# openai/ot-gan

Hardware: AMD Instinct MI355X
Metric: OT-GAN train images/sec (CIFAR-10 32x32, bs=256/GPU) (higher is better)
Workload: dtype f32 (Winograd-domain GEMMs on the fp16 matrix pipe with operands split into two scaled fp16 pieces = 22 significand bits, fp32 accumulate; errors at or below the fp32 MFMA chain's)

## Files before the change

### include/otgan_layers.h

```cpp
#ifndef OTGAN_LAYERS_H
#define OTGAN_LAYERS_H

#define OTGAN_ACT_NONE 0
#define OTGAN_ACT_CRELU 1
#define OTGAN_ACT_CELU 2
#define OTGAN_ACT_ELU 3
#define OTGAN_ACT_RELU 4

typedef struct otgan_conv_desc {
  int N;
  int H, W;
  int C;
  int ldx;
  int upsample;
  int KH, KW;
  int stride;
  int Cout;
  int ldy;
  int y_coff;
  int preact;
  int list_quads;
  const float* x_amax;
  const float* dy_amax;
  int y_accumulate;
  void* x_operand;
  float* y_amax_out;
  float* dx_amax_out;
  const float* w_amax;
  int x_amax_count;
  int list_width;
  float* glu_out;
  float* glu_amax_out;
  int dy_amax_count;
} otgan_conv_desc;


size_t otgan_conv2d_workspace_bytes(const otgan_conv_desc* d, int which);
int otgan_conv2d_glu_fused(const otgan_conv_desc* d);
size_t otgan_conv2d_operand_bytes(const otgan_conv_desc* d);

#define OTGAN_AMAX_RECORD_FLOATS 512
int otgan_absmax_f32(const float* x, long rows, int C, long ld, float* record, void* stream);
int otgan_conv2d_amax_fused(const otgan_conv_desc* d, int which);


size_t otgan_conv2d_folded_weight_elems(const otgan_conv_desc* d);
int otgan_conv2d_fold_weights_f32(const otgan_conv_desc* d, const float* w, float* weff,
                                  float* weffT, void* stream);

int otgan_conv2d_fwd_f32(const otgan_conv_desc* d, const float* x, const int32_t* cmap,
                         const float* wT, const float* bias, float* y, void* workspace,
                         size_t workspace_bytes, void* stream);

int otgan_conv2d_dgrad_f32(const otgan_conv_desc* d, const float* dy, const float* w,
                           const float* x, const int32_t* inv, float* dx, int lddx,
                           int accumulate, void* workspace, size_t workspace_bytes, void* stream);

size_t otgan_conv2d_filter_bytes(const otgan_conv_desc* d, int which);
#define OTGAN_DENSE16_MAX_BATCH 16
size_t otgan_dense16_filter_bytes(int nslices);
int otgan_dense16_prepare_filters_f32(const float* const* wT, const int* nslices, void* const* filters, int count,
                                      void* stream);
int otgan_dense16_h2_ok(const otgan_conv_desc* d);
int otgan_dense16_chain_fwd_f32(int N, int H, int W, int nslices, float* buf_group, int ld, const void* const* filters,
                                float* records, void* stream);
int otgan_dense16_chain_bwd_f32(int N, int H, int W, int nslices, float* g_group, int ldg, const float* x_group, int ldx,
                                const void* const* filters, const float* rec0, float* slice_records, void* stream);
typedef struct otgan_dense16_bwd_pair {
  const float* w;
  const void* fwd_filters;
  void* filters;
  int nslices_src, slice_index, pair_index;
} otgan_dense16_bwd_pair;
size_t otgan_dense16_bwd_filter_bytes(int npairs);
int otgan_dense16_prepare_bwd_filters_f32(const otgan_dense16_bwd_pair* pairs, int npairs, const void* const* all_fwd_filters,
                                          int nall, void* stream);
int otgan_dense16_bwd_slice_f32(int N, int H, int W, int npairs, const float* g, int ldg, const void* filters, const float* x,
                                int ldx, float* dx, const float* rec0, int nrec0, const float* rec1, int nrec1,
                                float* amax_out, void* stream);
int otgan_conv2d_prepare_filters_f32(const otgan_conv_desc* d, int which, const float* w, void* filters,
                                     size_t filter_bytes, void* stream);
int otgan_conv2d_prepare_filters_raw_f32(const otgan_conv_desc* d, int which, const float* V, const float* scale,
                                         void* filters, size_t filter_bytes, void* stream);
int otgan_conv2d_fwd_pf_f32(const otgan_conv_desc* d, const float* x, const int32_t* cmap,
                            const float* wT, const void* filters, const float* bias, float* y,
                            void* workspace, size_t workspace_bytes, void* stream);
int otgan_conv2d_dgrad_pf_f32(const otgan_conv_desc* d, const float* dy, const float* w, const void* filters,
                              const float* x, const int32_t* inv, float* dx, int lddx,
                              int accumulate, void* workspace, size_t workspace_bytes, void* stream);

int otgan_conv2d_wgrad_f32(const otgan_conv_desc* d, const float* x, const int32_t* cmap,
                           const float* dy, float* dw, void* workspace, size_t workspace_bytes,
                           void* stream);

int otgan_weightnorm_fwd_f32(const float* V, const float* g, int K, int Cout, float* w,
                             float* wT, float* inv_norm, void* stream);
int otgan_weightnorm_fwd_amax_f32(const float* V, const float* g, int K, int Cout, float* w, float* wT,
                                  float* inv_norm, float* w_amax, void* stream);
size_t otgan_weightnorm_scale_scratch_floats(int K, int Cout);
int otgan_weightnorm_scale_amax_f32(const float* V, const float* g, int K, int Cout, float* inv_norm, float* scale,
                                    float* w_amax, float* scratch, size_t scratch_floats, void* stream);
int otgan_weightnorm_bwd_f32(const float* V, const float* g, const float* inv_norm,
                             const float* dw, int K, int Cout, float* dV, float* dg,
                             float* scratch, void* stream);

#define OTGAN_WN_MAX_LAYERS 16
typedef struct otgan_wn_fwd_layer {
  const float* V;
  const float* g;
  float* w;
  float* wT;
  float* inv;
  int K;
} otgan_wn_fwd_layer;
typedef struct otgan_wn_part {
  const float* p;
  const int32_t* perm;
  int nrows;
  int rstride;
} otgan_wn_part;
typedef struct otgan_wn_bwd_layer {
  const float* V;
  const float* g;
  const float* inv;
  float* dV;
  float* dg;
  int Ceff, taps;
  otgan_wn_part part[3];
} otgan_wn_bwd_layer;
int otgan_weightnorm_fwd_batched16_f32(const otgan_wn_fwd_layer* layers, int n_layers, void* stream);
int otgan_weightnorm_bwd_batched16_f32(const otgan_wn_bwd_layer* layers, int n_layers, void* stream);

int otgan_colsum_f32(const float* a, long rows, int cols, long lda, float* out, float* scratch,
                     void* stream);

int otgan_glu_fwd_f32(const float* x, long rows, int C, float* y, void* stream);
int otgan_glu_bwd_f32(const float* x, const float* dy, long rows, int C, float* dx, void* stream);
int otgan_glu_fwd_amax_f32(const float* x, long rows, int C, float* y, float* y_amax, void* stream);
int otgan_glu_bwd_amax_f32(const float* x, const float* dy, long rows, int C, float* dx, float* dx_amax, void* stream);
int otgan_glu_bwd_colsum_f32(const float* x, const float* dy, long rows, int C, float* dx, float* dx_amax, float* colsum,
                             float* scratch, void* stream);
int otgan_tanh_fwd_f32(const float* x, long n, float* y, void* stream);
int otgan_tanh_bwd_f32(const float* y, const float* dy, long n, float* dx, void* stream);
int otgan_feature_head_fwd_f32(const float* x, int N, int HW, int C, float* f, float* norm,
                               void* stream);
int otgan_feature_head_bwd_f32(const float* x, const float* f, const float* norm,
                               const float* df, int N, int HW, int C, float* dx, void* stream);
int otgan_feature_head_bwd_amax_f32(const float* x, const float* f, const float* norm, const float* df, int N, int HW,
                                    int C, float* dx, float* dx_amax, void* stream);

int otgan_adam_step_f32(float* p, const float* grad, float* v, float* mg, long n, double lr,
                        double mom1, double mom2, double t, void* stream);
#define OTGAN_ADAM_MAX_SEGMENTS 32
int otgan_adam_step_gather_f32(float* p, const float* const* grads, const long* offsets, int nseg, float* v, float* mg,
                               double lr, double mom1, double mom2, double t, float* ema_shadow, double ema_decay,
                               void* stream);
void otgan_adam_coefficients(double mom1, double mom2, double t, float* out2);
int otgan_adam_step_coef_f32(float* p, const float* grad, float* v, float* mg, long n, double lr,
                             double mom1, double mom2, double t, const float* coef_dev, void* stream);
int otgan_adam_step_gather_coef_f32(float* p, const float* const* grads, const long* offsets, int nseg, float* v, float* mg,
                                    double lr, double mom1, double mom2, double t, const float* coef_dev, float* ema_shadow,
                                    double ema_decay, void* stream);
#define OTGAN_COPY2D_MAX_SEGMENTS 64
int otgan_copy2d_batched_f32(const float* const* src, float* const* dst, const int* rows, const int* cols,
                             const long* src_ld, const long* dst_ld, int nseg, void* stream);
#define OTGAN_GATHER3D_MAX_SEGMENTS 32
int otgan_gather3d_batched_f32(const float* const* src, float* const* dst, const int* n0, int n1, int n2,
                               const long* src_s0, const long* src_s1, const long* dst_s0, const long* dst_s1,
                               int base1, const int* map1_dev, float* amax_out, int nseg, void* stream);
int otgan_adamax_step_f32(float* p, const float* grad, float* v, float* mg, long n, double lr,
                          double mom1, double mom2, void* stream);
int otgan_nesterov_step_f32(float* p, const float* grad, float* v, long n, double lr, double mom1,
                            void* stream);
int otgan_ema_update_f32(float* shadow, const float* p, long n, double decay, void* stream);

typedef struct otgan_incep_conv_desc {
  int N, H, W;
  int C, ldx;
  int KH, KW;
  int stride_h, stride_w;
  int same;
  int Cout;
  int ldy, y_coff;
  int relu;
} otgan_incep_conv_desc;

#define OTGAN_INCEP_POOL_MAX 0
#define OTGAN_INCEP_POOL_AVG 1
typedef struct otgan_incep_pool_desc {
  int N, H, W, C, ldx;
  int KH, KW, stride_h, stride_w, same;
  int op;
  int ldy, y_coff;
} otgan_incep_pool_desc;

int otgan_incep_out_size(int in, int k, int stride, int same);
int otgan_incep_conv2d_f32(const otgan_incep_conv_desc* d, const float* x, const float* w, const float* bias, float* y,
                           void* stream);
int otgan_incep_pool_f32(const otgan_incep_pool_desc* d, const float* x, float* y, void* stream);
int otgan_incep_resize_f32(int N, int H, int W, int C, int OH, int OW, int align_corners, float scale, float shift,
                           const float* x, float* y, void* stream);
int otgan_incep_head_f32(int N, int HW, int C, int ldx, int classes, const float* x, const float* w, float* pool3,
                         float* logits, float* probs, void* stream);

int otgan_moments_update_f64(int n, int C, int ldx, const float* x, double* sum, double* outer, void* stream);

size_t otgan_kid_workspace_bytes(int nsub, int m);
int otgan_kid_sums_f64(int nsub, int m, int C, const float* x, int ldx, const int32_t* xi, const float* y, int ldy,
                       const int32_t* yi, double* out, void* workspace, size_t workspace_bytes, void* stream);

size_t otgan_knn_workspace_bytes(int nq, int ny, int k);
int otgan_knn_f64(int nq, int ny, int C, const float* q, int ldq, const float* y, int ldy, int k, int self0,
                  const double* thresh, double* nearest, int32_t* inside, void* workspace, size_t workspace_bytes,
                  void* stream);

size_t otgan_topk_dot_workspace_bytes(int nq, int ny, int k);
int otgan_topk_dot_f64(int nq, int ny, int C, const float* q, int ldq, const float* y, int ldy, int k, int self0,
                       int32_t* index, double* score, void* workspace, size_t workspace_bytes, void* stream);

#define OTGAN_BATCH_U8_MAX_SHARDS 32
int otgan_batch_from_u8_f32(const uint8_t* store, long n_images, int SH, int SW, const int32_t* perm, long perm_len,
                            const long* shard_offsets, int n_shards, int B, const uint8_t* flip, const float* lut, int S,
                            float* out, long ldo, void* stream);

#define OTGAN_AUG_COLOR 1
#define OTGAN_AUG_TRANSLATION 2
#define OTGAN_AUG_CUTOUT 4
int otgan_augment_fwd_f32(const float* x, long rows, int S, const float* u, int policy, float* y, void* stream);
int otgan_augment_bwd_f32(const float* dy, long rows, int S, const float* u, int policy, float* dx, void* stream);

#endif
```

### ot-gan_amd/_lib_layers.py

```python
import ctypes

c_fp = ctypes.c_void_p
c_int, c_long, c_float, c_size_t = ctypes.c_int, ctypes.c_long, ctypes.c_float, ctypes.c_size_t
c_double = ctypes.c_double


class ConvDesc(ctypes.Structure):
    _fields_ = [("N", c_int), ("H", c_int), ("W", c_int), ("C", c_int), ("ldx", c_int),
                ("upsample", c_int), ("KH", c_int), ("KW", c_int), ("stride", c_int),
                ("Cout", c_int), ("ldy", c_int), ("y_coff", c_int), ("preact", c_int),
                ("list_quads", c_int), ("x_amax", ctypes.c_void_p), ("dy_amax", ctypes.c_void_p),
                ("y_accumulate", c_int), ("x_operand", ctypes.c_void_p),
                ("y_amax_out", ctypes.c_void_p), ("dx_amax_out", ctypes.c_void_p), ("w_amax", ctypes.c_void_p),
                ("x_amax_count", c_int), ("list_width", c_int),
                ("glu_out", ctypes.c_void_p), ("glu_amax_out", ctypes.c_void_p), ("dy_amax_count", c_int)]


P_DESC = ctypes.POINTER(ConvDesc)


class IncepConvDesc(ctypes.Structure):
    _fields_ = [("N", c_int), ("H", c_int), ("W", c_int), ("C", c_int), ("ldx", c_int), ("KH", c_int), ("KW", c_int),
                ("stride_h", c_int), ("stride_w", c_int), ("same", c_int), ("Cout", c_int), ("ldy", c_int),
                ("y_coff", c_int), ("relu", c_int)]


class IncepPoolDesc(ctypes.Structure):
    _fields_ = [("N", c_int), ("H", c_int), ("W", c_int), ("C", c_int), ("ldx", c_int), ("KH", c_int), ("KW", c_int),
                ("stride_h", c_int), ("stride_w", c_int), ("same", c_int), ("op", c_int), ("ldy", c_int),
                ("y_coff", c_int)]


INCEP_POOL_MAX, INCEP_POOL_AVG = 0, 1


class Dense16BwdPair(ctypes.Structure):
    _fields_ = [("w", ctypes.c_void_p), ("fwd_filters", ctypes.c_void_p), ("filters", ctypes.c_void_p),
                ("nslices_src", c_int), ("slice_index", c_int), ("pair_index", c_int)]


class WnFwdLayer(ctypes.Structure):
    _fields_ = [("V", c_fp), ("g", c_fp), ("w", c_fp), ("wT", c_fp), ("inv", c_fp), ("K", c_int)]


class WnPart(ctypes.Structure):
    _fields_ = [("p", c_fp), ("perm", c_fp), ("nrows", c_int), ("rstride", c_int)]


class WnBwdLayer(ctypes.Structure):
    _fields_ = [("V", c_fp), ("g", c_fp), ("inv", c_fp), ("dV", c_fp), ("dg", c_fp), ("Ceff", c_int), ("taps", c_int),
                ("part", WnPart * 3)]


SIGNATURES = {
    "otgan_conv2d_workspace_bytes": (c_size_t, [P_DESC, c_int]),
    "otgan_conv2d_operand_bytes": (c_size_t, [P_DESC]),
    "otgan_conv2d_glu_fused": (c_int, [P_DESC]),
    "otgan_absmax_f32": (c_int, [c_fp, c_long, c_int, c_long, c_fp, c_fp]),
    "otgan_conv2d_amax_fused": (c_int, [P_DESC, c_int]),
    "otgan_conv2d_folded_weight_elems": (c_size_t, [P_DESC]),
    "otgan_conv2d_fold_weights_f32": (c_int, [P_DESC, c_fp, c_fp, c_fp, c_fp]),
    "otgan_conv2d_fwd_f32": (c_int, [P_DESC, c_fp, c_fp, c_fp, c_fp, c_fp, c_fp, c_size_t, c_fp]),
    "otgan_conv2d_dgrad_f32": (c_int, [P_DESC, c_fp, c_fp, c_fp, c_fp, c_fp, c_int, c_int, c_fp,
                                       c_size_t, c_fp]),
    "otgan_conv2d_wgrad_f32": (c_int, [P_DESC, c_fp, c_fp, c_fp, c_fp, c_fp, c_size_t, c_fp]),
    "otgan_conv2d_filter_bytes": (c_size_t, [P_DESC, c_int]),
    "otgan_dense16_filter_bytes": (c_size_t, [c_int]),
    "otgan_dense16_prepare_filters_f32": (c_int, [c_fp, c_fp, c_fp, c_int, c_fp]),
    "otgan_dense16_h2_ok": (c_int, [P_DESC]),
    "otgan_dense16_chain_fwd_f32": (c_int, [c_int, c_int, c_int, c_int, c_fp, c_int, c_fp, c_fp, c_fp]),
    "otgan_dense16_chain_bwd_f32": (c_int, [c_int, c_int, c_int, c_int, c_fp, c_int, c_fp, c_int, c_fp, c_fp, c_fp, c_fp]),
    "otgan_dense16_bwd_filter_bytes": (c_size_t, [c_int]),
    "otgan_dense16_prepare_bwd_filters_f32": (c_int, [c_fp, c_int, c_fp, c_int, c_fp]),
    "otgan_dense16_bwd_slice_f32": (c_int, [c_int, c_int, c_int, c_int, c_fp, c_int, c_fp, c_fp, c_int, c_fp, c_fp, c_int,
                                            c_fp, c_int, c_fp, c_fp]),
    "otgan_conv2d_prepare_filters_f32": (c_int, [P_DESC, c_int, c_fp, c_fp, c_size_t, c_fp]),
    "otgan_conv2d_fwd_pf_f32": (c_int, [P_DESC, c_fp, c_fp, c_fp, c_fp, c_fp, c_fp, c_fp, c_size_t, c_fp]),
    "otgan_conv2d_dgrad_pf_f32": (c_int, [P_DESC, c_fp, c_fp, c_fp, c_fp, c_fp, c_fp, c_int, c_int, c_fp,
                                          c_size_t, c_fp]),
    "otgan_weightnorm_fwd_f32": (c_int, [c_fp, c_fp, c_int, c_int, c_fp, c_fp, c_fp, c_fp]),
    "otgan_weightnorm_fwd_amax_f32": (c_int, [c_fp, c_fp, c_int, c_int, c_fp, c_fp, c_fp, c_fp, c_fp]),
    "otgan_weightnorm_scale_scratch_floats": (c_size_t, [c_int, c_int]),
    "otgan_weightnorm_scale_amax_f32": (c_int, [c_fp, c_fp, c_int, c_int, c_fp, c_fp, c_fp, c_fp, c_size_t, c_fp]),
    "otgan_conv2d_prepare_filters_raw_f32": (c_int, [P_DESC, c_int, c_fp, c_fp, c_fp, c_size_t, c_fp]),
    "otgan_weightnorm_bwd_f32": (c_int, [c_fp, c_fp, c_fp, c_fp, c_int, c_int, c_fp, c_fp, c_fp, c_fp]),
    "otgan_weightnorm_fwd_batched16_f32": (c_int, [ctypes.POINTER(WnFwdLayer), c_int, c_fp]),
    "otgan_weightnorm_bwd_batched16_f32": (c_int, [ctypes.POINTER(WnBwdLayer), c_int, c_fp]),
    "otgan_colsum_f32": (c_int, [c_fp, c_long, c_int, c_long, c_fp, c_fp, c_fp]),
    "otgan_glu_fwd_f32": (c_int, [c_fp, c_long, c_int, c_fp, c_fp]),
    "otgan_glu_bwd_f32": (c_int, [c_fp, c_fp, c_long, c_int, c_fp, c_fp]),
    "otgan_glu_fwd_amax_f32": (c_int, [c_fp, c_long, c_int, c_fp, c_fp, c_fp]),
    "otgan_glu_bwd_amax_f32": (c_int, [c_fp, c_fp, c_long, c_int, c_fp, c_fp, c_fp]),
    "otgan_feature_head_bwd_amax_f32": (c_int, [c_fp, c_fp, c_fp, c_fp, c_int, c_int, c_int, c_fp, c_fp, c_fp]),
    "otgan_tanh_fwd_f32": (c_int, [c_fp, c_long, c_fp, c_fp]),
    "otgan_tanh_bwd_f32": (c_int, [c_fp, c_fp, c_long, c_fp, c_fp]),
    "otgan_feature_head_fwd_f32": (c_int, [c_fp, c_int, c_int, c_int, c_fp, c_fp, c_fp]),
    "otgan_feature_head_bwd_f32": (c_int, [c_fp, c_fp, c_fp, c_fp, c_int, c_int, c_int, c_fp, c_fp]),
    "otgan_adam_step_f32": (c_int, [c_fp, c_fp, c_fp, c_fp, c_long, c_double, c_double, c_double,
                                    c_double, c_fp]),
    "otgan_adam_step_gather_f32": (c_int, [c_fp, c_fp, c_fp, c_int, c_fp, c_fp, c_double, c_double, c_double, c_double,
                                           c_fp, c_double, c_fp]),
    "otgan_adam_step_gather_coef_f32": (c_int, [c_fp, c_fp, c_fp, c_int, c_fp, c_fp, c_double, c_double, c_double, c_double,
                                                c_fp, c_fp, c_double, c_fp]),
    "otgan_adam_coefficients": (None, [c_double, c_double, c_double, c_fp]),
    "otgan_adam_step_coef_f32": (c_int, [c_fp, c_fp, c_fp, c_fp, c_long, c_double, c_double, c_double,
                                         c_double, c_fp, c_fp]),
    "otgan_glu_bwd_colsum_f32": (c_int, [c_fp, c_fp, c_long, c_int, c_fp, c_fp, c_fp, c_fp, c_fp]),
    "otgan_copy2d_batched_f32": (c_int, [c_fp, c_fp, c_fp, c_fp, c_fp, c_fp, c_int, c_fp]),
    "otgan_gather3d_batched_f32": (c_int, [c_fp, c_fp, c_fp, c_int, c_int, c_fp, c_fp, c_fp, c_fp, c_int, c_fp, c_fp, c_int, c_fp]),
    "otgan_adamax_step_f32": (c_int, [c_fp, c_fp, c_fp, c_fp, c_long, c_double, c_double, c_double, c_fp]),
    "otgan_nesterov_step_f32": (c_int, [c_fp, c_fp, c_fp, c_long, c_double, c_double, c_fp]),
    "otgan_ema_update_f32": (c_int, [c_fp, c_fp, c_long, c_double, c_fp]),
    "otgan_incep_out_size": (c_int, [c_int, c_int, c_int, c_int]),
    "otgan_incep_conv2d_f32": (c_int, [ctypes.POINTER(IncepConvDesc), c_fp, c_fp, c_fp, c_fp, c_fp]),
    "otgan_incep_pool_f32": (c_int, [ctypes.POINTER(IncepPoolDesc), c_fp, c_fp, c_fp]),
    "otgan_incep_resize_f32": (c_int, [c_int, c_int, c_int, c_int, c_int, c_int, c_int, c_float, c_float, c_fp, c_fp, c_fp]),
    "otgan_incep_head_f32": (c_int, [c_int, c_int, c_int, c_int, c_int, c_fp, c_fp, c_fp, c_fp, c_fp, c_fp]),
    "otgan_moments_update_f64": (c_int, [c_int, c_int, c_int, c_fp, c_fp, c_fp, c_fp]),
    "otgan_kid_workspace_bytes": (c_size_t, [c_int, c_int]),
    "otgan_kid_sums_f64": (c_int, [c_int, c_int, c_int, c_fp, c_int, c_fp, c_fp, c_int, c_fp, c_fp, c_fp, c_size_t, c_fp]),
    "otgan_knn_workspace_bytes": (c_size_t, [c_int, c_int, c_int]),
    "otgan_knn_f64": (c_int, [c_int, c_int, c_int, c_fp, c_int, c_fp, c_int, c_int, c_int, c_fp, c_fp, c_fp, c_fp, c_size_t, c_fp]),
    "otgan_topk_dot_workspace_bytes": (c_size_t, [c_int, c_int, c_int]),
    "otgan_topk_dot_f64": (c_int, [c_int, c_int, c_int, c_fp, c_int, c_fp, c_int, c_int, c_int, c_fp, c_fp, c_fp, c_size_t, c_fp]),
    "otgan_batch_from_u8_f32": (c_int, [c_fp, c_long, c_int, c_int, c_fp, c_long, c_fp, c_int, c_int, c_fp, c_fp, c_int,
                                        c_fp, c_long, c_fp]),
    "otgan_augment_fwd_f32": (c_int, [c_fp, c_long, c_int, c_fp, c_int, c_fp, c_fp]),
    "otgan_augment_bwd_f32": (c_int, [c_fp, c_long, c_int, c_fp, c_int, c_fp, c_fp]),
}
```

### ot-gan_amd/csrc/pointwise.hip

```cpp
#include "common.h"
#include "../../include/otgan.h"

namespace {

constexpr int kChunks = 256;

inline int grid_for(long n, int per_thread = 4) {
  long b = ceil_div_l(n, 256L * per_thread);
  if (b > 4096) b = 4096;
  if (b < 1) b = 1;
  return (int)b;
}

template <int OP, bool CMAX>
__device__ __forceinline__ void colreduce_body(const float* __restrict__ a, const float* __restrict__ b, long rows,
                                               int cols, long lda, float* __restrict__ partial,
                                               unsigned* __restrict__ pmax) {
  const int lane = threadIdx.x & 63, wave = threadIdx.x >> 6;
  const int c = blockIdx.x * 64 + lane;
  const int chunk = blockIdx.y;
  const long per = ceil_div_l(rows, (long)gridDim.y);
  const long r0 = chunk * per;
  long r1 = r0 + per;
  if (r1 > rows) r1 = rows;
  float s = 0.f;
  unsigned m = 0u;
  if (c < cols) {
    for (long r = r0 + wave; r < r1; r += 4) {
      const float av = a[r * lda + c];
      if (OP == 0) s += av;
      else if (OP == 1) s += av * av;
      else s += av * b[r * lda + c];
      if constexpr (CMAX) {
        const unsigned ab = amax_bits(av);
        m = ab > m ? ab : m;
      }
    }
  }
  __shared__ float red[4][64];
  red[wave][lane] = s;
  __syncthreads();
  if (wave == 0 && c < cols)
    partial[(long)chunk * cols + c] = (red[0][lane] + red[1][lane]) + (red[2][lane] + red[3][lane]);
  if constexpr (CMAX) {
    __shared__ unsigned redm[4][64];
    redm[wave][lane] = m;
    __syncthreads();
    if (wave == 0 && c < cols) {
#pragma unroll
      for (int k = 1; k < 4; ++k) m = redm[k][lane] > m ? redm[k][lane] : m;
      pmax[(long)chunk * cols + c] = m;
    }
  }
}
template <int OP>
__global__ __launch_bounds__(256) void colreduce_kernel(const float* __restrict__ a,
                                                        const float* __restrict__ b, long rows,
                                                        int cols, long lda,
                                                        float* __restrict__ partial) {
  colreduce_body<OP, false>(a, b, rows, cols, lda, partial, nullptr);
}
__global__ __launch_bounds__(256) void colsq_cmax_kernel(const float* __restrict__ a, long rows, int cols, long lda,
                                                         float* __restrict__ partial, unsigned* __restrict__ pmax) {
  colreduce_body<1, true>(a, nullptr, rows, cols, lda, partial, pmax);
}

template <int MODE>
__global__ __launch_bounds__(256) void colreduce_finish_kernel(const float* __restrict__ partial,
                                                               int nchunk, int cols,
                                                               float* __restrict__ out) {
  const int lane = threadIdx.x & 63, part = threadIdx.x >> 6;
  const int c = blockIdx.x * 64 + lane;
  float s = 0.f;
  if (c < cols)
    for (int k = part; k < nchunk; k += 4) s += partial[(long)k * cols + c];
  __shared__ float red[4][64];
  red[part][lane] = s;
  __syncthreads();
  if (part == 0 && c < cols) {
    const float t = (red[0][lane] + red[1][lane]) + (red[2][lane] + red[3][lane]);
    out[c] = MODE == 1 ? rsqrtf(fmaxf(t, 1e-12f)) : t;
  }
}

template <int OP, bool CMAX>
__device__ __forceinline__ void colreduce4_body(const float* __restrict__ a, const float* __restrict__ b, long rows,
                                                int cols, long lda, float* __restrict__ partial,
                                                unsigned* __restrict__ pmax) {
  const int lane = threadIdx.x & 63, wave = threadIdx.x >> 6;
  const int cq = lane & 15, rsub = (lane >> 4) + 4 * wave;
  const int c = blockIdx.x * 64 + 4 * cq;
  const int chunk = blockIdx.y;
  const long per = ceil_div_l(rows, (long)gridDim.y);
  const long r0 = chunk * per;
  long r1 = r0 + per;
  if (r1 > rows) r1 = rows;
  float4 s = make_float4(0.f, 0.f, 0.f, 0.f);
  uint4 m = make_uint4(0u, 0u, 0u, 0u);
  if (c < cols) {
    for (long r = r0 + rsub; r < r1; r += 16) {
      const float4 av = *reinterpret_cast<const float4*>(a + r * lda + c);
      if (OP == 0) {
        s.x += av.x; s.y += av.y; s.z += av.z; s.w += av.w;
      } else if (OP == 1) {
        s.x += av.x * av.x; s.y += av.y * av.y; s.z += av.z * av.z; s.w += av.w * av.w;
      } else {
        const float4 bv = *reinterpret_cast<const float4*>(b + r * lda + c);
        s.x += av.x * bv.x; s.y += av.y * bv.y; s.z += av.z * bv.z; s.w += av.w * bv.w;
      }
      if constexpr (CMAX) {
        const unsigned bx = amax_bits(av.x), by = amax_bits(av.y), bz = amax_bits(av.z), bw = amax_bits(av.w);
        m.x = bx > m.x ? bx : m.x; m.y = by > m.y ? by : m.y; m.z = bz > m.z ? bz : m.z; m.w = bw > m.w ? bw : m.w;
      }
    }
  }
  __shared__ float4 red[16][17];
  red[rsub][cq] = s;
  __syncthreads();
  if (threadIdx.x < 16 && c < cols) {
    float4 t = make_float4(0.f, 0.f, 0.f, 0.f);
#pragma unroll
    for (int k = 0; k < 16; ++k) {
      const float4 v = red[k][threadIdx.x];
      t.x += v.x; t.y += v.y; t.z += v.z; t.w += v.w;
    }
    const int cc = blockIdx.x * 64 + 4 * threadIdx.x;
    *reinterpret_cast<float4*>(partial + (long)chunk * cols + cc) = t;
  }
  if constexpr (CMAX) {
    __shared__ uint4 redm[16][17];
    redm[rsub][cq] = m;
    __syncthreads();
    if (threadIdx.x < 16 && c < cols) {
      uint4 u = make_uint4(0u, 0u, 0u, 0u);
#pragma unroll
      for (int k = 0; k < 16; ++k) {
        const uint4 v = redm[k][threadIdx.x];
        u.x = v.x > u.x ? v.x : u.x; u.y = v.y > u.y ? v.y : u.y; u.z = v.z > u.z ? v.z : u.z; u.w = v.w > u.w ? v.w : u.w;
      }
      *reinterpret_cast<uint4*>(pmax + (long)chunk * cols + (blockIdx.x * 64 + 4 * threadIdx.x)) = u;
    }
  }
}
template <int OP>
__global__ __launch_bounds__(256) void colreduce4_kernel(const float* __restrict__ a,
                                                         const float* __restrict__ b, long rows,
                                                         int cols, long lda,
                                                         float* __restrict__ partial) {
  colreduce4_body<OP, false>(a, b, rows, cols, lda, partial, nullptr);
}
__global__ __launch_bounds__(256) void colsq_cmax4_kernel(const float* __restrict__ a, long rows, int cols, long lda,
                                                          float* __restrict__ partial, unsigned* __restrict__ pmax) {
  colreduce4_body<1, true>(a, nullptr, rows, cols, lda, partial, pmax);
}

template <int OP>
int colreduce(const float* a, const float* b, long rows, int cols, long lda, float* partial,
              int* nchunk_out, hipStream_t s, unsigned* pmax = nullptr) {
  const int colblocks = ceil_div(cols, 64);
  long nchunk = ceil_div(1024, colblocks);
  if (nchunk > kChunks) nchunk = kChunks;
  if (nchunk > ceil_div_l(rows, 64)) nchunk = ceil_div_l(rows, 64);
  if (nchunk < 1) nchunk = 1;
  dim3 grid(colblocks, (int)nchunk);
  const bool vec = (cols % 4 == 0) && (lda % 4 == 0) && ((reinterpret_cast<uintptr_t>(a) & 15) == 0) &&
                   (!b || (reinterpret_cast<uintptr_t>(b) & 15) == 0) &&
                   ((reinterpret_cast<uintptr_t>(partial) & 15) == 0) &&
                   ((reinterpret_cast<uintptr_t>(pmax) & 15) == 0);
  if (pmax) {
    if (vec) hipLaunchKernelGGL(colsq_cmax4_kernel, grid, dim3(256), 0, s, a, rows, cols, lda, partial, pmax);
    else hipLaunchKernelGGL(colsq_cmax_kernel, grid, dim3(256), 0, s, a, rows, cols, lda, partial, pmax);
  } else if (vec) hipLaunchKernelGGL(colreduce4_kernel<OP>, grid, dim3(256), 0, s, a, b, rows, cols, lda, partial);
  else hipLaunchKernelGGL(colreduce_kernel<OP>, grid, dim3(256), 0, s, a, b, rows, cols, lda, partial);
  *nchunk_out = (int)nchunk;
  OTGAN_CHECK_LAUNCH("colreduce");
  return OTGAN_OK;
}

__global__ __launch_bounds__(256) void weightnorm_apply_kernel(const float* __restrict__ V,
                                                               const float* __restrict__ g,
                                                               const float* __restrict__ inv,
                                                               int K, int Cout,
                                                               float* __restrict__ w,
                                                               float* __restrict__ wT,
                                                               float* __restrict__ rec) {
  __shared__ float tile[32][33];
  const int c0 = blockIdx.x * 32, k0 = blockIdx.y * 32;
  const int tx = threadIdx.x & 31, ty = threadIdx.x >> 5;
  unsigned mb = 0u;
#pragma unroll
  for (int i = 0; i < 4; ++i) {
    const int k = k0 + ty + 8 * i, c = c0 + tx;
    float v = 0.f;
    if (k < K && c < Cout) {
      v = V[(long)k * Cout + c] * (g[c] * inv[c]);
      w[(long)k * Cout + c] = v;
    }
    tile[ty + 8 * i][tx] = v;
    const unsigned b = amax_bits(v);
    mb = b > mb ? b : mb;
  }
  if (wT) {
    __syncthreads();
#pragma unroll
    for (int i = 0; i < 4; ++i) {
      const int c = c0 + ty + 8 * i, k = k0 + tx;
      if (k < K && c < Cout) wT[(long)c * K + k] = tile[tx][ty + 8 * i];
    }
  }
  if (rec) amax_commit(rec, mb);
}

__global__ __launch_bounds__(256) void weightnorm_scale_finish_kernel(const float* __restrict__ partial,
                                                                      const unsigned* __restrict__ pmax, int nchunk,
                                                                      int cols, const float* __restrict__ g,
                                                                      float* __restrict__ inv, float* __restrict__ scale,
                                                                      float* __restrict__ rec) {
  const int lane = threadIdx.x & 63, part = threadIdx.x >> 6;
  const int c = blockIdx.x * 64 + lane;
  float s = 0.f;
  unsigned m = 0u;
  if (c < cols)
    for (int k = part; k < nchunk; k += 4) {
      s += partial[(long)k * cols + c];
      const unsigned b = pmax[(long)k * cols + c];
      m = b > m ? b : m;
    }
  __shared__ float red[4][64];
  __shared__ unsigned redm[4][64];
  red[part][lane] = s;
  redm[part][lane] = m;
  __syncthreads();
  unsigned mb = 0u;
  if (part == 0 && c < cols) {
    const float t = (red[0][lane] + red[1][lane]) + (red[2][lane] + red[3][lane]);
    const float iv = rsqrtf(fmaxf(t, 1e-12f));
    const float sc = __fmul_rn(g[c], iv);
#pragma unroll
    for (int k = 1; k < 4; ++k) m = redm[k][lane] > m ? redm[k][lane] : m;
    inv[c] = iv;
    scale[c] = sc;
    mb = amax_bits(__fmul_rn(__uint_as_float(m), sc));
  }
  amax_commit(rec, mb);
}

__global__ void weightnorm_bwd_kernel(const float* __restrict__ V, const float* __restrict__ g,
                                      const float* __restrict__ inv, const float* __restrict__ dw,
                                      const float* __restrict__ dot, long total, int Cout,
                                      float* __restrict__ dV) {
  for (long i = (long)blockIdx.x * blockDim.x + threadIdx.x; i < total;
       i += (long)gridDim.x * blockDim.x) {
    const int c = (int)(i % Cout);
    const float iv = inv[c];
    dV[i] = g[c] * iv * (dw[i] - V[i] * dot[c] * iv * iv);
  }
}
__global__ __launch_bounds__(256) void wn_dot_finish_kernel(const float* __restrict__ partial, int nchunk, int cols,
                                                            const float* __restrict__ inv, float* __restrict__ dot,
                                                            float* __restrict__ dg) {
  const int lane = threadIdx.x & 63, part = threadIdx.x >> 6;
  const int c = blockIdx.x * 64 + lane;
  float s = 0.f;
  if (c < cols)
    for (int k = part; k < nchunk; k += 4) s += partial[(long)k * cols + c];
  __shared__ float red[4][64];
  red[part][lane] = s;
  __syncthreads();
  if (part == 0 && c < cols) {
    const float t = (red[0][lane] + red[1][lane]) + (red[2][lane] + red[3][lane]);
    dot[c] = t;
    dg[c] = t * inv[c];
  }
}
__global__ void weightnorm_dg_kernel(const float* __restrict__ dot, const float* __restrict__ inv,
                                     int Cout, float* __restrict__ dg) {
  const int c = blockIdx.x * blockDim.x + threadIdx.x;
  if (c < Cout) dg[c] = dot[c] * inv[c];
}

constexpr int kWnThreads = 512, kWnRowLanes = kWnThreads / 4;
inline bool aligned16(const void* p) { return (reinterpret_cast<uintptr_t>(p) & 15) == 0; }
struct WnFwdArgs {
  otgan_wn_fwd_layer l[OTGAN_WN_MAX_LAYERS];
};
struct WnBwdArgs {
  otgan_wn_bwd_layer l[OTGAN_WN_MAX_LAYERS];
};
__device__ __forceinline__ float4 wn_tree(float4 v, float4 (*red)[4], int rl, int cq) {
  red[rl][cq] = v;
  __syncthreads();
#pragma unroll
  for (int h = kWnRowLanes / 2; h > 0; h >>= 1) {
    if (rl < h) {
      const float4 a = red[rl][cq], b = red[rl + h][cq];
      red[rl][cq] = make_float4(a.x + b.x, a.y + b.y, a.z + b.z, a.w + b.w);
    }
    __syncthreads();
  }
  const float4 r = red[0][cq];
  __syncthreads();
  return r;
}
__global__ __launch_bounds__(kWnThreads) void wn_fwd_batched_kernel(WnFwdArgs a) {
  __shared__ float4 red[kWnRowLanes][4];
  const otgan_wn_fwd_layer& L = a.l[blockIdx.x];
  const int cq = threadIdx.x & 3, rl = threadIdx.x >> 2;
  float4 s = make_float4(0.f, 0.f, 0.f, 0.f);
  for (int r = rl; r < L.K; r += kWnRowLanes) {
    const float4 v = *reinterpret_cast<const float4*>(L.V + (long)r * 16 + 4 * cq);
    s.x += v.x * v.x; s.y += v.y * v.y; s.z += v.z * v.z; s.w += v.w * v.w;
  }
  s = wn_tree(s, red, rl, cq);
  const float4 g = *reinterpret_cast<const float4*>(L.g + 4 * cq);
  const float4 iv = make_float4(rsqrtf(fmaxf(s.x, 1e-12f)), rsqrtf(fmaxf(s.y, 1e-12f)), rsqrtf(fmaxf(s.z, 1e-12f)),
                                rsqrtf(fmaxf(s.w, 1e-12f)));
  if (rl == 0) *reinterpret_cast<float4*>(L.inv + 4 * cq) = iv;
  const float4 sc = make_float4(g.x * iv.x, g.y * iv.y, g.z * iv.z, g.w * iv.w);
  for (int r = rl; r < L.K; r += kWnRowLanes) {
    const float4 v = *reinterpret_cast<const float4*>(L.V + (long)r * 16 + 4 * cq);
    const float4 w = make_float4(v.x * sc.x, v.y * sc.y, v.z * sc.z, v.w * sc.w);
    *reinterpret_cast<float4*>(L.w + (long)r * 16 + 4 * cq) = w;
    if (L.wT) {
      float* t = L.wT + (long)(4 * cq) * L.K + r;
      t[0] = w.x; t[L.K] = w.y; t[2L * L.K] = w.z; t[3L * L.K] = w.w;
    }
  }
}
__device__ __forceinline__ const float* wn_dw_row(const otgan_wn_bwd_layer& L, int tap, int e) {
#pragma unroll
  for (int i = 0; i < 3; ++i) {
    const otgan_wn_part& p = L.part[i];
    if (e < p.nrows || i == 2) {
      const int ee = p.perm ? p.perm[e] : e;
      return p.p + ((long)tap * p.nrows + ee) * p.rstride;
    }
    e -= p.nrows;
  }
  return nullptr;
}
__global__ __launch_bounds__(kWnThreads) void wn_bwd_batched_kernel(WnBwdArgs a) {
  __shared__ float4 red[kWnRowLanes][4];
  const otgan_wn_bwd_layer& L = a.l[blockIdx.x];
  const int cq = threadIdx.x & 3, rl = threadIdx.x >> 2;
  const int K = L.taps * L.Ceff;
  float4 s = make_float4(0.f, 0.f, 0.f, 0.f);
  for (int r = rl; r < K; r += kWnRowLanes) {
    const int tap = r / L.Ceff, e = r - tap * L.Ceff;
    const float4 d = *reinterpret_cast<const float4*>(wn_dw_row(L, tap, e) + 4 * cq);
    const float4 v = *reinterpret_cast<const float4*>(L.V + (long)r * 16 + 4 * cq);
    s.x += d.x * v.x; s.y += d.y * v.y; s.z += d.z * v.z; s.w += d.w * v.w;
  }
  s = wn_tree(s, red, rl, cq);
  const float4 g = *reinterpret_cast<const float4*>(L.g + 4 * cq);
  const float4 iv = *reinterpret_cast<const float4*>(L.inv + 4 * cq);
  if (rl == 0) *reinterpret_cast<float4*>(L.dg + 4 * cq) = make_float4(s.x * iv.x, s.y * iv.y, s.z * iv.z, s.w * iv.w);
  const float4 sc = make_float4(g.x * iv.x, g.y * iv.y, g.z * iv.z, g.w * iv.w);
  const float4 pr = make_float4(s.x * iv.x * iv.x, s.y * iv.y * iv.y, s.z * iv.z * iv.z, s.w * iv.w * iv.w);
  for (int r = rl; r < K; r += kWnRowLanes) {
    const int tap = r / L.Ceff, e = r - tap * L.Ceff;
    const float4 d = *reinterpret_cast<const float4*>(wn_dw_row(L, tap, e) + 4 * cq);
    const float4 v = *reinterpret_cast<const float4*>(L.V + (long)r * 16 + 4 * cq);
    *reinterpret_cast<float4*>(L.dV + (long)r * 16 + 4 * cq) =
        make_float4(sc.x * (d.x - v.x * pr.x), sc.y * (d.y - v.y * pr.y), sc.z * (d.z - v.z * pr.z), sc.w * (d.w - v.w * pr.w));
  }
}

__device__ __forceinline__ float sigmoidf_(float x) { return 1.f / (1.f + expf(-x)); }

__global__ void glu_fwd_kernel(const float* __restrict__ x, long rows, int C, float* __restrict__ y) {
  const long total = rows * C;
  for (long i = (long)blockIdx.x * blockDim.x + threadIdx.x; i < total;
       i += (long)gridDim.x * blockDim.x) {
    const long r = i / C;
    const int c = (int)(i - r * C);
    const float a = x[r * 2 * C + c], l = x[r * 2 * C + C + c];
    y[i] = a * sigmoidf_(l);
  }
}
__global__ void glu_bwd_kernel(const float* __restrict__ x, const float* __restrict__ dy, long rows,
                               int C, float* __restrict__ dx) {
  const long total = rows * C;
  for (long i = (long)blockIdx.x * blockDim.x + threadIdx.x; i < total;
       i += (long)gridDim.x * blockDim.x) {
    const long r = i / C;
    const int c = (int)(i - r * C);
    const float a = x[r * 2 * C + c], l = x[r * 2 * C + C + c];
    const float s = sigmoidf_(l), d = dy[i];
    dx[r * 2 * C + c] = d * s;
    dx[r * 2 * C + C + c] = d * a * s * (1.f - s);
  }
}
__global__ __launch_bounds__(256) void glu_fwd4_kernel(const float* __restrict__ x, long rows, int C4,
                                                       float* __restrict__ y, float* __restrict__ rec) {
  const long total = rows * C4;
  unsigned mb = 0u;
  for (long i = (long)blockIdx.x * 256 + threadIdx.x; i < total; i += (long)gridDim.x * 256) {
    const long r = i / C4;
    const long c = i - r * C4;
    const f32x4 a = *reinterpret_cast<const f32x4*>(x + 4 * (r * 2 * C4 + c));
    const f32x4 l = *reinterpret_cast<const f32x4*>(x + 4 * (r * 2 * C4 + C4 + c));
    f32x4 o;
#pragma unroll
    for (int k = 0; k < 4; ++k) o[k] = a[k] * sigmoidf_(l[k]);
    *reinterpret_cast<f32x4*>(y + 4 * i) = o;
    mb = amax_bits4(o, mb);
  }
  if (rec) amax_commit(rec, mb);
}
__global__ __launch_bounds__(256) void glu_bwd4_kernel(const float* __restrict__ x, const float* __restrict__ dy,
                                                       long rows, int C4, float* __restrict__ dx,
                                                       float* __restrict__ rec) {
  const long total = rows * C4;
  unsigned mb = 0u;
  for (long i = (long)blockIdx.x * 256 + threadIdx.x; i < total; i += (long)gridDim.x * 256) {
    const long r = i / C4;
    const long c = i - r * C4;
    const f32x4 a = *reinterpret_cast<const f32x4*>(x + 4 * (r * 2 * C4 + c));
    const f32x4 l = *reinterpret_cast<const f32x4*>(x + 4 * (r * 2 * C4 + C4 + c));
    const f32x4 d = *reinterpret_cast<const f32x4*>(dy + 4 * i);
    f32x4 da, dl;
#pragma unroll
    for (int k = 0; k < 4; ++k) {
      const float s = sigmoidf_(l[k]);
      da[k] = d[k] * s;
      dl[k] = d[k] * a[k] * s * (1.f - s);
    }
    *reinterpret_cast<f32x4*>(dx + 4 * (r * 2 * C4 + c)) = da;
    *reinterpret_cast<f32x4*>(dx + 4 * (r * 2 * C4 + C4 + c)) = dl;
    mb = amax_bits4(dl, amax_bits4(da, mb));
  }
  if (rec) amax_commit(rec, mb);
}
__global__ __launch_bounds__(256) void glu_bwd4_colsum_kernel(const float* __restrict__ x, const float* __restrict__ dy,
                                                              long rows, int C, float* __restrict__ dx,
                                                              float* __restrict__ rec, float* __restrict__ partial) {
  const int lane = threadIdx.x & 63, wave = threadIdx.x >> 6;
  const int cq = lane & 15, rsub = (lane >> 4) + 4 * wave;
  const int c = blockIdx.x * 64 + 4 * cq;
  const int chunk = blockIdx.y;
  const long per = ceil_div_l(rows, (long)gridDim.y);
  const long r0 = chunk * per;
  long r1 = r0 + per;
  if (r1 > rows) r1 = rows;
  f32x4 sa = {0.f, 0.f, 0.f, 0.f}, sl = {0.f, 0.f, 0.f, 0.f};
  unsigned mb = 0u;
  if (c < C) {
    for (long r = r0 + rsub; r < r1; r += 16) {
      const f32x4 a = *reinterpret_cast<const f32x4*>(x + r * 2 * C + c);
      const f32x4 l = *reinterpret_cast<const f32x4*>(x + r * 2 * C + C + c);
      const f32x4 d = *reinterpret_cast<const f32x4*>(dy + r * C + c);
      f32x4 da, dl;
#pragma unroll
      for (int k = 0; k < 4; ++k) {
        const float sg = sigmoidf_(l[k]);
        da[k] = d[k] * sg;
        dl[k] = d[k] * a[k] * sg * (1.f - sg);
      }
      *reinterpret_cast<f32x4*>(dx + r * 2 * C + c) = da;
      *reinterpret_cast<f32x4*>(dx + r * 2 * C + C + c) = dl;
      sa += da;
      sl += dl;
      mb = amax_bits4(dl, amax_bits4(da, mb));
    }
  }
  __shared__ f32x4 red[2][16][17];
  red[0][rsub][cq] = sa;
  red[1][rsub][cq] = sl;
  __syncthreads();
  if (threadIdx.x < 32) {
    const int half = threadIdx.x >> 4, q = threadIdx.x & 15;
    const int cc = blockIdx.x * 64 + 4 * q;
    if (cc < C) {
      f32x4 t = {0.f, 0.f, 0.f, 0.f};
#pragma unroll
      for (int k = 0; k < 16; ++k) t += red[half][k][q];
      *reinterpret_cast<f32x4*>(partial + (long)chunk * 2 * C + half * C + cc) = t;
    }
  }
  if (rec) amax_commit(rec, mb);
}
__global__ void tanh_fwd_kernel(const float* __restrict__ x, long n, float* __restrict__ y) {
  for (long i = (long)blockIdx.x * blockDim.x + threadIdx.x; i < n; i += (long)gridDim.x * blockDim.x)
    y[i] = tanhf(x[i]);
}
__global__ void tanh_bwd_kernel(const float* __restrict__ y, const float* __restrict__ dy, long n,
                                float* __restrict__ dx) {
  for (long i = (long)blockIdx.x * blockDim.x + threadIdx.x; i < n; i += (long)gridDim.x * blockDim.x)
    dx[i] = dy[i] * (1.f - y[i] * y[i]);
}

__device__ __forceinline__ double block_sum_d(double v, double* red) {
  v = wave_sum_d(v);
  const int wave = threadIdx.x >> 6, lane = threadIdx.x & 63;
  __syncthreads();
  if (lane == 0) red[wave] = v;
  __syncthreads();
  double s = 0;
  for (int k = 0; k < (int)(blockDim.x >> 6); ++k) s += red[k];
  return s;
}

template <int THREADS>
__global__ __launch_bounds__(THREADS) void feature_head_fwd4_kernel(const float* __restrict__ x, int HW, int C4,
                                                                    float* __restrict__ f, float* __restrict__ norm) {
  __shared__ double red[THREADS / 64];
  const int n = blockIdx.x;
  const long per4 = (long)HW * C4;
  const f32x4* xp = reinterpret_cast<const f32x4*>(x) + n * per4;
  double s = 0;
  for (long i = threadIdx.x; i < per4; i += THREADS) {
    const f32x4 v = xp[i];
    s += (double)v[0] * v[0] + (double)v[1] * v[1] + (double)v[2] * v[2] + (double)v[3] * v[3];
  }
  s = block_sum_d(s, red);
  const float nrm = (float)sqrt(s);
  if (threadIdx.x == 0) norm[n] = nrm;
  f32x4* fp = reinterpret_cast<f32x4*>(f) + n * per4 * 2;
  for (long i = threadIdx.x; i < per4; i += THREADS) {
    const long p = i / C4;
    const long c = i - p * C4;
    const f32x4 v = xp[i];
    f32x4 a, b;
#pragma unroll
    for (int k = 0; k < 4; ++k) {
      a[k] = fmaxf(v[k], 0.f) / nrm;
      b[k] = fmaxf(-v[k], 0.f) / nrm;
    }
    fp[p * 2 * C4 + c] = a;
    fp[p * 2 * C4 + C4 + c] = b;
  }
}
template <int THREADS>
__global__ __launch_bounds__(THREADS) void feature_head_bwd4_kernel(const float* __restrict__ x, const float* __restrict__ f,
                                                                    const float* __restrict__ norm, const float* __restrict__ df,
                                                                    int HW, int C4, float* __restrict__ dx, float* __restrict__ rec) {
  __shared__ double red[THREADS / 64];
  const int n = blockIdx.x;
  const long per4 = (long)HW * C4;
  const f32x4* fp = reinterpret_cast<const f32x4*>(f) + n * per4 * 2;
  const f32x4* dfp = reinterpret_cast<const f32x4*>(df) + n * per4 * 2;
  double s = 0;
  for (long i = threadIdx.x; i < 2 * per4; i += THREADS) {
    const f32x4 a = fp[i], b = dfp[i];
    s += (double)a[0] * b[0] + (double)a[1] * b[1] + (double)a[2] * b[2] + (double)a[3] * b[3];
  }
  s = block_sum_d(s, red);
  const float dot = (float)s, inv = 1.f / norm[n];
  const f32x4* xp = reinterpret_cast<const f32x4*>(x) + n * per4;
  f32x4* dxp = reinterpret_cast<f32x4*>(dx) + n * per4;
  unsigned mb = 0u;
  for (long i = threadIdx.x; i < per4; i += THREADS) {
    const long p = i / C4;
    const long c = i - p * C4;
    const f32x4 v = xp[i];
    const long ip = p * 2 * C4 + c, in = ip + C4;
    const f32x4 fpv = fp[ip], fnv = fp[in], dpv = dfp[ip], dnv = dfp[in];
    f32x4 o;
#pragma unroll
    for (int k = 0; k < 4; ++k) {
      const float dup = (dpv[k] - fpv[k] * dot) * inv;
      const float dun = (dnv[k] - fnv[k] * dot) * inv;
      o[k] = v[k] > 0.f ? dup : (v[k] < 0.f ? -dun : 0.f);
    }
    dxp[i] = o;
    mb = amax_bits4(o, mb);
  }
  if (rec) amax_commit(rec, mb);
}

__global__ __launch_bounds__(256) void feature_head_fwd_kernel(const float* __restrict__ x, int HW,
                                                               int C, float* __restrict__ f,
                                                               float* __restrict__ norm) {
  __shared__ double red[4];
  const int n = blockIdx.x;
  const long per = (long)HW * C;
  const float* xp = x + n * per;
  double s = 0;
  for (long i = threadIdx.x; i < per; i += blockDim.x) s += (double)xp[i] * (double)xp[i];
  s = block_sum_d(s, red);
  const float nrm = (float)sqrt(s);
  if (threadIdx.x == 0) norm[n] = nrm;
  float* fp = f + n * per * 2;
  for (long i = threadIdx.x; i < per; i += blockDim.x) {
    const long p = i / C;
    const int c = (int)(i - p * C);
    const float v = xp[i];
    fp[p * 2 * C + c] = fmaxf(v, 0.f) / nrm;
    fp[p * 2 * C + C + c] = fmaxf(-v, 0.f) / nrm;
  }
}
__global__ __launch_bounds__(256) void feature_head_bwd_kernel(const float* __restrict__ x,
                                                               const float* __restrict__ f,
                                                               const float* __restrict__ norm,
                                                               const float* __restrict__ df, int HW,
                                                               int C, float* __restrict__ dx,
                                                               float* __restrict__ rec) {
  __shared__ double red[4];
  const int n = blockIdx.x;
  const long per = (long)HW * C;
  const float* fp = f + n * per * 2;
  const float* dfp = df + n * per * 2;
  double s = 0;
  for (long i = threadIdx.x; i < 2 * per; i += blockDim.x) s += (double)fp[i] * (double)dfp[i];
  s = block_sum_d(s, red);
  const float dot = (float)s, inv = 1.f / norm[n];
  const float* xp = x + n * per;
  float* dxp = dx + n * per;
  unsigned mb = 0u;
  for (long i = threadIdx.x; i < per; i += blockDim.x) {
    const long p = i / C;
    const int c = (int)(i - p * C);
    const float v = xp[i];
    const long ip = p * 2 * C + c, in = ip + C;
    const float dup = (dfp[ip] - fp[ip] * dot) * inv;
    const float dun = (dfp[in] - fp[in] * dot) * inv;
    const float o = v > 0.f ? dup : (v < 0.f ? -dun : 0.f);
    dxp[i] = o;
    const unsigned b = amax_bits(o);
    mb = b > mb ? b : mb;
  }
  if (rec) amax_commit(rec, mb);
}

__device__ __forceinline__ float adam_elem(float p, float gi, float* __restrict__ v, float* __restrict__ mg, long j, float lr,
                                           float mom1, float om1, float mom2, float om2, float c1, float c2) {
#pragma clang fp contract(off)
  float vhat;
  if (mom1 > 0.f) {
    const float vt = mom1 * v[j] + om1 * gi;
    v[j] = vt;
    vhat = vt / c1;
  } else {
    vhat = gi;
  }
  const float mgt = mom2 * mg[j] + om2 * gi * gi;
  mg[j] = mgt;
  const float mghat = mgt / c2;
  const float step = lr * (vhat / sqrtf(mghat + 1e-8f));
  return p - step;
}
__device__ __forceinline__ float ema_elem(float sh, float p, float decay, float omd) {
#pragma clang fp contract(off)
  return decay * sh + omd * p;
}
__global__ void adam_kernel(float* __restrict__ p, const float* __restrict__ g, float* __restrict__ v,
                            float* __restrict__ mg, long n, float lr, float mom1, float om1,
                            float mom2, float om2, float c1, float c2, const float* __restrict__ coef) {
  if (coef) {
    c1 = coef[0];
    c2 = coef[1];
  }
  for (long i = (long)blockIdx.x * blockDim.x + threadIdx.x; i < n; i += (long)gridDim.x * blockDim.x)
    p[i] = adam_elem(p[i], g[i], v, mg, i, lr, mom1, om1, mom2, om2, c1, c2);
}
__global__ void adamax_kernel(float* __restrict__ p, const float* __restrict__ g,
                              float* __restrict__ v, float* __restrict__ mg, long n, float lr,
                              float mom1, float om1, float mom2) {
#pragma clang fp contract(off)
  for (long i = (long)blockIdx.x * blockDim.x + threadIdx.x; i < n; i += (long)gridDim.x * blockDim.x) {
    const float gi = g[i];
    float vt = gi;
    if (mom1 > 0.f) {
      vt = mom1 * v[i] + om1 * gi;
      v[i] = vt;
    }
    const float mgt = fmaxf(mom2 * mg[i] + 1e-8f, fabsf(gi));
    mg[i] = mgt;
    p[i] -= lr * (vt / mgt);
  }
}
__global__ void nesterov_kernel(float* __restrict__ p, const float* __restrict__ g,
                                float* __restrict__ v, long n, float lr, float mom1, float opm) {
#pragma clang fp contract(off)
  for (long i = (long)blockIdx.x * blockDim.x + threadIdx.x; i < n; i += (long)gridDim.x * blockDim.x) {
    const float vo = v[i];
    const float vn = mom1 * vo - lr * g[i];
    p[i] = p[i] - mom1 * vo + opm * vn;
    v[i] = vn;
  }
}
struct Copy2dSegs {
  const float* src[OTGAN_COPY2D_MAX_SEGMENTS];
  float* dst[OTGAN_COPY2D_MAX_SEGMENTS];
  int rows[OTGAN_COPY2D_MAX_SEGMENTS], cols[OTGAN_COPY2D_MAX_SEGMENTS];
  long sld[OTGAN_COPY2D_MAX_SEGMENTS], dld[OTGAN_COPY2D_MAX_SEGMENTS];
};
__global__ __launch_bounds__(256) void copy2d_batched_kernel(Copy2dSegs g) {
  const int sg = blockIdx.y;
  const int rows = g.rows[sg], cols = g.cols[sg];
  const float* __restrict__ src = g.src[sg];
  float* __restrict__ dst = g.dst[sg];
  const long sld = g.sld[sg], dld = g.dld[sg];
  const long total = (long)rows * cols;
  for (long i = (long)blockIdx.x * 256 + threadIdx.x; i < total; i += (long)gridDim.x * 256) {
    const long r = i / cols, c = i - r * cols;
    dst[r * dld + c] = src[r * sld + c];
  }
}
extern "C" int otgan_copy2d_batched_f32(const float* const* src, float* const* dst, const int* rows, const int* cols,
                                        const long* src_ld, const long* dst_ld, int nseg, void* stream) {
  OTGAN_CHECK_ARG(src && dst && rows && cols && src_ld && dst_ld && nseg > 0 && nseg <= OTGAN_COPY2D_MAX_SEGMENTS, "bad arguments");
  Copy2dSegs g;
  long most = 0;
  for (int i = 0; i < nseg; ++i) {
    OTGAN_CHECK_ARG(src[i] && dst[i] && rows[i] > 0 && cols[i] > 0 && src_ld[i] >= cols[i] && dst_ld[i] >= cols[i], "bad segment");
    g.src[i] = src[i]; g.dst[i] = dst[i]; g.rows[i] = rows[i]; g.cols[i] = cols[i]; g.sld[i] = src_ld[i]; g.dld[i] = dst_ld[i];
    const long t = (long)rows[i] * cols[i];
    most = t > most ? t : most;
  }
  long bx = (most + 256 * 4 - 1) / (256 * 4);
  if (bx > 256) bx = 256;
  hipLaunchKernelGGL(copy2d_batched_kernel, dim3((unsigned)bx, (unsigned)nseg), dim3(256), 0, (hipStream_t)stream, g);
  OTGAN_CHECK_LAUNCH("copy2d_batched");
  return OTGAN_OK;
}

struct Gather3dSegs {
  const float* src[OTGAN_GATHER3D_MAX_SEGMENTS];
  float* dst[OTGAN_GATHER3D_MAX_SEGMENTS];
  int n0[OTGAN_GATHER3D_MAX_SEGMENTS];
  long ss0[OTGAN_GATHER3D_MAX_SEGMENTS], ss1[OTGAN_GATHER3D_MAX_SEGMENTS];
  long ds0[OTGAN_GATHER3D_MAX_SEGMENTS], ds1[OTGAN_GATHER3D_MAX_SEGMENTS];
  int n1, n2, base1;
  const int* map1;
  float* amax;
};
__global__ __launch_bounds__(256) void gather3d_batched_kernel(Gather3dSegs g) {
  const int sg = blockIdx.y;
  const float* __restrict__ src = g.src[sg];
  float* __restrict__ dst = g.dst[sg];
  const long ss0 = g.ss0[sg], ss1 = g.ss1[sg], ds0 = g.ds0[sg], ds1 = g.ds1[sg];
  const int n1 = g.n1, n2 = g.n2;
  const long total = (long)g.n0[sg] * n1 * n2;
  unsigned mb = 0u;
  for (long i = (long)blockIdx.x * 256 + threadIdx.x; i < total; i += (long)gridDim.x * 256) {
    const int i2 = (int)(i % n2);
    const long r = i / n2;
    const int i1 = (int)(r % n1);
    const long i0 = r / n1;
    const int j1 = g.base1 + (g.map1 ? g.map1[i1] : i1);
    const float v = src[i0 * ss0 + j1 * ss1 + i2];
    const unsigned b = amax_bits(v);
    mb = b > mb ? b : mb;
    dst[i0 * ds0 + i1 * ds1 + i2] = v;
  }
  if (g.amax) amax_commit(g.amax, mb);
}
extern "C" int otgan_gather3d_batched_f32(const float* const* src, float* const* dst, const int* n0, int n1, int n2,
                                          const long* src_s0, const long* src_s1, const long* dst_s0, const long* dst_s1,
                                          int base1, const int* map1_dev, float* amax_out, int nseg, void* stream) {
  OTGAN_CHECK_ARG(src && dst && n0 && src_s0 && src_s1 && dst_s0 && dst_s1 && n1 > 0 && n2 > 0 && base1 >= 0 && nseg > 0 &&
                  nseg <= OTGAN_GATHER3D_MAX_SEGMENTS, "bad arguments");
  Gather3dSegs g;
  long most = 0;
  for (int i = 0; i < nseg; ++i) {
    OTGAN_CHECK_ARG(src[i] && dst[i] && n0[i] > 0, "bad segment");
    g.src[i] = src[i]; g.dst[i] = dst[i]; g.n0[i] = n0[i];
    g.ss0[i] = src_s0[i]; g.ss1[i] = src_s1[i]; g.ds0[i] = dst_s0[i]; g.ds1[i] = dst_s1[i];
    const long t = (long)n0[i] * n1 * n2;
    most = t > most ? t : most;
  }
  g.n1 = n1; g.n2 = n2; g.base1 = base1; g.map1 = map1_dev; g.amax = amax_out;
  long bx = (most + 256 * 4 - 1) / (256 * 4);
  if (bx > 256) bx = 256;
  hipLaunchKernelGGL(gather3d_batched_kernel, dim3((unsigned)bx, (unsigned)nseg), dim3(256), 0, (hipStream_t)stream, g);
  OTGAN_CHECK_LAUNCH("gather3d_batched");
  return OTGAN_OK;
}

struct AdamSegs {
  const float* g[OTGAN_ADAM_MAX_SEGMENTS];
  long off[OTGAN_ADAM_MAX_SEGMENTS + 1];
};
__global__ void adam_gather_kernel(float* __restrict__ p, AdamSegs segs, float* __restrict__ v, float* __restrict__ mg,
                                   float lr, float mom1, float om1, float mom2, float om2, float c1, float c2,
                                   float* __restrict__ sh, float decay, float omd, const float* __restrict__ coef) {
  if (coef) {
    c1 = coef[0];
    c2 = coef[1];
  }
  const int seg = blockIdx.y;
  const long base = segs.off[seg], n = segs.off[seg + 1] - base;
  const float* __restrict__ g = segs.g[seg];
  for (long i = (long)blockIdx.x * blockDim.x + threadIdx.x; i < n; i += (long)gridDim.x * blockDim.x) {
    const long j = base + i;
    const float pn = adam_elem(p[j], g[i], v, mg, j, lr, mom1, om1, mom2, om2, c1, c2);
    p[j] = pn;
    if (sh) sh[j] = ema_elem(sh[j], pn, decay, omd);
  }
}
__global__ void ema_kernel(float* __restrict__ sh, const float* __restrict__ p, long n, float decay,
                           float omd) {
  for (long i = (long)blockIdx.x * blockDim.x + threadIdx.x; i < n; i += (long)gridDim.x * blockDim.x)
    sh[i] = ema_elem(sh[i], p[i], decay, omd);
}

}

extern "C" {

int otgan_weightnorm_fwd_amax_f32(const float* V, const float* g, int K, int Cout, float* w, float* wT,
                                  float* inv_norm, float* w_amax, void* stream) {
  OTGAN_CHECK_ARG(V && g && w && inv_norm && K > 0 && Cout > 0, "bad arguments");
  hipStream_t s = (hipStream_t)stream;
  ProfScope ps(OTGAN_PROF_POINTWISE, 0.0, 4.0 * 3 * (double)K * Cout, s);
  float* partial = w;
  int nchunk = 0;
  int rc = colreduce<1>(V, nullptr, K, Cout, Cout, partial, &nchunk, s);
  if (rc) return rc;
  hipLaunchKernelGGL(colreduce_finish_kernel<1>, dim3(ceil_div(Cout, 64)), dim3(256), 0, s, partial,
                     nchunk, Cout, inv_norm);
  dim3 grid(ceil_div(Cout, 32), ceil_div(K, 32));
  hipLaunchKernelGGL(weightnorm_apply_kernel, grid, dim3(256), 0, s, V, g, inv_norm, K, Cout, w, wT, w_amax);
  OTGAN_CHECK_LAUNCH("weightnorm fwd");
  return OTGAN_OK;
}
size_t otgan_weightnorm_scale_scratch_floats(int K, int Cout) {
  if (K <= 0 || Cout <= 0) return 0;
  long nchunk = ceil_div_l(K, 64);
  if (nchunk > kChunks) nchunk = kChunks;
  return 2 * (size_t)nchunk * Cout;
}
int otgan_weightnorm_scale_amax_f32(const float* V, const float* g, int K, int Cout, float* inv_norm, float* scale,
                                    float* w_amax, float* scratch, size_t scratch_floats, void* stream) {
  OTGAN_CHECK_ARG(V && g && inv_norm && scale && w_amax && scratch && K > 0 && Cout > 0, "bad arguments");
  OTGAN_CHECK_ARG((reinterpret_cast<uintptr_t>(scratch) & 15) == 0 && scratch_floats >= otgan_weightnorm_scale_scratch_floats(K, Cout),
                  "scratch misaligned or smaller than otgan_weightnorm_scale_scratch_floats");
  hipStream_t s = (hipStream_t)stream;
  ProfScope ps(OTGAN_PROF_POINTWISE, 0.0, 4.0 * (double)K * Cout, s);
  long bound = ceil_div_l(K, 64);
  if (bound > kChunks) bound = kChunks;
  unsigned* pmax = reinterpret_cast<unsigned*>(scratch + (size_t)bound * Cout);
  int nchunk = 0;
  int rc = colreduce<1>(V, nullptr, K, Cout, Cout, scratch, &nchunk, s, pmax);
  if (rc) return rc;
  hipLaunchKernelGGL(weightnorm_scale_finish_kernel, dim3(ceil_div(Cout, 64)), dim3(256), 0, s, scratch, pmax, nchunk,
                     Cout, g, inv_norm, scale, w_amax);
  OTGAN_CHECK_LAUNCH("weightnorm scale");
  return OTGAN_OK;
}
int otgan_weightnorm_fwd_f32(const float* V, const float* g, int K, int Cout, float* w, float* wT, float* inv_norm,
                             void* stream) {
  return otgan_weightnorm_fwd_amax_f32(V, g, K, Cout, w, wT, inv_norm, nullptr, stream);
}

int otgan_weightnorm_bwd_f32(const float* V, const float* g, const float* inv_norm, const float* dw,
                             int K, int Cout, float* dV, float* dg, float* scratch, void* stream) {
  OTGAN_CHECK_ARG(V && g && inv_norm && dw && dV && dg && scratch && K > 0 && Cout > 0, "bad arguments");
  hipStream_t s = (hipStream_t)stream;
  ProfScope ps(OTGAN_PROF_POINTWISE, 0.0, 4.0 * 5 * (double)K * Cout, s);
  float* partial = dV;
  int nchunk = 0;
  int rc = colreduce<2>(dw, V, K, Cout, Cout, partial, &nchunk, s);
  if (rc) return rc;
  hipLaunchKernelGGL(wn_dot_finish_kernel, dim3(ceil_div(Cout, 64)), dim3(256), 0, s, partial, nchunk, Cout, inv_norm, scratch, dg);
  const long total = (long)K * Cout;
  hipLaunchKernelGGL(weightnorm_bwd_kernel, dim3(grid_for(total)), dim3(256), 0, s, V, g, inv_norm, dw,
                     scratch, total, Cout, dV);
  OTGAN_CHECK_LAUNCH("weightnorm bwd");
  return OTGAN_OK;
}

int otgan_weightnorm_fwd_batched16_f32(const otgan_wn_fwd_layer* layers, int n_layers, void* stream) {
  OTGAN_CHECK_ARG(layers && n_layers > 0, "bad arguments");
  hipStream_t s = (hipStream_t)stream;
  double bytes = 0.0;
  for (int i = 0; i < n_layers; ++i) {
    const otgan_wn_fwd_layer& l = layers[i];
    OTGAN_CHECK_ARG(l.V && l.g && l.w && l.inv && l.K > 0, "layer %d: null pointer or empty", i);
    OTGAN_CHECK_ARG(aligned16(l.V) && aligned16(l.g) && aligned16(l.w) && aligned16(l.inv), "layer %d: 16-byte alignment", i);
    bytes += 4.0 * 4 * (double)l.K * 16;
  }
  ProfScope ps(OTGAN_PROF_POINTWISE, 0.0, bytes, s);
  for (int i0 = 0; i0 < n_layers; i0 += OTGAN_WN_MAX_LAYERS) {
    const int n = n_layers - i0 < OTGAN_WN_MAX_LAYERS ? n_layers - i0 : OTGAN_WN_MAX_LAYERS;
    WnFwdArgs a;
    memset(&a, 0, sizeof(a));
    for (int i = 0; i < n; ++i) a.l[i] = layers[i0 + i];
    hipLaunchKernelGGL(wn_fwd_batched_kernel, dim3(n), dim3(kWnThreads), 0, s, a);
  }
  OTGAN_CHECK_LAUNCH("weightnorm fwd (batched)");
  return OTGAN_OK;
}

int otgan_weightnorm_bwd_batched16_f32(const otgan_wn_bwd_layer* layers, int n_layers, void* stream) {
  OTGAN_CHECK_ARG(layers && n_layers > 0, "bad arguments");
  hipStream_t s = (hipStream_t)stream;
  double bytes = 0.0;
  for (int i = 0; i < n_layers; ++i) {
    const otgan_wn_bwd_layer& l = layers[i];
    OTGAN_CHECK_ARG(l.V && l.g && l.inv && l.dV && l.dg && l.Ceff > 0 && l.taps > 0, "layer %d: null pointer or empty", i);
    OTGAN_CHECK_ARG(aligned16(l.V) && aligned16(l.g) && aligned16(l.inv) && aligned16(l.dV) && aligned16(l.dg), "layer %d: 16-byte alignment", i);
    int rows = 0;
    for (int p = 0; p < 3; ++p) {
      const otgan_wn_part& q = l.part[p];
      OTGAN_CHECK_ARG(q.nrows >= 0 && (q.nrows == 0 || (q.p && aligned16(q.p) && q.rstride >= 16 && q.rstride % 4 == 0)),
                      "layer %d part %d: pointer / stride", i, p);
      rows += q.nrows;
    }
    OTGAN_CHECK_ARG(rows == l.Ceff, "layer %d: the parts hold %d rows per tap, Ceff is %d", i, rows, l.Ceff);
    bytes += 4.0 * 5 * (double)l.taps * l.Ceff * 16;
  }
  ProfScope ps(OTGAN_PROF_POINTWISE, 0.0, bytes, s);
  for (int i0 = 0; i0 < n_layers; i0 += OTGAN_WN_MAX_LAYERS) {
    const int n = n_layers - i0 < OTGAN_WN_MAX_LAYERS ? n_layers - i0 : OTGAN_WN_MAX_LAYERS;
    WnBwdArgs a;
    memset(&a, 0, sizeof(a));
    for (int i = 0; i < n; ++i) a.l[i] = layers[i0 + i];
    hipLaunchKernelGGL(wn_bwd_batched_kernel, dim3(n), dim3(kWnThreads), 0, s, a);
  }
  OTGAN_CHECK_LAUNCH("weightnorm bwd (batched)");
  return OTGAN_OK;
}

int otgan_colsum_f32(const float* a, long rows, int cols, long lda, float* out, float* scratch,
                     void* stream) {
  OTGAN_CHECK_ARG(a && out && scratch && rows > 0 && cols > 0 && lda >= cols, "bad arguments");
  hipStream_t s = (hipStream_t)stream;
  ProfScope ps(OTGAN_PROF_POINTWISE, 0.0, 4.0 * (double)rows * cols, s);
  int nchunk = 0;
  int rc = colreduce<0>(a, nullptr, rows, cols, lda, scratch, &nchunk, s);
  if (rc) return rc;
  hipLaunchKernelGGL(colreduce_finish_kernel<0>, dim3(ceil_div(cols, 64)), dim3(256), 0, s, scratch,
                     nchunk, cols, out);
  OTGAN_CHECK_LAUNCH("colsum");
  return OTGAN_OK;
}


int otgan_glu_fwd_amax_f32(const float* x, long rows, int C, float* y, float* y_amax, void* stream) {
  OTGAN_CHECK_ARG(x && y && rows > 0 && C > 0, "bad arguments");
  hipStream_t s = (hipStream_t)stream;
  ProfScope ps(OTGAN_PROF_POINTWISE, 0.0, 4.0 * 3 * (double)rows * C, s);
  if (C % 4 == 0 && aligned16(x) && aligned16(y)) {
    hipLaunchKernelGGL(glu_fwd4_kernel, dim3(grid_for(rows * C, 8)), dim3(256), 0, s, x, rows, C / 4, y, y_amax);
  } else {
    OTGAN_CHECK_ARG(!y_amax, "glu: an amax record needs C %% 4 == 0 and 16-byte aligned tensors");
    hipLaunchKernelGGL(glu_fwd_kernel, dim3(grid_for(rows * C)), dim3(256), 0, s, x, rows, C, y);
  }
  OTGAN_CHECK_LAUNCH("glu fwd");
  return OTGAN_OK;
}
int otgan_glu_fwd_f32(const float* x, long rows, int C, float* y, void* stream) {
  return otgan_glu_fwd_amax_f32(x, rows, C, y, nullptr, stream);
}
int otgan_glu_bwd_amax_f32(const float* x, const float* dy, long rows, int C, float* dx, float* dx_amax, void* stream) {
  OTGAN_CHECK_ARG(x && dy && dx && rows > 0 && C > 0, "bad arguments");
  hipStream_t s = (hipStream_t)stream;
  ProfScope ps(OTGAN_PROF_POINTWISE, 0.0, 4.0 * 5 * (double)rows * C, s);
  if (C % 4 == 0 && aligned16(x) && aligned16(dy) && aligned16(dx)) {
    hipLaunchKernelGGL(glu_bwd4_kernel, dim3(grid_for(rows * C, 8)), dim3(256), 0, s, x, dy, rows, C / 4, dx, dx_amax);
  } else {
    OTGAN_CHECK_ARG(!dx_amax, "glu: an amax record needs C %% 4 == 0 and 16-byte aligned tensors");
    hipLaunchKernelGGL(glu_bwd_kernel, dim3(grid_for(rows * C)), dim3(256), 0, s, x, dy, rows, C, dx);
  }
  OTGAN_CHECK_LAUNCH("glu bwd");
  return OTGAN_OK;
}
int otgan_glu_bwd_colsum_f32(const float* x, const float* dy, long rows, int C, float* dx, float* dx_amax, float* colsum,
                             float* scratch, void* stream) {
  OTGAN_CHECK_ARG(x && dy && dx && colsum && scratch && rows > 0 && C > 0 && C % 4 == 0 && aligned16(x) && aligned16(dy) &&
                      aligned16(dx) && aligned16(scratch),
                  "glu bwd with column sums: C %% 4 == 0 and 16-byte aligned tensors");
  hipStream_t s = (hipStream_t)stream;
  ProfScope ps(OTGAN_PROF_POINTWISE, 0.0, 4.0 * 5 * (double)rows * C, s);
  const int colblocks = ceil_div(C, 64);
  long nchunk = ceil_div(1024, colblocks);
  if (nchunk > kChunks) nchunk = kChunks;
  if (nchunk > ceil_div_l(rows, 64)) nchunk = ceil_div_l(rows, 64);
  if (nchunk < 1) nchunk = 1;
  hipLaunchKernelGGL(glu_bwd4_colsum_kernel, dim3(colblocks, (int)nchunk), dim3(256), 0, s, x, dy, rows, C, dx, dx_amax, scratch);
  hipLaunchKernelGGL(colreduce_finish_kernel<0>, dim3(ceil_div(2 * C, 64)), dim3(256), 0, s, scratch, (int)nchunk, 2 * C, colsum);
  OTGAN_CHECK_LAUNCH("glu bwd (+ column sums)");
  return OTGAN_OK;
}
int otgan_glu_bwd_f32(const float* x, const float* dy, long rows, int C, float* dx, void* stream) {
  return otgan_glu_bwd_amax_f32(x, dy, rows, C, dx, nullptr, stream);
}
int otgan_tanh_fwd_f32(const float* x, long n, float* y, void* stream) {
  OTGAN_CHECK_ARG(x && y && n > 0, "bad arguments");
  hipLaunchKernelGGL(tanh_fwd_kernel, dim3(grid_for(n)), dim3(256), 0, (hipStream_t)stream, x, n, y);
  OTGAN_CHECK_LAUNCH("tanh fwd");
  return OTGAN_OK;
}
int otgan_tanh_bwd_f32(const float* y, const float* dy, long n, float* dx, void* stream) {
  OTGAN_CHECK_ARG(y && dy && dx && n > 0, "bad arguments");
  hipLaunchKernelGGL(tanh_bwd_kernel, dim3(grid_for(n)), dim3(256), 0, (hipStream_t)stream, y, dy, n, dx);
  OTGAN_CHECK_LAUNCH("tanh bwd");
  return OTGAN_OK;
}

int otgan_feature_head_fwd_f32(const float* x, int N, int HW, int C, float* f, float* norm,
                               void* stream) {
  OTGAN_CHECK_ARG(x && f && norm && N > 0 && HW > 0 && C > 0, "bad arguments");
  hipStream_t s = (hipStream_t)stream;
  ProfScope ps(OTGAN_PROF_POINTWISE, 0.0, 4.0 * 4 * (double)N * HW * C, s);
  if (C % 4 == 0 && aligned16(x) && aligned16(f))
    hipLaunchKernelGGL(feature_head_fwd4_kernel<1024>, dim3(N), dim3(1024), 0, s, x, HW, C / 4, f, norm);
  else
    hipLaunchKernelGGL(feature_head_fwd_kernel, dim3(N), dim3(256), 0, s, x, HW, C, f, norm);
  OTGAN_CHECK_LAUNCH("feature head fwd");
  return OTGAN_OK;
}
int otgan_feature_head_bwd_amax_f32(const float* x, const float* f, const float* norm, const float* df,
                                    int N, int HW, int C, float* dx, float* dx_amax, void* stream) {
  OTGAN_CHECK_ARG(x && f && norm && df && dx && N > 0 && HW > 0 && C > 0, "bad arguments");
  hipStream_t s = (hipStream_t)stream;
  ProfScope ps(OTGAN_PROF_POINTWISE, 0.0, 4.0 * 10 * (double)N * HW * C, s);
  if (C % 4 == 0 && aligned16(x) && aligned16(f) && aligned16(df) && aligned16(dx))
    hipLaunchKernelGGL(feature_head_bwd4_kernel<1024>, dim3(N), dim3(1024), 0, s, x, f, norm, df, HW, C / 4, dx, dx_amax);
  else
    hipLaunchKernelGGL(feature_head_bwd_kernel, dim3(N), dim3(256), 0, s, x, f, norm, df, HW, C, dx, dx_amax);
  OTGAN_CHECK_LAUNCH("feature head bwd");
  return OTGAN_OK;
}
int otgan_feature_head_bwd_f32(const float* x, const float* f, const float* norm, const float* df,
                               int N, int HW, int C, float* dx, void* stream) {
  return otgan_feature_head_bwd_amax_f32(x, f, norm, df, N, HW, C, dx, nullptr, stream);
}

void otgan_adam_coefficients(double mom1, double mom2, double t, float* out2) {
  out2[0] = 1.f - powf((float)mom1, (float)t);
  out2[1] = 1.f - powf((float)mom2, (float)t);
}
int otgan_adam_step_f32(float* p, const float* grad, float* v, float* mg, long n, double lr,
                        double mom1, double mom2, double t, void* stream) {
  return otgan_adam_step_coef_f32(p, grad, v, mg, n, lr, mom1, mom2, t, nullptr, stream);
}
int otgan_adam_step_coef_f32(float* p, const float* grad, float* v, float* mg, long n, double lr,
                             double mom1, double mom2, double t, const float* coef_dev, void* stream) {
  OTGAN_CHECK_ARG(p && grad && mg && n > 0 && (coef_dev || t >= 1.0) && (mom1 <= 0.0 || v), "bad arguments");
  hipStream_t s = (hipStream_t)stream;
  ProfScope ps(OTGAN_PROF_POINTWISE, 0.0, 4.0 * 7 * (double)n, s);
  float c[2] = {1.f, 1.f};
  if (!coef_dev) otgan_adam_coefficients(mom1, mom2, t, c);
  hipLaunchKernelGGL(adam_kernel, dim3(grid_for(n)), dim3(256), 0, s, p, grad, v, mg, n, (float)lr,
                     (float)mom1, (float)(1.0 - mom1), (float)mom2, (float)(1.0 - mom2), c[0], c[1], coef_dev);
  OTGAN_CHECK_LAUNCH("adam");
  return OTGAN_OK;
}
int otgan_adam_step_gather_f32(float* p, const float* const* grads, const long* offsets, int nseg, float* v, float* mg,
                               double lr, double mom1, double mom2, double t, float* ema_shadow, double ema_decay,
                               void* stream) {
  return otgan_adam_step_gather_coef_f32(p, grads, offsets, nseg, v, mg, lr, mom1, mom2, t, nullptr, ema_shadow, ema_decay, stream);
}
int otgan_adam_step_gather_coef_f32(float* p, const float* const* grads, const long* offsets, int nseg, float* v, float* mg,
                                    double lr, double mom1, double mom2, double t, const float* coef_dev, float* ema_shadow,
                                    double ema_decay, void* stream) {
  OTGAN_CHECK_ARG(p && grads && offsets && mg && nseg > 0 && nseg <= OTGAN_ADAM_MAX_SEGMENTS && (coef_dev || t >= 1.0) && (mom1 <= 0.0 || v),
                  "bad arguments (at most %d segments)", OTGAN_ADAM_MAX_SEGMENTS);
  hipStream_t s = (hipStream_t)stream;
  AdamSegs segs;
  memset(&segs, 0, sizeof(segs));
  long longest = 0;
  for (int i = 0; i < nseg; ++i) {
    OTGAN_CHECK_ARG(grads[i] && offsets[i + 1] > offsets[i], "segment %d: null gradient or empty range", i);
    segs.g[i] = grads[i];
    segs.off[i] = offsets[i];
    if (offsets[i + 1] - offsets[i] > longest) longest = offsets[i + 1] - offsets[i];
  }
  segs.off[nseg] = offsets[nseg];
  const long n = offsets[nseg] - offsets[0];
  ProfScope ps(OTGAN_PROF_POINTWISE, 0.0, 4.0 * (ema_shadow ? 9 : 7) * (double)n, s);
  float c[2] = {1.f, 1.f};
  if (!coef_dev) otgan_adam_coefficients(mom1, mom2, t, c);
  hipLaunchKernelGGL(adam_gather_kernel, dim3(grid_for(longest), nseg), dim3(256), 0, s, p, segs, v, mg, (float)lr,
                     (float)mom1, (float)(1.0 - mom1), (float)mom2, (float)(1.0 - mom2), c[0], c[1], ema_shadow,
                     (float)ema_decay, (float)(1.0 - ema_decay), coef_dev);
  OTGAN_CHECK_LAUNCH("adam (gathered gradients)");
  return OTGAN_OK;
}
int otgan_adamax_step_f32(float* p, const float* grad, float* v, float* mg, long n, double lr,
                          double mom1, double mom2, void* stream) {
  OTGAN_CHECK_ARG(p && grad && mg && n > 0 && (mom1 <= 0.0 || v), "bad arguments");
  hipLaunchKernelGGL(adamax_kernel, dim3(grid_for(n)), dim3(256), 0, (hipStream_t)stream, p, grad, v,
                     mg, n, (float)lr, (float)mom1, (float)(1.0 - mom1), (float)mom2);
  OTGAN_CHECK_LAUNCH("adamax");
  return OTGAN_OK;
}
int otgan_nesterov_step_f32(float* p, const float* grad, float* v, long n, double lr, double mom1,
                            void* stream) {
  OTGAN_CHECK_ARG(p && grad && v && n > 0, "bad arguments");
  hipLaunchKernelGGL(nesterov_kernel, dim3(grid_for(n)), dim3(256), 0, (hipStream_t)stream, p, grad,
                     v, n, (float)lr, (float)mom1, (float)(1.0 + mom1));
  OTGAN_CHECK_LAUNCH("nesterov");
  return OTGAN_OK;
}
int otgan_ema_update_f32(float* shadow, const float* p, long n, double decay, void* stream) {
  OTGAN_CHECK_ARG(shadow && p && n > 0, "bad arguments");
  hipLaunchKernelGGL(ema_kernel, dim3(grid_for(n)), dim3(256), 0, (hipStream_t)stream, shadow, p, n,
                     (float)decay, (float)(1.0 - decay));
  OTGAN_CHECK_LAUNCH("ema");
  return OTGAN_OK;
}

}
```

### ot-gan_amd/ops.py

```python
import ctypes
import os
import sys
import weakref
from collections import OrderedDict

import torch

from . import _lib
from ._lib_layers import ConvDesc, WnBwdLayer, WnFwdLayer

ACT = {None: 0, "none": 0, "crelu": 1, "celu": 2, "elu": 3, "relu": 4}
DOUBLED = (1, 2)

_ws = {}


class _NullCtx:
    def __enter__(self):
        return None

    def __exit__(self, *exc):
        return False


_NULL_CTX = _NullCtx()


def workspace(nbytes, device):
    key = (device.index if device.index is not None else torch.cuda.current_device(),
           torch.cuda.current_stream(device).cuda_stream)
    buf = _ws.get(key)
    if buf is None or buf.numel() < nbytes:
        buf = torch.empty(int(max(nbytes, 1 << 20)), dtype=torch.uint8, device=device)
        _ws[key] = buf
    return buf


def _need_cuda(*ts):
    for t in ts:
        if t is not None and not t.is_cuda:
            raise _lib.OtganError("otgan_amd ops need CUDA (MI355X) tensors; there is no CPU fallback")


_map_cache = {}


def channel_maps(segs, preact, device):
    segs = tuple(int(s) for s in segs)
    if preact not in DOUBLED or len(segs) <= 1:
        return None, None
    key = (segs, device)
    hit = _map_cache.get(key)
    if hit is not None:
        return hit
    C = sum(segs)
    cmap, invp, invn = [], [0] * C, [0] * C
    off = 0
    for s in segs:
        base = len(cmap)
        cmap += [off + i for i in range(s)]
        cmap += [(off + i) | (1 << 31) for i in range(s)]
        for i in range(s):
            invp[off + i] = base + i
            invn[off + i] = base + s + i
        off += s
    cm = torch.tensor([c - (1 << 32) if c >= (1 << 31) else c for c in cmap], dtype=torch.int32,
                      device=device)
    inv = torch.tensor(invp + invn, dtype=torch.int32, device=device)
    _map_cache[key] = (cm, inv)
    return cm, inv


def make_desc(x, C, upsample, kh, kw, stride, cout, ldy, y_coff, preact, segs=None):
    N, H, W, ldx = x.shape
    quads = 1 if all(int(s) % 4 == 0 for s in (segs or (C,))) else 0
    return ConvDesc(N, H, W, C, ldx, 1 if upsample else 0, kh, kw, stride, cout, ldy, y_coff, preact, quads)


def out_hw(H, W, upsample, stride):
    Hin, Win = (H * 2, W * 2) if upsample else (H, W)
    return -(-Hin // stride), -(-Win // stride)


weights_epoch = 0
_storage_epoch = {}
_wcache = OrderedDict()
_WCACHE_MAX = 1024


def bump_weights_epoch(t=None):
    global weights_epoch
    if t is None:
        weights_epoch += 1
    else:
        key = t.untyped_storage().data_ptr()
        _storage_epoch[key] = _storage_epoch.get(key, 0) + 1


def _epoch_of(t):
    return _storage_epoch.get(t.untyped_storage().data_ptr(), 0)


def _token(V, g):
    return (weights_epoch, _epoch_of(V), _epoch_of(g), V._version, g._version)


def cached_weights(V, g, compute):
    key = id(V)
    token = _token(V, g)
    hit = _wcache.get(key)
    if hit is not None and hit[0] is V and hit[1] is g and hit[2] == token:
        _wcache.move_to_end(key)
        return hit[3]
    val = compute()
    _wcache[key] = (V, g, token, val)
    _wcache.move_to_end(key)
    while len(_wcache) > _WCACHE_MAX:
        _wcache.popitem(last=False)
    return val


def weights_in(t):
    key = t.untyped_storage().data_ptr()
    ents = [(k, e[0], e[1], e[3]) for k, e in _wcache.items() if e[0].untyped_storage().data_ptr() == key]
    mine = {id(e[3][0]) for e in ents}
    blocks = [(k, e) for k, e in _block_cache.items() if e[0] and all(id(w) in mine for w in e[0])]
    return ents, blocks


def forget_weights(t):
    ents, blocks = weights_in(t)
    for k, *_ in ents:
        _wcache.pop(k, None)
    for k, _e in blocks:
        _block_cache.pop(k, None)


def forget_stream(stream):
    for key in [k for k in _ws if k[1] == stream.cuda_stream]:
        del _ws[key]


def forget_side_events():
    for e in _wcache.values():
        if isinstance(e[3][-1], dict):
            e[3][-1].pop("bwd_event", None)


def reinstate_weights(snap):
    ents, blocks = snap
    for k, V, g, val in ents:
        _wcache[k] = (V, g, _token(V, g), val)
        _wcache.move_to_end(k)
    for k, e in blocks:
        _block_cache[k] = e
        _block_cache.move_to_end(k)
    while len(_wcache) > _WCACHE_MAX:
        _wcache.popitem(last=False)
    while len(_block_cache) > 64:
        _block_cache.popitem(last=False)


def weightnorm_fwd(V2d, g):
    K, Cout = V2d.shape
    w = torch.empty_like(V2d)
    wT = torch.empty((Cout, K), dtype=V2d.dtype, device=V2d.device)
    inv = torch.empty(Cout, dtype=V2d.dtype, device=V2d.device)
    rec = amax_slot(V2d.device)
    _lib.check(_lib.lib().otgan_weightnorm_fwd_amax_f32(V2d.data_ptr(), g.data_ptr(), K, Cout,
                                                        w.data_ptr(), wT.data_ptr(), inv.data_ptr(), rec.data_ptr(),
                                                        _lib.stream_ptr()), "weightnorm_fwd")
    tag_amax(w, rec)
    tag_amax(wT, rec)
    return w, wT, inv


FILTERS_FROM_RAW = True


def weightnorm_scale(V2d, g):
    K, Cout = V2d.shape
    L = _lib.lib()
    inv = torch.empty(Cout, dtype=V2d.dtype, device=V2d.device)
    scale = torch.empty(Cout, dtype=V2d.dtype, device=V2d.device)
    rec = amax_slot(V2d.device)
    n = L.otgan_weightnorm_scale_scratch_floats(K, Cout)
    scratch = torch.empty(n, dtype=torch.float32, device=V2d.device)
    _lib.check(L.otgan_weightnorm_scale_amax_f32(V2d.data_ptr(), g.data_ptr(), K, Cout, inv.data_ptr(), scale.data_ptr(),
                                                 rec.data_ptr(), scratch.data_ptr(), n, _lib.stream_ptr()),
               "weightnorm_scale")
    tag_amax(scale, rec)
    leave(scale, "raw", V2d)
    return scale, inv


def weightnorm_bwd(V2d, g, inv, dw):
    K, Cout = V2d.shape
    dV = torch.empty_like(V2d)
    dg = torch.empty_like(g)
    scratch = torch.empty(Cout, dtype=V2d.dtype, device=V2d.device)
    _lib.check(_lib.lib().otgan_weightnorm_bwd_f32(V2d.data_ptr(), g.data_ptr(), inv.data_ptr(),
                                                   dw.data_ptr(), K, Cout, dV.data_ptr(),
                                                   dg.data_ptr(), scratch.data_ptr(),
                                                   _lib.stream_ptr()), "weightnorm_bwd")
    return dV, dg


def colsum(a2d_ptr, rows, cols, lda, device):
    out = torch.empty(cols, dtype=torch.float32, device=device)
    scratch = torch.empty(256 * cols, dtype=torch.float32, device=device)
    _lib.check(_lib.lib().otgan_colsum_f32(a2d_ptr, rows, cols, lda, out.data_ptr(),
                                           scratch.data_ptr(), _lib.stream_ptr()), "colsum")
    return out


_LAUNCH_POINTERS = ("x_amax", "dy_amax", "w_amax", "y_amax_out", "dx_amax_out", "glu_out", "glu_amax_out", "x_operand")
_LAUNCH_INTS = ("ldy", "y_accumulate")


def launch_desc(desc, **fields):
    d = ConvDesc.from_buffer_copy(desc)
    for name, v in fields.items():
        if name in _LAUNCH_INTS:
            setattr(d, name, int(v))
        elif name in _LAUNCH_POINTERS:
            if isinstance(v, tuple):
                v, count = v
                assert name in ("x_amax", "dy_amax"), name
                setattr(d, name + "_count", int(count))
            setattr(d, name, _lib.ptr(v))
        else:
            raise TypeError(f"{name} is not a per-launch field of otgan_conv_desc")
    return d


def conv_fwd_raw(desc, x, cmap, wT, bias, y, filters=None, **fields):
    L = _lib.lib()
    desc = launch_desc(desc, **fields)
    need = L.otgan_conv2d_workspace_bytes(ctypes.byref(desc), 0)
    ws = workspace(need, x.device)
    _lib.check(L.otgan_conv2d_fwd_pf_f32(ctypes.byref(desc), x.data_ptr(), _lib.ptr(cmap),
                                         wT.data_ptr(), _lib.ptr(filters), _lib.ptr(bias), y.data_ptr(),
                                         ws.data_ptr(), ws.numel(), _lib.stream_ptr()), "conv2d_fwd")


def conv_dgrad_raw(desc, dy, w, x, inv, dx, lddx, accumulate, filters=None, **fields):
    L = _lib.lib()
    desc = launch_desc(desc, **fields)
    need = L.otgan_conv2d_workspace_bytes(ctypes.byref(desc), 1)
    ws = workspace(need, dy.device)
    _lib.check(L.otgan_conv2d_dgrad_pf_f32(ctypes.byref(desc), dy.data_ptr(), w.data_ptr(), _lib.ptr(filters),
                                           _lib.ptr(x), _lib.ptr(inv), dx.data_ptr(), lddx,
                                           1 if accumulate else 0, ws.data_ptr(), ws.numel(),
                                           _lib.stream_ptr()), "conv2d_dgrad")


def absmax_record(t):
    rec = torch.empty(AMAX_RECORD_FLOATS, dtype=torch.float32, device=t.device)
    C = t.shape[-1]
    _lib.check(_lib.lib().otgan_absmax_f32(t.data_ptr(), t.numel() // C, C, C, rec.data_ptr(), _lib.stream_ptr()),
               "absmax")
    return rec


AMAX_RECORD_FLOATS = 512
_AMAX_SLOTS = 256
_amax_pool = {}
_GRAD_INPLACE = True
DENSE_SPLIT = True
DENSE_H2_AT_64 = True
DENSE_GROUP = None


_HANDOFF = "_otgan_handoff"


def leave(t, kind, value):
    tag = getattr(t, _HANDOFF, None)
    if tag is None or tag[0] != t._version:
        tag = (t._version, {})
        setattr(t, _HANDOFF, tag)
    tag[1][kind] = value
    return t


def take(t, kind, remove=False):
    tag = getattr(t, _HANDOFF, None)
    if tag is None:
        return None
    if tag[0] != t._version:
        delattr(t, _HANDOFF)
        return None
    return tag[1].pop(kind, None) if remove else tag[1].get(kind)


def forget(t):
    if hasattr(t, _HANDOFF):
        delattr(t, _HANDOFF)


def colsum_of(t):
    return take(t, "colsum")


def amax_slot(device):
    ent = _amax_pool.get(device)
    cur = torch.cuda.current_stream(device)
    if ent is None or ent[1] >= _AMAX_SLOTS:
        pool = torch.zeros((_AMAX_SLOTS, AMAX_RECORD_FLOATS), dtype=torch.float32, device=device)
        ent = [pool, 0, cur.cuda_stream, cur.record_event(), set()]
        _amax_pool[device] = ent
    elif cur.cuda_stream != ent[2] and cur.cuda_stream not in ent[4]:
        cur.wait_event(ent[3])
        ent[0].record_stream(cur)
        ent[4].add(cur.cuda_stream)
    rec = ent[0][ent[1]]
    ent[1] += 1
    return rec


def amax_slots(device, n):
    if n > _AMAX_SLOTS:
        return torch.zeros((n, AMAX_RECORD_FLOATS), dtype=torch.float32, device=device)
    ent = _amax_pool.get(device)
    if ent is not None and ent[1] + n > _AMAX_SLOTS:
        ent[1] = _AMAX_SLOTS
    first = amax_slot(device)
    ent = _amax_pool[device]
    i0 = ent[1] - 1
    ent[1] = i0 + n
    return ent[0][i0:i0 + n]


def reset_amax_pool():
    _amax_pool.clear()


def tag_amax(t, rec):
    return leave(t, "amax", rec)


def amax_of(t):
    return take(t, "amax")


def carry_amax(dst, src):
    rec = amax_of(src)
    if rec is not None:
        tag_amax(dst, rec)
    return dst


def amax_fused(desc, which):
    return bool(_lib.lib().otgan_conv2d_amax_fused(ctypes.byref(desc), which))


def shared_x_operand(desc, device):
    nbytes = _lib.lib().otgan_conv2d_operand_bytes(ctypes.byref(desc))
    if not nbytes:
        return None
    buf = torch.empty((nbytes + 3) // 4, dtype=torch.float32, device=device)
    desc.x_operand = buf.data_ptr()
    return buf


def prepare_filters(desc, which, w, **fields):
    L = _lib.lib()
    fields.setdefault("w_amax", amax_of(w))
    desc = launch_desc(desc, **fields)
    nbytes = L.otgan_conv2d_filter_bytes(ctypes.byref(desc), which)
    if not nbytes:
        return None
    buf = torch.empty((nbytes + 3) // 4, dtype=torch.float32, device=w.device)
    raw = take(w, "raw")
    if raw is not None:
        _lib.check(L.otgan_conv2d_prepare_filters_raw_f32(ctypes.byref(desc), which, raw.data_ptr(), w.data_ptr(),
                                                          buf.data_ptr(), buf.numel() * 4, _lib.stream_ptr()),
                   "prepare_filters_raw")
        return buf
    _lib.check(L.otgan_conv2d_prepare_filters_f32(ctypes.byref(desc), which, w.data_ptr(), buf.data_ptr(),
                                                  buf.numel() * 4, _lib.stream_ptr()), "prepare_filters")
    return buf


def conv_wgrad_raw(desc, x, cmap, dy, dw, **fields):
    L = _lib.lib()
    desc = launch_desc(desc, **fields)
    need = L.otgan_conv2d_workspace_bytes(ctypes.byref(desc), 2)
    ws = workspace(need, dy.device)
    _lib.check(L.otgan_conv2d_wgrad_f32(ctypes.byref(desc), x.data_ptr(), _lib.ptr(cmap),
                                        dy.data_ptr(), dw.data_ptr(), ws.data_ptr(), ws.numel(),
                                        _lib.stream_ptr()), "conv2d_wgrad")


def fold_weights(desc, w):
    nfold = _lib.lib().otgan_conv2d_folded_weight_elems(ctypes.byref(desc))
    weff = torch.empty(nfold, dtype=w.dtype, device=w.device)
    weffT = torch.empty(nfold, dtype=w.dtype, device=w.device)
    _lib.check(_lib.lib().otgan_conv2d_fold_weights_f32(ctypes.byref(desc), w.data_ptr(), weff.data_ptr(),
                                                        weffT.data_ptr(), _lib.stream_ptr()), "fold_weights")
    return weff, weffT


SIDE_STREAM = None
_SIDE_SEEN = set()


def join_side_stream(tensors=()):
    _SIDE_SEEN.clear()
    if SIDE_STREAM is None:
        return
    cur = torch.cuda.current_stream()
    cur.wait_stream(SIDE_STREAM)
    for t in tensors:
        if t is not None and t.is_cuda:
            t.record_stream(cur)


_PENDING_GLU = [None]


def _drop_unclaimed_glu():
    ref = _PENDING_GLU[0]
    if ref is not None:
        t = ref()
        if t is not None:
            take(t, "glu", remove=True)
        _PENDING_GLU[0] = None


SIGN_TRACE = None


def _trace_signs(x):
    if SIGN_TRACE is not None:
        SIGN_TRACE.append((x.detach() > 0).cpu())


class Conv2dFunction(torch.autograd.Function):

    @staticmethod
    def forward(ctx, x, V, g, b, stride, upsample, preact, segs, glu_hint=False, grow=0):
        _need_cuda(x, V, g, b)
        _drop_unclaimed_glu()
        x = x.contiguous()
        if preact in (1, 4):
            _trace_signs(x)
        N, H, W, C = x.shape
        KH, KW, Cin_eff, Cout = V.shape if V.dim() == 4 else (1, 1) + tuple(V.shape)
        if Cin_eff != C * (2 if preact in DOUBLED else 1):
            raise ValueError(f"weight expects {Cin_eff} effective input channels, input gives "
                             f"{C * (2 if preact in DOUBLED else 1)}")
        V2d = V.contiguous().view(KH * KW * Cin_eff, Cout)
        OH, OW = out_hw(H, W, upsample, stride)
        grow = int(grow) if (grow and Cout % 4 == 0 and not glu_hint and _GROW_IN_PLACE) else 0
        if grow:
            full = torch.empty((N, OH, OW, Cout + grow), dtype=x.dtype, device=x.device)
            full._otgan_grow = True
            y = full[..., :Cout]
        else:
            y = torch.empty((N, OH, OW, Cout), dtype=x.dtype, device=x.device)
        desc = make_desc(x, C, upsample, KH, KW, stride, Cout, Cout + grow, 0, preact,
                         segs if (segs and not upsample) else None)
        cmap, inv = channel_maps(segs if (segs and not upsample) else (C,), preact, x.device)
        nfold = _lib.lib().otgan_conv2d_folded_weight_elems(ctypes.byref(desc))

        def has(which):
            return _lib.lib().otgan_conv2d_filter_bytes(ctypes.byref(desc), which) > 0

        unf_f = bool(nfold) and has(2)
        unf_b = bool(nfold) and has(3)
        raw_ok = (FILTERS_FROM_RAW and cmap is None and ((unf_f and unf_b) if nfold else (has(0) and has(1))) and
                  all(t is None or t.data_ptr() % 16 == 0 for t in (x, V2d, b)))

        def compute(raw=raw_ok):
            if raw:
                scale, inv_norm = weightnorm_scale(V2d, g)
                return scale, scale, inv_norm, {"fwd": prepare_filters(desc, 2 if nfold else 0, scale), "bwd": None,
                                                "bwd_done": False, "bwd_which": 3 if nfold else 1, "raw": scale}
            w, wT, inv_norm = weightnorm_fwd(V2d, g)
            wd = w
            if nfold and not (unf_f and unf_b):
                wd_f, wT_f = fold_weights(desc, w)
                if not unf_b:
                    wd = wd_f
                if not unf_f:
                    wT = wT_f
            return wd, wT, inv_norm, {"fwd": prepare_filters(desc, 2 if unf_f else 0, wT), "bwd": None,
                                      "bwd_done": False, "bwd_which": 3 if unf_b else 1}

        wd, wT, inv_norm, filt = cached_weights(V, g, compute)
        if "raw" in filt and not raw_ok:
            wd, wT, inv_norm, filt = compute(False)
        ctx.w_rec = amax_of(wT)
        ctx.x_rec = None
        if filt["fwd"] is not None and x.is_contiguous() and C % 4 == 0:
            ctx.x_rec = amax_of(x)
            if ctx.x_rec is None:
                ctx.x_rec = absmax_record(x)
        fwd = launch_desc(desc, w_amax=ctx.w_rec, x_amax=ctx.x_rec if ctx.x_rec is not None else amax_of(x))
        ctx.x_op = None
        if (ctx.needs_input_grad[1] or ctx.needs_input_grad[2]) and cmap is None and filt["fwd"] is not None:
            ctx.x_op = shared_x_operand(fwd, x.device)
        y_rec = y_glu = glu_rec = None
        if amax_fused(fwd, 0):
            y_rec = amax_slot(x.device)
        if glu_hint and cmap is None and _lib.lib().otgan_conv2d_glu_fused(ctypes.byref(fwd)):
            y_glu = torch.empty((N, OH, OW, Cout // 2), dtype=x.dtype, device=x.device)
            glu_rec = amax_slot(x.device)
        conv_fwd_raw(fwd, x, cmap, V2d if "raw" in filt else wT, b, y, filt["fwd"], y_amax_out=y_rec, glu_out=y_glu,
                     glu_amax_out=glu_rec)
        if y_glu is not None:
            leave(y, "glu", tag_amax(y_glu, glu_rec))
            _PENDING_GLU[0] = weakref.ref(y)
        if y_rec is not None:
            tag_amax(y, y_rec)
        if (SIDE_STREAM is not None and ctx.needs_input_grad[0] and not filt["bwd_done"] and
                _lib.lib().otgan_conv2d_filter_bytes(ctypes.byref(desc), filt["bwd_which"]) > 0):
            cur = torch.cuda.current_stream()
            SIDE_STREAM.wait_stream(cur)
            with torch.cuda.stream(SIDE_STREAM):
                filt["bwd"], filt["bwd_done"] = prepare_filters(desc, filt["bwd_which"], wd), True
                filt["bwd_event"] = SIDE_STREAM.record_event()
            wd.record_stream(SIDE_STREAM)
        ctx.save_for_backward(x, V2d, g, wd, inv_norm)
        ctx.filt = filt
        ctx.desc, ctx.cmap, ctx.inv = desc, cmap, inv
        ctx.vshape = V.shape
        ctx.has_b = b is not None
        return y

    @staticmethod
    def backward(ctx, dy):
        x, V2d, g, w, inv_norm = ctx.saved_tensors
        ld = channel_prefix_stride(dy)
        if ld is None:
            dy = carry_amax(dy.contiguous(), dy)
            if "raw" in ctx.filt and dy.data_ptr() % 16:
                dy = carry_amax(dy.clone(), dy)
            ld = dy.shape[-1]
        dx = dV = dg = db = None
        dy_rec = None
        if ctx.x_rec is not None and dy.shape[-1] % 4 == 0:
            dy_rec = amax_of(dy)
            if dy_rec is None:
                dy_rec = (absmax_record(dy) if dy.is_contiguous() else
                          absmax_record_strided(dy.data_ptr(), dy.numel() // dy.shape[-1], dy.shape[-1], ld, dy.device))
        desc = launch_desc(ctx.desc, ldy=ld, w_amax=ctx.w_rec, x_amax=ctx.x_rec, x_operand=ctx.x_op, dy_amax=dy_rec)
        if ctx.needs_input_grad[0]:
            dx = torch.empty_like(x)
            filt = ctx.filt
            if "raw" in filt:
                src, w = filt["raw"], V2d
            else:
                src = w
            if not filt["bwd_done"]:
                filt["bwd"], filt["bwd_done"] = prepare_filters(desc, filt["bwd_which"], src), True
            elif filt.get("bwd_event") is not None:
                torch.cuda.current_stream().wait_event(filt["bwd_event"])
                if filt["bwd"] is not None:
                    filt["bwd"].record_stream(torch.cuda.current_stream())
            dx_rec = None
            if amax_fused(desc, 1) and (ctx.inv is None or filt["bwd"] is None):
                dx_rec = amax_slot(x.device)
            conv_dgrad_raw(desc, dy, w, x, ctx.inv, dx, x.shape[3], False, filt["bwd"], dx_amax_out=dx_rec)
            if dx_rec is not None:
                tag_amax(dx, dx_rec)
        need_w = ctx.needs_input_grad[1] or ctx.needs_input_grad[2]
        need_b = ctx.has_b and ctx.needs_input_grad[3]
        side = SIDE_STREAM if (need_w or need_b) else None
        if side is not None:
            side.wait_stream(torch.cuda.current_stream())
            for t in (dy, x, ctx.x_op, dy_rec, ctx.x_rec):
                if t is not None:
                    t.record_stream(side)
        with (torch.cuda.stream(side) if side is not None else _NULL_CTX):
            if need_w:
                dw = torch.empty_like(V2d)
                conv_wgrad_raw(desc, x, ctx.cmap, dy, dw)
                dV2d, dg = weightnorm_bwd(V2d, g, inv_norm, dw)
                dV = dV2d.view(ctx.vshape)
            if need_b:
                db = colsum_of(dy)
                if db is None:
                    rows = dy.numel() // dy.shape[-1]
                    db = colsum(dy.data_ptr(), rows, dy.shape[-1], ld, dy.device)
        if side is not None:
            key = V2d.untyped_storage().data_ptr() + V2d.storage_offset()
            if key in _SIDE_SEEN:
                torch.cuda.current_stream().wait_stream(side)
            _SIDE_SEEN.add(key)
        return dx, dV, dg, db, None, None, None, None, None, None


def conv2d_op(x, V, g, b, stride=1, upsample=False, preact=0, segs=None, glu_hint=False, grow=0):
    return Conv2dFunction.apply(x, V, g, b, int(stride), bool(upsample), int(preact),
                                tuple(segs) if segs else None, bool(glu_hint), int(grow))


def channel_prefix_stride(t):
    if t.dim() != 4 or t.is_contiguous():
        return None
    N, H, W, C = t.shape
    ld = t.stride(2)
    if (t.stride(3) != 1 or ld < C or ld % 4 or C % 4 or t.stride(1) != W * ld or t.stride(0) != H * W * ld
            or t.data_ptr() % 16):
        return None
    return int(ld)


def grown_buffer(x, Ctot, claim=False):
    base = x._base if x.dim() == 4 else None
    if base is None or not getattr(base, "_otgan_grow", False) or not base.is_contiguous():
        return None
    N, H, W, C = x.shape
    if tuple(base.shape) != (N, H, W, Ctot) or x.data_ptr() != base.data_ptr() or channel_prefix_stride(x) != Ctot:
        return None
    if claim:
        base._otgan_grow = False
    return base


def dense_op(x, V, g, b, preact=0, segs=None):
    N, C = x.shape
    y = Conv2dFunction.apply(x.view(N, 1, 1, C), V, g, b, 1, False,
                             int(preact), tuple(segs) if segs else None)
    return y.view(N, -1)


def absmax_record_strided(t_ptr, rows, C, ld, device):
    rec = torch.empty(AMAX_RECORD_FLOATS, dtype=torch.float32, device=device)
    _lib.check(_lib.lib().otgan_absmax_f32(t_ptr, rows, C, ld, rec.data_ptr(), _lib.stream_ptr()), "absmax")
    return rec


def _input_row_order(segs0, preact, device):
    segs0 = tuple(int(c) for c in segs0)
    if preact not in DOUBLED or len(segs0) <= 1:
        return None
    key = ("rows", segs0, device)
    hit = _map_cache.get(key)
    if hit is None:
        pos, neg, off = [], [], 0
        for c in segs0:
            pos += [2 * off + i for i in range(c)]
            neg += [2 * off + c + i for i in range(c)]
            off += c
        hit = torch.tensor(pos + neg, dtype=torch.int64, device=device)
        _map_cache[key] = hit
    return hit


def _aligned16(*ts):
    return all(t is None or t.data_ptr() % 16 == 0 for t in ts)


def weightnorm_fwd_block(V2ds, gs):
    L = len(V2ds)
    Ks = [int(v.shape[0]) for v in V2ds]
    dev, dt = V2ds[0].device, V2ds[0].dtype
    w_all = torch.empty(sum(Ks) * 16, dtype=dt, device=dev)
    wT_all = torch.empty(sum(Ks) * 16, dtype=dt, device=dev)
    inv_all = torch.empty(L * 16, dtype=dt, device=dev)
    arr = (WnFwdLayer * L)()
    out, off = [], 0
    wp, tp, ip = w_all.data_ptr(), wT_all.data_ptr(), inv_all.data_ptr()
    for k in range(L):
        n = Ks[k] * 16
        a = arr[k]
        a.V, a.g, a.K = V2ds[k].data_ptr(), gs[k].data_ptr(), Ks[k]
        a.w, a.wT, a.inv = wp + 4 * off, tp + 4 * off, ip + 64 * k
        out.append((w_all[off:off + n].view(Ks[k], 16), wT_all[off:off + n].view(16, Ks[k]), inv_all[16 * k:16 * k + 16]))
        off += n
    _lib.check(_lib.lib().otgan_weightnorm_fwd_batched16_f32(arr, L, _lib.stream_ptr()), "weightnorm_fwd_batched")
    return out


def weightnorm_bwd_block(V2ds, gs, invs, parts):
    L = len(V2ds)
    Ks = [int(v.shape[0]) for v in V2ds]
    dev, dt = V2ds[0].device, V2ds[0].dtype
    dV_all = torch.empty(sum(Ks) * 16, dtype=dt, device=dev)
    dg_all = torch.empty(L * 16, dtype=dt, device=dev)
    arr = (WnBwdLayer * L)()
    dVs, dgs, off = [], [], 0
    vp, gp = dV_all.data_ptr(), dg_all.data_ptr()
    for k in range(L):
        n = Ks[k] * 16
        a = arr[k]
        a.V, a.g, a.inv = V2ds[k].data_ptr(), gs[k].data_ptr(), invs[k].data_ptr()
        a.dV, a.dg = vp + 4 * off, gp + 64 * k
        a.taps = 9
        a.Ceff = Ks[k] // 9
        for i, (ptr, perm, nrows, rstride) in enumerate(parts[k]):
            q = a.part[i]
            q.p, q.perm, q.nrows, q.rstride = ptr, (perm.data_ptr() if perm is not None else None), nrows, rstride
        dVs.append(dV_all[off:off + n].view(Ks[k], 16))
        dgs.append(dg_all[16 * k:16 * k + 16])
        off += n
    _lib.check(_lib.lib().otgan_weightnorm_bwd_batched16_f32(arr, L, _lib.stream_ptr()), "weightnorm_bwd_batched")
    return dVs, dgs


def _row_order_back(order):
    if order is None:
        return None
    key = ("back", order.data_ptr())
    hit = _map_cache.get(key)
    if hit is None:
        back = torch.empty_like(order)
        back[order] = torch.arange(order.numel(), device=order.device)
        hit = (order, back.to(torch.int32))
        _map_cache[key] = hit
    return hit[1]


_block_cache = OrderedDict()
DENSE16_MAX_BATCH = 16
DENSE16_MAX_CHAIN = 17


def _wide_operands(per_layer, layers, row0, nrows, order, F, desc):
    layers = list(layers)
    nl = len(layers)
    n = nl * F
    ref = per_layer[layers[0]][0]
    w = torch.empty((9 * nrows, n), dtype=ref.dtype, device=ref.device)
    wT = torch.empty((n, 9 * nrows), dtype=ref.dtype, device=ref.device)
    map32 = None
    if order is not None:
        key = ("rows32", order.data_ptr())
        hit = _map_cache.get(key)
        if hit is None:
            hit = (order, order.to(torch.int32))
            _map_cache[key] = hit
        map32 = hit[1]
    segs_w, segs_t = [], []
    for j, k in enumerate(layers):
        w_k, wT_k = per_layer[k][0], per_layer[k][1]
        assert w_k.is_contiguous() and wT_k.is_contiguous()
        ceff = w_k.shape[0] // 9
        assert row0 + nrows <= ceff
        segs_w.append((w_k.data_ptr(), w.data_ptr() + 4 * j * F, 9, ceff * F, F, nrows * n, n))
        segs_t.append((wT_k.data_ptr(), wT.data_ptr() + 4 * j * F * 9 * nrows, F * 9, ceff, 1, nrows, 1))
    rec = amax_slot(ref.device)
    gather3d_batched(segs_w, nrows, F, row0, map32, rec)
    gather3d_batched(segs_t, nrows, 1, row0, map32)
    tag_amax(w, rec)
    tag_amax(wT, rec)
    return {"w": w, "wT": wT, "fwd": prepare_filters(desc, 0, wT), "bwd": None, "bwd_done": False}


def _split_block_weights(Vs, per_layer, plan, F):
    key = id(Vs[0])
    ws = [pl[0] for pl in per_layer]
    hit = _block_cache.get(key)
    cut = plan["key"][1:]
    if hit is not None and len(hit[0]) == len(ws) and all(a is b for a, b in zip(hit[0], ws)) and hit[2] == cut:
        _block_cache.move_to_end(key)
        return hit[1]
    L = len(per_layer)
    val = {"wide": [_wide_operands(per_layer, range(wd["d0"], L), wd["row0"], wd["nrows"], wd["order"], F, wd["desc"])
                    for wd in plan["wide"]],
           "w_g": [None] * L, "wT_g": [None] * L}
    own = [k for k in range(L) if plan["own_len"][k]]
    if own:
        dev, dt = per_layer[own[0]][0].device, per_layer[own[0]][0].dtype
        sizes = [9 * (per_layer[k][0].shape[0] // 9 - plan["own_row0"][k]) * F for k in own]
        flat_w = torch.empty(sum(sizes), dtype=dt, device=dev)
        flat_wT = torch.empty(sum(sizes), dtype=dt, device=dev)
        segs, off = [], 0
        for k, sz in zip(own, sizes):
            r0 = plan["own_row0"][k]
            ceff = per_layer[k][0].shape[0] // 9
            n_own = ceff - r0
            w_k, wT_k = per_layer[k][0], per_layer[k][1]
            assert w_k.is_contiguous() and wT_k.is_contiguous()
            val["w_g"][k] = flat_w[off:off + sz].view(9 * n_own, F)
            val["wT_g"][k] = flat_wT[off:off + sz].view(F, 9 * n_own)
            segs.append((w_k.data_ptr() + 4 * r0 * F, val["w_g"][k].data_ptr(), 9, n_own * F, ceff * F, n_own * F))
            segs.append((wT_k.data_ptr() + 4 * r0, val["wT_g"][k].data_ptr(), 9 * F, n_own, ceff, n_own))
            off += sz
        copy2d_batched(segs)
        val["_own_flat"] = (flat_w, flat_wT)
        val["h2"] = [None] * L
        if plan.get("h2"):
            lib = _lib.lib()
            nsl = [plan["own_len"][k] for k in own]
            fbytes = [int(lib.otgan_dense16_filter_bytes(n)) for n in nsl]
            flat_q = torch.empty(sum(fbytes), dtype=torch.uint8, device=dev)
            off = 0
            for k, nb in zip(own, fbytes):
                val["h2"][k] = flat_q[off:off + nb]
                off += nb
            n = len(own)
            pw = (ctypes.c_void_p * n)(*[val["wT_g"][k].data_ptr() for k in own])
            pn = (ctypes.c_int * n)(*nsl)
            pf = (ctypes.c_void_p * n)(*[val["h2"][k].data_ptr() for k in own])
            _lib.check(lib.otgan_dense16_prepare_filters_f32(ctypes.cast(pw, ctypes.c_void_p), ctypes.cast(pn, ctypes.c_void_p),
                                                              ctypes.cast(pf, ctypes.c_void_p), n, _lib.stream_ptr()),
                       "dense16_prepare_filters")
            val["_h2_flat"] = flat_q
    _block_cache[key] = (ws, val, cut)
    while len(_block_cache) > 64:
        _block_cache.popitem(last=False)
    return val


def _split_block_plan(N, H, W, C0, L, F, segs0, preact, device):
    if not DENSE_SPLIT or F != 16 or L < 2 or any(int(c) % 4 for c in segs0):
        return None
    mult = 2 if preact in DOUBLED else 1
    Ctot = C0 + L * F
    lib = _lib.lib()
    desc_in = ConvDesc(N, H, W, C0, Ctot, 0, 3, 3, 1, L * F, Ctot, C0, preact, 1)
    if not lib.otgan_conv2d_filter_bytes(ctypes.byref(desc_in), 0):
        return None
    wide = [{"desc": desc_in, "x_off": 0, "C": C0, "d0": 0, "row0": 0, "nrows": C0 * mult,
             "order": _input_row_order(segs0, preact, device), "accumulate": 0, "after": -1}]
    group = (L + 1) // 2 if DENSE_GROUP is None else int(DENSE_GROUP)
    g0 = [0] * L
    for s0 in range(0, L, group) if group > 0 else ():
        s1 = min(s0 + group, L)
        if s1 >= L:
            break
        n = s1 - s0
        desc = ConvDesc(N, H, W, n * F, Ctot, 0, 3, 3, 1, (L - s1) * F, Ctot, C0 + s1 * F, preact, 1)
        if not lib.otgan_conv2d_filter_bytes(ctypes.byref(desc), 0):
            break
        wide.append({"desc": desc, "x_off": C0 + s0 * F, "C": n * F, "d0": s1, "row0": (C0 + s0 * F) * mult,
                     "nrows": n * F * mult, "order": _input_row_order((F,) * n, preact, device), "accumulate": 1,
                     "after": s1 - 1})
        for k in range(s1, L):
            g0[k] = s1
    for wd in wide:
        wd["back"] = _row_order_back(wd["order"])
    probe = ConvDesc(N, H, W, F, Ctot, 0, 3, 3, 1, F, Ctot, C0, preact, 1)
    probe.list_width = F
    h2 = bool(lib.otgan_dense16_h2_ok(ctypes.byref(launch_desc(probe, y_accumulate=1)))) and (W != 64 or DENSE_H2_AT_64)
    own_len = [k - g0[k] for k in range(L)]
    starts = sorted({wd["d0"] for wd in wide}) + [L]
    if sum(1 for n in own_len if n) > DENSE16_MAX_BATCH or max(b - a for a, b in zip(starts[:-1], starts[1:])) > DENSE16_MAX_CHAIN:
        h2 = False
    return {"wide": wide, "g0": g0, "own_len": own_len, "h2": h2,
            "own_row0": [(C0 + g0[k] * F) * mult for k in range(L)],
            "key": (N, H, W, C0, L, F, tuple(segs0), preact, tuple(g0), h2)}


def _calibrate_backward_arg_refs():
    seen = []

    class _Probe(torch.autograd.Function):
        @staticmethod
        def forward(ctx, x):
            return x * 2

        @staticmethod
        def backward(ctx, dy):
            seen.append(sys.getrefcount(dy))
            return dy

    with torch.enable_grad():
        x = torch.zeros(2, requires_grad=True)
        (_Probe.apply(x) * 3).sum().backward()
    return seen[0]


_BACKWARD_ARG_REFS = _calibrate_backward_arg_refs()
_GROW_IN_PLACE = True


class DenseBlockFunction(torch.autograd.Function):

    @staticmethod
    def forward(ctx, x0, segs0, ksize, preact, *params):
        _need_cuda(x0)
        L = len(params) // 3
        N, H, W, C0 = x0.shape
        F = params[0].shape[-1]
        Ctot = C0 + L * F
        buf = grown_buffer(x0, Ctot, claim=True)
        if buf is None:
            buf = torch.empty((N, H, W, Ctot), dtype=x0.dtype, device=x0.device)
            buf[..., :C0].copy_(x0)
# ... 243 lines not shown


def _block_input_grad(G, C0):
    v = G[..., :C0]
    return v if channel_prefix_stride(v) is not None else v.contiguous()


def _dense16_bwd_filters(sw, plan, L, F, device):
    hit = sw.get("h2_bwd")
    if hit is not None:
        return hit
    from ._lib_layers import Dense16BwdPair
    lib = _lib.lib()
    starts = [wd["d0"] for wd in plan["wide"]] + [L]
    gend = {}
    for a, b in zip(starts[:-1], starts[1:]):
        for c in range(a, b):
            gend[c] = b
    nsl = {c: gend[c] - 1 - c for c in range(L) if gend[c] - 1 - c >= 1}
    sizes = {c: int(lib.otgan_dense16_bwd_filter_bytes(n)) for c, n in nsl.items()}
    flat = torch.empty(sum(sizes.values()), dtype=torch.uint8, device=device)
    out, off, pairs = {}, 0, []
    for c in sorted(nsl):
        out[c] = flat[off:off + sizes[c]]
        off += sizes[c]
        for j in range(nsl[c]):
            k = c + 1 + j
            pairs.append(Dense16BwdPair(sw["w_g"][k].data_ptr(), sw["h2"][k].data_ptr(), out[c].data_ptr(),
                                        plan["own_len"][k], c - plan["g0"][k], j))
    allf = [sw["h2"][k] for k in range(L) if sw["h2"][k] is not None]
    if pairs:
        arr = (Dense16BwdPair * len(pairs))(*pairs)
        pf = (ctypes.c_void_p * len(allf))(*[t.data_ptr() for t in allf])
        _lib.check(lib.otgan_dense16_prepare_bwd_filters_f32(ctypes.cast(arr, ctypes.c_void_p), len(pairs),
                                                              ctypes.cast(pf, ctypes.c_void_p), len(allf), _lib.stream_ptr()),
                   "dense16_prepare_bwd_filters")
    res = {"flat": flat, "slice": out, "nsl": nsl}
    sw["h2_bwd"] = res
    return res


def _backward_by_slice(ctx, buf, saved, G, dbuf, need_w):
    L, C0, F = ctx.L, ctx.C0, ctx.F
    N, H, W, Ctot = buf.shape
    plan, sw = ctx.plan, ctx.sw
    lib = _lib.lib()
    grads = [None] * (3 * L)
    dw_g = [None] * L
    wides = plan["wide"]
    dw_wide = [None] * len(wides)
    bw = _dense16_bwd_filters(sw, plan, L, F, buf.device)
    tag = amax_of(dbuf)
    RR = amax_slots(buf.device, L + 1)
    RS, Rc = RR[:L], RR[L]
    Rc.copy_(tag if tag is not None else absmax_record(G))
    R0 = amax_slot(buf.device)
    ctx.dx0_rec = R0
    gptr, bptr = G.data_ptr(), buf.data_ptr()
    side = SIDE_STREAM if need_w else None
    if side is not None:
        for t in [G, buf, RR, R0, ctx.fwd_recs[0]] + [t for t in ctx.x_ops if t is not None]:
            t.record_stream(side)

    def wgrad_stream():
        if side is None:
            return _NULL_CTX
        side.wait_stream(torch.cuda.current_stream())
        return torch.cuda.stream(side)

    def wide_bwd(i, need_dx):
        d0 = wides[i]["d0"]
        dw_wide[i] = _wide_bwd(ctx, buf, G, i, need_w, need_dx, (RR[d0], L + 1 - d0), Rc if i > 0 else R0, wgrad_stream)

    starts = [wd["d0"] for wd in wides] + [L]
    for gi in reversed(range(len(wides))):
        d0, d1 = starts[gi], starts[gi + 1]
        if gi + 1 < len(wides):
            wide_bwd(gi + 1, True)
        if d1 - d0 >= 2:
            pf = (ctypes.c_void_p * (d1 - d0 - 1))(*[bw["slice"][c].data_ptr() for c in range(d0, d1 - 1)])
            off0 = 4 * (C0 + d0 * F)
            _lib.check(lib.otgan_dense16_chain_bwd_f32(N, H, W, d1 - d0, gptr + off0, Ctot, bptr + off0, Ctot,
                                                       ctypes.cast(pf, ctypes.c_void_p), Rc.data_ptr(), RS[d0].data_ptr(),
                                                       _lib.stream_ptr()), "dense16_chain_bwd")
        for c in reversed(range(d0, d1)):
            if need_w and plan["own_len"][c]:
                desc = ctx.descs[c]
                cmap, _inv = ctx.maps[c]
                off = C0 + plan["g0"][c] * F
                R, gbase, gidx = ctx.fwd_recs
                with wgrad_stream():
                    dw_g[c] = torch.empty_like(sw["w_g"][c])
                    conv_wgrad_raw(desc, buf[..., off:], cmap, G, dw_g[c], dy_amax=(RR[c], L + 1 - c),
                                   x_amax=(R[gbase[gidx[plan["g0"][c]]]], 1 + plan["own_len"][c]))
    wide_bwd(0, ctx.needs_input_grad[0])
    if need_w:
        assert ctx.batched and len(wides) <= 2
        with wgrad_stream():
            _block_weight_grads(ctx, saved, grads, dw_g, dw_wide)
            _block_bias_grads(ctx, G, grads)
    return grads


def dense_block_op(x0, segs0, params, ksize=3, preact=1):
    flat = [t for p in params for t in p]
    return DenseBlockFunction.apply(x0, tuple(segs0), int(ksize), int(preact), *flat)


class GluFunction(torch.autograd.Function):

    @staticmethod
    def forward(ctx, x):
        _need_cuda(x)
        x = x.contiguous()
        C2 = x.shape[-1]
        rows = x.numel() // C2
        pre = take(x, "glu", remove=True)
        if pre is not None:
            _PENDING_GLU[0] = None
            ctx.save_for_backward(x)
            return pre
        y = torch.empty(x.shape[:-1] + (C2 // 2,), dtype=x.dtype, device=x.device)
        rec = amax_slot(x.device) if (C2 // 2) % 4 == 0 and _aligned16(x, y) else None
        _lib.check(_lib.lib().otgan_glu_fwd_amax_f32(x.data_ptr(), rows, C2 // 2, y.data_ptr(), _lib.ptr(rec),
                                                     _lib.stream_ptr()), "glu_fwd")
        if rec is not None:
            tag_amax(y, rec)
        ctx.save_for_backward(x)
        return y

    @staticmethod
    def backward(ctx, dy):
        (x,) = ctx.saved_tensors
        dy = dy.contiguous()
        C2 = x.shape[-1]
        dx = torch.empty_like(x)
        if (C2 // 2) % 4 == 0 and _aligned16(x, dy, dx):
            rec = amax_slot(x.device)
            cs = torch.empty(C2, dtype=x.dtype, device=x.device)
            scratch = torch.empty(256 * C2, dtype=x.dtype, device=x.device)
            _lib.check(_lib.lib().otgan_glu_bwd_colsum_f32(x.data_ptr(), dy.data_ptr(), x.numel() // C2, C2 // 2,
                                                           dx.data_ptr(), rec.data_ptr(), cs.data_ptr(), scratch.data_ptr(),
                                                           _lib.stream_ptr()), "glu_bwd_colsum")
            leave(dx, "colsum", cs)
            tag_amax(dx, rec)
        else:
            _lib.check(_lib.lib().otgan_glu_bwd_amax_f32(x.data_ptr(), dy.data_ptr(), x.numel() // C2,
                                                         C2 // 2, dx.data_ptr(), None, _lib.stream_ptr()), "glu_bwd")
        return dx


class TanhFunction(torch.autograd.Function):
    @staticmethod
    def forward(ctx, x):
        _need_cuda(x)
        x = x.contiguous()
        y = torch.empty_like(x)
        _lib.check(_lib.lib().otgan_tanh_fwd_f32(x.data_ptr(), x.numel(), y.data_ptr(),
                                                 _lib.stream_ptr()), "tanh_fwd")
        ctx.save_for_backward(y)
        return y

    @staticmethod
    def backward(ctx, dy):
        (y,) = ctx.saved_tensors
        dy = dy.contiguous()
        dx = torch.empty_like(y)
        _lib.check(_lib.lib().otgan_tanh_bwd_f32(y.data_ptr(), dy.data_ptr(), y.numel(),
                                                 dx.data_ptr(), _lib.stream_ptr()), "tanh_bwd")
        return dx


class FeatureHeadFunction(torch.autograd.Function):

    @staticmethod
    def forward(ctx, x):
        _need_cuda(x)
        x = x.contiguous()
        _trace_signs(x)
        N, H, W, C = x.shape
        f = torch.empty((N, H * W * 2 * C), dtype=x.dtype, device=x.device)
        norm = torch.empty(N, dtype=x.dtype, device=x.device)
        _lib.check(_lib.lib().otgan_feature_head_fwd_f32(x.data_ptr(), N, H * W, C, f.data_ptr(),
                                                         norm.data_ptr(), _lib.stream_ptr()), "head_fwd")
        ctx.save_for_backward(x, f, norm)
        return f

    @staticmethod
    def backward(ctx, df):
        x, f, norm = ctx.saved_tensors
        df = df.contiguous()
        N, H, W, C = x.shape
        dx = torch.empty_like(x)
        rec = amax_slot(x.device) if C % 4 == 0 else None
        _lib.check(_lib.lib().otgan_feature_head_bwd_amax_f32(x.data_ptr(), f.data_ptr(), norm.data_ptr(),
                                                              df.data_ptr(), N, H * W, C, dx.data_ptr(), _lib.ptr(rec),
                                                              _lib.stream_ptr()), "head_bwd")
        if rec is not None:
            tag_amax(dx, rec)
        return dx


class ConcatChannelsFunction(torch.autograd.Function):

    @staticmethod
    def forward(ctx, *xs):
        ctx.widths = [int(t.shape[-1]) for t in xs]
        y = torch.cat(xs, 3)
        if all(w % 4 == 0 for w in ctx.widths) and any(amax_of(t) is not None for t in xs):
            recs = [amax_of(t) if amax_of(t) is not None else absmax_record(t.contiguous()) for t in xs]
            rec = recs[0]
            for r in recs[1:]:
                rec = torch.maximum(rec, r)
            tag_amax(y, rec)
        return y

    @staticmethod
    def backward(ctx, dy):
        rec = amax_of(dy)
        outs = []
        for piece in dy.split(ctx.widths, 3):
            piece = piece.contiguous()
            if rec is not None:
                tag_amax(piece, rec)
            outs.append(piece)
        return tuple(outs)


def concat_channels(xs):
    return ConcatChannelsFunction.apply(*xs)


class ExtendChannelsFunction(torch.autograd.Function):

    @staticmethod
    def forward(ctx, Ctot, x, *others):
        base = grown_buffer(x, Ctot)
        assert base is not None
        ctx.widths = [int(t.shape[-1]) for t in (x,) + others]
        rec = amax_of(x) if all(w % 4 == 0 for w in ctx.widths) else None
        if rec is not None:
            for t in others:
                r = amax_of(t)
                rec = torch.maximum(rec, r if r is not None else absmax_record(t.contiguous()))
        off = ctx.widths[0]
        for t in others:
            base[..., off:off + t.shape[-1]].copy_(t)
            off += t.shape[-1]
        y = base[..., :off]
        if rec is not None:
            tag_amax(y, rec)
        return y

    @staticmethod
    def backward(ctx, dy):
        rec = amax_of(dy)
        outs, off = [], 0
        for i, w in enumerate(ctx.widths):
            piece = dy[..., off:off + w]
            off += w
            if not ctx.needs_input_grad[1 + i]:
                outs.append(None)
                continue
            if i > 0 or channel_prefix_stride(piece) is None:
                piece = piece.contiguous()
            if rec is not None:
                tag_amax(piece, rec)
            outs.append(piece)
        return (None, *outs)


def extend_channels(xs, Ctot):
    if grown_buffer(xs[0], Ctot) is None or any(t.shape[:3] != xs[0].shape[:3] for t in xs[1:]):
        return None
    return ExtendChannelsFunction.apply(int(Ctot), *xs)


glu = GluFunction.apply
tanh = TanhFunction.apply
feature_head = FeatureHeadFunction.apply


def adam_step(p, grad, v, mg, lr, mom1, mom2, t, coef=None):
    bump_weights_epoch(p)
    _lib.check(_lib.lib().otgan_adam_step_coef_f32(p.data_ptr(), grad.data_ptr(), _lib.ptr(v), mg.data_ptr(),
                                                   p.numel(), float(lr), float(mom1), float(mom2),
                                                   float(t), _lib.ptr(coef), _lib.stream_ptr()), "adam_step")


ADAM_MAX_SEGMENTS = 32


def adam_coefficients(mom1, mom2, t):
    out = (ctypes.c_float * 2)()
    _lib.lib().otgan_adam_coefficients(float(mom1), float(mom2), float(t), ctypes.cast(out, ctypes.c_void_p))
    return float(out[0]), float(out[1])


def adam_step_gather(p_flat, grads, offsets, v, mg, lr, mom1, mom2, t, ema_shadow=None, ema_decay=0.0, coef=None):
    n = len(grads)
    bump_weights_epoch(p_flat)
    if ema_shadow is not None:
        bump_weights_epoch(ema_shadow)
    gp = (ctypes.c_void_p * n)(*[g.data_ptr() for g in grads])
    off = (ctypes.c_long * (n + 1))(*offsets)
    _lib.check(_lib.lib().otgan_adam_step_gather_coef_f32(p_flat.data_ptr(), ctypes.cast(gp, ctypes.c_void_p),
                                                          ctypes.cast(off, ctypes.c_void_p), n, _lib.ptr(v), mg.data_ptr(),
                                                          float(lr), float(mom1), float(mom2), float(t), _lib.ptr(coef),
                                                          _lib.ptr(ema_shadow), float(ema_decay), _lib.stream_ptr()),
               "adam_step_gather")


COPY2D_MAX_SEGMENTS = 64


def copy2d_batched(segs):
    for i0 in range(0, len(segs), COPY2D_MAX_SEGMENTS):
        part = segs[i0:i0 + COPY2D_MAX_SEGMENTS]
        n = len(part)
        src = (ctypes.c_void_p * n)(*[q[0] for q in part])
        dst = (ctypes.c_void_p * n)(*[q[1] for q in part])
        rows = (ctypes.c_int * n)(*[q[2] for q in part])
        cols = (ctypes.c_int * n)(*[q[3] for q in part])
        sld = (ctypes.c_long * n)(*[q[4] for q in part])
        dld = (ctypes.c_long * n)(*[q[5] for q in part])
        cast = lambda a: ctypes.cast(a, ctypes.c_void_p)
        _lib.check(_lib.lib().otgan_copy2d_batched_f32(cast(src), cast(dst), cast(rows), cast(cols), cast(sld), cast(dld), n,
                                                       _lib.stream_ptr()), "copy2d_batched")


GATHER3D_MAX_SEGMENTS = 32


def gather3d_batched(segs, n1, n2, base1=0, map1=None, amax_out=None):
    assert map1 is None or (map1.dtype == torch.int32 and map1.numel() == n1 and map1.is_contiguous())
    assert amax_out is None or len(segs) <= GATHER3D_MAX_SEGMENTS
    for i0 in range(0, len(segs), GATHER3D_MAX_SEGMENTS):
        part = segs[i0:i0 + GATHER3D_MAX_SEGMENTS]
        n = len(part)
        cast = lambda a: ctypes.cast(a, ctypes.c_void_p)
        arr = lambda ty, i: cast((ty * n)(*[q[i] for q in part]))
        _lib.check(_lib.lib().otgan_gather3d_batched_f32(arr(ctypes.c_void_p, 0), arr(ctypes.c_void_p, 1), arr(ctypes.c_int, 2),
                                                         int(n1), int(n2), arr(ctypes.c_long, 3), arr(ctypes.c_long, 4),
                                                         arr(ctypes.c_long, 5), arr(ctypes.c_long, 6), int(base1),
                                                         _lib.ptr(map1), _lib.ptr(amax_out), n, _lib.stream_ptr()),
                   "gather3d_batched")


def adamax_step(p, grad, v, mg, lr, mom1, mom2):
    bump_weights_epoch(p)
    _lib.check(_lib.lib().otgan_adamax_step_f32(p.data_ptr(), grad.data_ptr(), _lib.ptr(v),
                                                mg.data_ptr(), p.numel(), float(lr), float(mom1),
                                                float(mom2), _lib.stream_ptr()), "adamax_step")


def nesterov_step(p, grad, v, lr, mom1):
    bump_weights_epoch(p)
    _lib.check(_lib.lib().otgan_nesterov_step_f32(p.data_ptr(), grad.data_ptr(), v.data_ptr(),
                                                  p.numel(), float(lr), float(mom1),
                                                  _lib.stream_ptr()), "nesterov_step")


def ema_update(shadow, p, decay):
    bump_weights_epoch(shadow)
    _lib.check(_lib.lib().otgan_ema_update_f32(shadow.data_ptr(), p.data_ptr(), p.numel(),
                                               float(decay), _lib.stream_ptr()), "ema_update")


BATCH_U8_MAX_SHARDS = 32


def batch_from_u8(store, offsets, B, S, lut, perm=None, flip=None, out=None):
    if not (store.is_cuda and store.dtype == torch.uint8 and store.dim() == 4 and store.shape[3] == 3 and store.is_contiguous()):
        raise _lib.OtganError("batch_from_u8 takes a contiguous CUDA (MI355X) uint8 [n, H, W, 3] store; there is no CPU fallback")
    rows = len(offsets) * int(B)
    if out is None:
        out = torch.empty(rows, S, S, 3, dtype=torch.float32, device=store.device)
    if not (out.dtype == torch.float32 and out.shape == (rows, S, S, 3) and out[:1].is_contiguous() and out.device == store.device):
        raise _lib.OtganError("batch_from_u8: out must be float32 [%d, %d, %d, 3] on %s with contiguous images, found %s %s on %s"
                              % (rows, S, S, store.device, out.dtype, tuple(out.shape), out.device))
    if perm is not None and not (perm.dtype == torch.int32 and perm.dim() == 1 and perm.is_contiguous()
                                 and perm.device == store.device):
        raise _lib.OtganError("batch_from_u8: perm must be a contiguous 1-D int32 tensor on %s, found %s %s on %s"
                              % (store.device, perm.dtype, tuple(perm.shape), perm.device))
    if flip is not None:
        if flip.dtype == torch.bool and flip.is_contiguous():
            flip = flip.view(torch.uint8)
        if not (flip.dtype == torch.uint8 and flip.numel() == rows and flip.is_contiguous() and flip.device == store.device):
            raise _lib.OtganError("batch_from_u8: flip must be %d contiguous bool / uint8 values on %s, found %s %s on %s"
                                  % (rows, store.device, flip.dtype, tuple(flip.shape), flip.device))
    if not (lut.dtype == torch.float32 and lut.numel() == 256 and lut.is_contiguous() and lut.device == store.device):
        raise _lib.OtganError("batch_from_u8: lut must be 256 contiguous float32 values on %s, found %s %s on %s"
                              % (store.device, lut.dtype, tuple(lut.shape), lut.device))
    off = (ctypes.c_long * len(offsets))(*[int(o) for o in offsets])
    with torch.cuda.device(store.device):
        _lib.check(_lib.lib().otgan_batch_from_u8_f32(store.data_ptr(), store.shape[0], store.shape[1], store.shape[2],
                                                      _lib.ptr(perm), perm.numel() if perm is not None else 0,
                                                      ctypes.cast(off, ctypes.c_void_p), len(offsets), int(B), _lib.ptr(flip),
                                                      lut.data_ptr(), int(S), out.data_ptr(), out.stride(0) if rows > 1 else 3 * S * S,
                                                      _lib.stream_ptr()), "batch_from_u8")
    return out


AUG_COLOR, AUG_TRANSLATION, AUG_CUTOUT = 1, 2, 4


def _augment_launch(fn, name, src, u, policy):
    _need_cuda(src, u)
    src = src.contiguous()
    if not (src.dtype == torch.float32 and src.dim() == 4 and src.shape[1] == src.shape[2] and src.shape[3] == 3):
        raise _lib.OtganError("%s takes float32 [rows, S, S, 3] images, found %s %s" % (name, src.dtype, tuple(src.shape)))
    rows, S = src.shape[0], src.shape[1]
    if not (u.dtype == torch.float32 and tuple(u.shape) == (rows, 8) and u.is_contiguous() and u.device == src.device):
        raise _lib.OtganError("%s: u must be contiguous float32 [%d, 8] on %s, found %s %s on %s"
                              % (name, rows, src.device, u.dtype, tuple(u.shape), u.device))
    out = torch.empty_like(src)
    with torch.cuda.device(src.device):
        _lib.check(fn(src.data_ptr(), rows, S, u.data_ptr(), int(policy), out.data_ptr(), _lib.stream_ptr()), name)
    return out


class AugmentFunction(torch.autograd.Function):

    @staticmethod
    def forward(ctx, x, u, policy):
        ctx.policy = int(policy)
        ctx.save_for_backward(u)
        return _augment_launch(_lib.lib().otgan_augment_fwd_f32, "augment_fwd", x, u, policy)

    @staticmethod
    def backward(ctx, dy):
        (u,) = ctx.saved_tensors
        return augment_transpose(dy, u, ctx.policy), None, None


def augment(x, u, policy):
    return AugmentFunction.apply(x, u, policy)


def augment_transpose(dy, u, policy):
    return _augment_launch(_lib.lib().otgan_augment_bwd_f32, "augment_bwd", dy, u, policy)
```

### ot-gan_amd/trainer.py

```python
import importlib
import os

import torch

from . import parallel
from .utils import augment, matching, nn


def _lib_prof_on():
    from . import _lib
    return _lib.prof_enabled()


class _frozen:

    def __init__(self, params):
        self.params = [p for p in params if p.requires_grad]

    def __enter__(self):
        for p in self.params:
            p.requires_grad_(False)

    def __exit__(self, *exc):
        for p in self.params:
            p.requires_grad_(True)
        return False


class _Region:
    __slots__ = ("pairs", "e0")

    def __init__(self, pairs):
        self.pairs = pairs

    def __enter__(self):
        self.e0 = torch.cuda.Event(enable_timing=True)
        self.e0.record()

    def __exit__(self, *exc):
        e1 = torch.cuda.Event(enable_timing=True)
        e1.record()
        self.pairs.append((self.e0, e1))
        return False


class _NoRegion:
    def __enter__(self):
        return None

    def __exit__(self, *exc):
        return False


_NO_REGION = _NoRegion()


class OTGAN:

    def __init__(self, args, device, init_batch=None):
        self.args = args
        self.device = device
        self.rank, self.world = parallel.get_rank(), parallel.world_size()
        if args.nr_gpu % 2 != 0:
            raise AssertionError("nr_gpu must be even (train.py:34)")
        if args.nr_gpu % self.world != 0:
            raise ValueError("--nr_gpu (logical shards) must be a multiple of the number of ranks")
        self.shards = args.nr_gpu // self.world
        self.scope = getattr(args, "matching_scope", "global")
        if self.world == 1:
            self.scope = "local"
        if self.scope == "global" and self.world % 2 != 0:
            raise ValueError(f"global matching scope needs an even number of ranks (got {self.world}): with an odd "
                             "count one rank's shards straddle the two mini-batch halves; use --matching_scope local")
        self.collectives = not parallel._skip_collectives()
        if self.scope == "local" and self.shards % 2 != 0:
            raise ValueError("local matching needs an even number of shards per rank")
        self.nb = self.shards * args.batch_size
        self.aug_policy = augment.parse_policy(getattr(args, "augment", ""))
        mod = importlib.import_module(f".models.{args.model}", package=__package__)
        self.generator, self.discriminator = mod.generator, mod.discriminator
        self.generator.reset(seed=args.seed, device=device)
        self.discriminator.reset(seed=args.seed, device=device)
        self.model_opts = {"nonlinearity": args.nonlinearity}
        size = getattr(args, "image_size", 32)
        if size != 32:
            if args.model == "densenet":
                mod.check_image_size(size)
            elif args.model != "dcgan":
                raise ValueError(f"--model {args.model} takes --image_size 32 only (dcgan and densenet also take 64)")
            self.model_opts["image_size"] = size
        ddi = bool(getattr(args, "data_dependent_init", False))
        if ddi and init_batch is None:
            raise ValueError("--data_dependent_init needs an initial data batch (OTGAN(args, device, init_batch=...))")
        nn.data_dependent_init(ddi)
        try:
            with torch.no_grad():
                x0 = init_batch.to(device) if ddi else torch.zeros(2, size, size, 3, device=device)
                f = self.discriminator(x0, init=True, **self.model_opts)
                self.generator(batch_size=x0.shape[0], init=True, device=device, **self.model_opts)
        finally:
            nn.data_dependent_init(False)
        self.num_features = f.shape[-1]
        groups = (self.discriminator.flatten(), self.generator.flatten())
        if ddi and self.world > 1:
            from . import ops
            for grp in groups:
                parallel.broadcast_(grp.flat, src=0)
            ops.bump_weights_epoch()
        self.disc_params = self.discriminator.trainable_variables()
        self.gen_params = self.generator.trainable_variables()
        self.ema = nn.ExponentialMovingAverage(decay=0.999)
        self.maintain_averages = self.ema.apply(self.gen_params)
        mk = {"adam": nn.adam_updates, "adamax": nn.adamax_updates, "nesterov": nn.nesterov_updates}
        if args.optimizer not in mk:
            raise ValueError("unsupported optimizer")
        kw = {"mom1": 0.5} if args.optimizer == "nesterov" else {"mom1": 0.5, "mom2": 0.999}
        if self.collectives:
            parallel.resolve_collectives_mode(device)
        self.collectives_mode = parallel.collectives_mode() if self.collectives else "none"
        side_ok = os.environ.get("OTGAN_SIDE_STREAM", "1") != "0"
        overlap = self.collectives and self.collectives_mode == "overlapped"
        self.disc_buckets = parallel.GradBuckets(self.disc_params) if overlap else None
        self.gen_buckets = parallel.GradBuckets(self.gen_params) if overlap else None
        self.gen_optimizer = mk[args.optimizer](self.gen_params, **kw)
        self.disc_optimizer = mk[args.optimizer](self.disc_params, **kw)
        self.ema_fused = self.gen_optimizer.fuse_ema(self.ema)
        self.step_counter = 0
        self.last = {}
        import collections
        self._max_ahead = 2
        self._step_ends, self._free_events = collections.deque(), []
        self.timers = None
        self._d_weights_in_graph = False
        on = side_ok
        self.fork_real_pass = self.fork_wgrad = on
        self._side_stream = torch.cuda.Stream(device=device) if on else None
        env = os.environ.get("OTGAN_STEP_GRAPH")
        asked = getattr(args, "step_graph", None)
        want = (env == "1") if env in ("0", "1") else (args.model == "densenet" if asked is None else bool(asked))
        self.graphs = GraphedSteps(self) if (want and not self.collectives and self.world == 1) else None

    def enable_timers(self, on=True):
        self.timers = {} if on else None
        if on and self.graphs is not None:
            self.graphs.drop("region timers need the eager step")
            self.graphs = None

    def _timed(self, name):
        if self.timers is None:
            return _NO_REGION
        return _Region(self.timers.setdefault(name, []))

    def collect_timers(self, steps):
        torch.cuda.synchronize()
        out = {}
        for name, pairs in (self.timers or {}).items():
            out[name + "_ms"] = round(sum(a.elapsed_time(b) for a, b in pairs) / max(1, steps), 4)
        if "match_total_ms" in out:
            out["matching_ms"] = round(out.pop("match_total_ms") - out.get("allgather_in_match_ms", 0.0), 4)
        out["allgather_ms"] = round(out.pop("allgather_in_match_ms", 0.0) + out.pop("allgather_early_ms", 0.0), 4)
        self.timers = {} if self.timers is not None else None
        return out

    def sinkhorn_rows(self):
        S = self.args.nr_gpu if (self.scope == "global" and self.world > 1) else self.shards
        return S * self.args.batch_size if self.args.single_batch else (S // 2) * self.args.batch_size

    def _match(self, f_gen, f_dat, pending_dat=None, need_dat=True):
        a = self.args
        plain = not (a.single_batch or a.no_sinkhorn)
        if self.scope == "global" and self.world > 1:
            S = self.world * self.shards
            with self._timed("allgather_in_match"):
                allg = parallel.all_gather_rows(f_gen)
                alld = pending_dat.wait() if pending_dat is not None else parallel.all_gather_rows(f_dat)
            if plain:
                if rank_stack_ok(self.nb, allg):
                    g_gen, g_dat, ent, dist = rank_matching_stack(self.rank, self.world, self.nb, allg, alld, a.sinkhorn_lambda,
                                                                  a.nr_sinkhorn_iter, need_dat, self._gather_slices)
                    return g_gen, g_dat, dist, ent
                K = self._sharded_log_kernels(f_gen, f_dat, allg, alld)
                g_gen, g_dat, ent, dist = matching.matched_feature_grads(
                    allg, alld, a.sinkhorn_lambda, a.nr_sinkhorn_iter, need_b=need_dat,
                    rows=(self.rank * self.nb, self.nb), log_kernels=K)
                return g_gen, g_dat, dist, ent
            if a.single_batch:
                K = self._sharded_single_log_kernels(f_gen, f_dat, allg, alld)
                g_gen, g_dat, ent, dist = matching.matched_feature_grads_single_batch(
                    allg, alld, a.sinkhorn_lambda, a.nr_sinkhorn_iter, need_b=need_dat,
                    rows=(self.rank * self.nb, self.nb), log_kernels=K)
                return g_gen, g_dat, dist, ent
            fa, fb = list(torch.chunk(allg, S, 0)), list(torch.chunk(alld, S, 0))
        else:
            if pending_dat is not None:
                f_dat = pending_dat.wait()
            if plain:
                g_gen, g_dat, ent, dist = matching.matched_feature_grads(
                    f_gen, f_dat, a.sinkhorn_lambda, a.nr_sinkhorn_iter, need_b=need_dat)
                return g_gen, g_dat, dist, ent
            if a.single_batch:
                g_gen, g_dat, ent, dist = matching.matched_feature_grads_single_batch(
                    f_gen, f_dat, a.sinkhorn_lambda, a.nr_sinkhorn_iter, need_b=need_dat)
                return g_gen, g_dat, dist, ent
            fa = list(torch.chunk(f_gen, self.shards, 0))
            fb = list(torch.chunk(f_dat, self.shards, 0))
        if a.single_batch:
            m = matching.get_matched_features_single_batch(fa, fb, a.sinkhorn_lambda, a.nr_sinkhorn_iter)
        else:
            m = matching.get_matched_features_random(fa, fb)
        dist = m.distance if m.distance is not None else matching.calc_distance(fa, fb, m)
        lo = self.rank * self.shards if (self.scope == "global" and self.world > 1) else 0
        pick = lambda lst: torch.cat(lst[lo:lo + self.shards], 0)
        grad_gen = pick(m[0]) - pick(m[2])
        grad_dat = pick(m[1]) - pick(m[3])
        return grad_gen, grad_dat, dist, m[4]

    def _gather_slices(self, mine):
        with self._timed("allgather_in_match"):
            return parallel.all_gather_rows(mine.unsqueeze(0))

    def _sharded_log_kernels(self, f_gen, f_dat, fa, fb):
        mine = rank_log_kernel_slices(self.rank, self.world, f_gen, f_dat, fa, fb, self.args.sinkhorn_lambda)
        with self._timed("allgather_in_match"):
            allk = parallel.all_gather_rows(mine.unsqueeze(0))
        return assemble_log_kernels(allk, self.world)

    def _sharded_single_log_kernels(self, f_gen, f_dat, allg, alld):
        mine = rank_single_log_kernel_slices(f_gen, f_dat, allg, alld, self.args.sinkhorn_lambda)
        with self._timed("allgather_in_match"):
            allk = parallel.all_gather_rows(mine.unsqueeze(0))
        return assemble_single_log_kernels(allk, self.args.sinkhorn_lambda)

    def step(self, x_data, noise=None, aug=None, apply_updates=True):
        assert x_data.shape[0] == self.nb
        period = self.args.nr_gen_per_disc + 1
        phase = self.step_counter % period
        kind = "disc" if phase == 0 else "gen"
        self._throttle()
        if self.graphs is not None and noise is None and aug is None and apply_updates:
            done = self.graphs.run(x_data, phase)
            if done is not None:
                self.last = done
                self._mark_step_end()
                return self.last
        from . import ops
        ops.SIDE_STREAM = self._side_stream if self.fork_wgrad else None
        try:
            dist, ent, grads = self._step_body(x_data, kind, noise, apply_updates, aug)
        finally:
            ops.SIDE_STREAM = None
        self._mark_step_end()
        self._d_weights_in_graph = False
        self.step_counter += 1
        self.last = {"kind": kind, "distance": dist, "entropy": ent}
        if not apply_updates:
            self.last["grads"] = grads
        return self.last

    def _throttle(self):
        if self._max_ahead > 0 and len(self._step_ends) >= self._max_ahead:
            ev = self._step_ends.popleft()
            ev.synchronize()
            self._free_events.append(ev)

    def _mark_step_end(self):
        if self._max_ahead > 0:
            ev = self._free_events.pop() if self._free_events else torch.cuda.Event()
            ev.record()
            self._step_ends.append(ev)
            if len(self._step_ends) > self._max_ahead:
                self._free_events.append(self._step_ends.popleft())

    def _optimise(self, opt, grads, lr, critic):
        opt(grads, lr=lr)
        if not critic and not self.ema_fused:
            self.maintain_averages()

    def _backward(self, outputs, params, grad_outputs):
        from . import ops
        grads = torch.autograd.grad(outputs, params, grad_outputs)
        if self.fork_wgrad:
            ops.join_side_stream(grads)
        return grads

    def prepare_step_graphs(self, x_data):
        if self.graphs is None:
            return 0
        period = self.args.nr_gen_per_disc + 1
        kinds = {self.graphs._kind(p) for p in range(period)}
        n = 0
        while self.graphs is not None and self.graphs.dead is None and set(self.graphs.graphs) != kinds and n < 3 * period + 2:
            self.step(x_data)
            n += 1
        return n

    def _step_body(self, x_data, kind, noise=None, apply_updates=True, aug=None):
        a = self.args
        T = None
        if self.aug_policy:
            from . import ops
            u = aug if aug is not None else augment.draw(2 * self.nb, self.device)
            assert tuple(u.shape) == (2 * self.nb, augment.SLOTS), "aug: [2 * nb, 8] uniforms"
            T = lambda x, rows: ops.augment(x, u[rows], self.aug_policy)
        real, fake, both = slice(0, self.nb), slice(self.nb, 2 * self.nb), slice(0, 2 * self.nb)
        gkw = dict(self.model_opts)
        if noise is not None:
            gkw["noise"] = noise
        if kind == "disc":
            with torch.no_grad():
                ema = self.ema if a.train_disc_against_ema else None
                x_gen = self.generator(batch_size=self.nb, ema=ema, device=self.device, **gkw)
            x_all = torch.cat([x_data, x_gen], 0)
            f_all = self.discriminator(x_all if T is None else T(x_all, both), **self.model_opts)
            f_dat, f_gen = f_all[:self.nb], f_all[self.nb:]
            with self._timed("match_total"):
                g_gen, g_dat, dist, ent = self._match(f_gen.detach(), f_dat.detach())
            if self.disc_buckets is not None:
                self.disc_buckets.arm()
            grads = self._backward(f_all, self.disc_params, torch.cat([g_dat, g_gen], 0))
            with self._timed("allreduce"):
                grads = (self.disc_buckets.finish() if self.disc_buckets is not None
                         else parallel.allreduce_sum_(list(grads)))
            if apply_updates:
                self._optimise(self.disc_optimizer, grads, -a.learning_rate_disc, critic=True)
        else:
            side = self._side_stream if self.fork_real_pass else None
            if side is not None:
                main = torch.cuda.current_stream()
                side.wait_stream(main)
                with torch.cuda.stream(side), torch.no_grad():
                    f_dat = self.discriminator(x_data if T is None else T(x_data, real), **self.model_opts)
                    pending = None
                    if self.collectives_mode == "overlapped" and (self.scope == "global" or self.world == 1):
                        with self._timed("allgather_early"):
                            pending = parallel.all_gather_rows_async(f_dat)
                f_dat.record_stream(main)
                x_gen = self.generator(batch_size=self.nb, device=self.device, **gkw)
                main.wait_stream(side)
            else:
                with torch.no_grad():
                    f_dat = self.discriminator(x_data if T is None else T(x_data, real), **self.model_opts)
                with self._timed("allgather_early"):
                    pending = (parallel.all_gather_rows_async(f_dat)
                               if self.collectives and (self.scope == "global" or self.world == 1) else None)
                x_gen = self.generator(batch_size=self.nb, device=self.device, **gkw)
            with _frozen(self.disc_params):
                f_gen = self.discriminator(x_gen if T is None else T(x_gen, fake), **self.model_opts)
            with self._timed("match_total"):
                g_gen, _g_dat, dist, ent = self._match(f_gen.detach(), f_dat, pending, need_dat=False)
            if self.gen_buckets is not None:
                self.gen_buckets.arm()
            grads = self._backward(f_gen, self.gen_params, g_gen)
            with self._timed("allreduce"):
                grads = (self.gen_buckets.finish() if self.gen_buckets is not None
                         else parallel.allreduce_sum_(list(grads)))
            if apply_updates:
                self._optimise(self.gen_optimizer, grads, a.learning_rate_gen, critic=False)
        return dist, ent, grads

    @torch.no_grad()
    def sample(self, n, ema=False):
        return self.generator(batch_size=n, ema=self.ema if ema else None, device=self.device, **self.model_opts)

    PROBE_BATCH = 500

    @torch.no_grad()
    def critic_features(self, x):
        from . import ops
        f = self.discriminator(x, **self.model_opts).float()
        if self.graphs is not None and self._d_weights_in_graph and self.graphs.critic_ops is not None:
            ops.reinstate_weights(self.graphs.critic_ops)
        return f

    def state_dict(self, full=True):
        sd = {"step_counter": self.step_counter}
        for t in (self.discriminator, self.generator):
            sd.update({k: v.detach().cpu() for k, v in t.named_variables().items()})
        if full:
            sd["__optim__"] = {"gen": self.gen_optimizer.state_dict(), "disc": self.disc_optimizer.state_dict()}
            names = list(self.generator.named_variables())
            sd["__ema__"] = {n: self.ema.average(p).detach().cpu() for n, p in zip(names, self.gen_params)}
        return sd

    def load_state_dict(self, sd):
        from . import ops
        moments = lambda: [id(t) for o in (self.gen_optimizer, self.disc_optimizer) for st in getattr(o, "state", ())
                           for t in st.values() if t is not None]
        before = moments()
        with torch.no_grad():
            for t in (self.discriminator, self.generator):
                for k, v in t.named_variables().items():
                    v.copy_(sd[k].to(v.device))
            names = list(self.generator.named_variables())
            ema = sd.get("__ema__")
            for n, p in zip(names, self.gen_params):
                src = ema[n].to(p.device) if ema is not None else p.detach()
                self.ema.average(p).copy_(src)
        opt = sd.get("__optim__")
        if opt is not None:
            self.gen_optimizer.load_state_dict(opt["gen"])
            self.disc_optimizer.load_state_dict(opt["disc"])
        ops.bump_weights_epoch()
        self.step_counter = int(sd.get("step_counter", 0))
        if self.graphs is not None:
            if moments() != before:
                self.graphs.drop("checkpoint loaded (the optimisers' moment buffers are new tensors)", recapture=True)
            else:
                self._d_weights_in_graph = False

    def check_finite(self):
        for k in ("distance", "entropy"):
            v = self.last.get(k)
            if v is not None and not bool(torch.isfinite(v)):
                raise FloatingPointError(f"non-finite matching {k} in step {self.step_counter - 1}: the Sinkhorn "
                                         "kernel failed (device shared / partitioned?) or the model diverged")

    def close(self):
        for b in (self.disc_buckets, self.gen_buckets):
            if b is not None:
                b.remove()
        self.disc_buckets = self.gen_buckets = None
        from . import ops
        streams = [self._side_stream]
        if self.graphs is not None:
            streams.append(self.graphs.stream)
            self.graphs.drop("trainer closed")
            self.graphs = None
        for t in (self.disc_params[0], self.gen_params[0], self.ema.average(self.gen_params[0])):
            ops.forget_weights(t)
        for s in streams:
            if s is not None:
                ops.forget_stream(s)
                matching.forget_stream(s)


class GraphedSteps:

    def __init__(self, model):
        self.m = model
        self.graphs = {}
        self.x = None
        self.stream = None
        self.warm = 0
        self.dead = None
        self.critic_ops = None

    def drop(self, why, recapture=False):
        self.graphs = {}
        self.critic_ops = None
        self.m._d_weights_in_graph = False
        self.warm = 0
        if not recapture:
            self.dead = why

    def _kind(self, phase):
        return "disc" if phase == 0 else ("gen1" if phase == 1 else "gen")

    def run(self, x_data, phase):
        from . import ops
        m = self.m
        period = m.args.nr_gen_per_disc + 1
        if self.dead is not None or _lib_prof_on():
            return None
        if self.warm < period:
            self.warm += 1
            return None
        kind = self._kind(phase)
        if kind not in self.graphs:
            if kind != "gen1" and period > 1 and not m._d_weights_in_graph:
                return None
            try:
                self._capture(x_data, kind)
            except Exception as e:
                import warnings
                warnings.warn(f"otgan_amd: step graph capture failed ({type(e).__name__}: {e}); continuing with eager steps")
                self.drop(f"capture failed: {e}")
                return None
        elif kind != "gen1" and period > 1 and not m._d_weights_in_graph:
            return None
        g, dist, ent = self.graphs[kind]
        opt = m.disc_optimizer if kind == "disc" else m.gen_optimizer
        self.x.copy_(x_data)
        if getattr(opt, "coef_dev", None) is not None:
            opt.write_coefficients()
        g.replay()
        opt.t += 1.0
        m.step_counter += 1
        m._d_weights_in_graph = kind != "disc"
        self._bump_written(kind)
        if kind == "gen1" and self.critic_ops is not None:
            ops.reinstate_weights(self.critic_ops)
        return {"kind": "disc" if kind == "disc" else "gen", "distance": dist, "entropy": ent}

    def _bump_written(self, kind):
        m = self.m
        ts = list(m.disc_params if kind == "disc" else m.gen_params)
        if kind != "disc":
            ts += [m.ema.average(p) for p in m.gen_params]
        self._bump(ts)

    @staticmethod
    def _bump(ts):
        from . import ops
        seen = set()
        for t in ts:
            key = t.untyped_storage().data_ptr()
            if key not in seen:
                seen.add(key)
                ops.bump_weights_epoch(t)

    def _capture(self, x_data, kind):
        from . import ops
        m = self.m
        if self.x is None:
            self.x = torch.empty_like(x_data)
            self.stream = torch.cuda.Stream(device=m.device)
        for opt in (m.gen_optimizer, m.disc_optimizer):
            if hasattr(opt, "ensure_state"):
                opt.ensure_state()
                if opt.coef_dev is None:
                    opt.coef_dev = torch.ones(2, dtype=torch.float32, device=m.device)
        self.x.copy_(x_data)
        ts = list(m.gen_params) + [m.ema.average(p) for p in m.gen_params]
        if kind == "gen1":
            ts += list(m.disc_params)
        self._bump(ts)
        saved_t = (m.gen_optimizer.t, m.disc_optimizer.t)
        ops.reset_amax_pool()
        g = torch.cuda.CUDAGraph()
        try:
            m.gen_optimizer.capturing = m.disc_optimizer.capturing = True
            ops.SIDE_STREAM = m._side_stream if m.fork_wgrad else None
            with torch.cuda.graph(g, stream=self.stream):
                try:
                    dist, ent, _ = m._step_body(self.x, "disc" if kind == "disc" else "gen")
                except BaseException:
                    if ops.SIDE_STREAM is not None:
                        torch.cuda.current_stream().wait_stream(ops.SIDE_STREAM)
                    raise
        finally:
            ops.SIDE_STREAM = None
            m.gen_optimizer.capturing = m.disc_optimizer.capturing = False
            m.gen_optimizer.t, m.disc_optimizer.t = saved_t
            ops.reset_amax_pool()
            ops.forget_side_events()
        self.graphs[kind] = (g, dist, ent)
        if kind == "gen1":
            self.critic_ops = ops.weights_in(m.disc_params[0])


def rank_log_kernel_slices(rank, world, f_gen, f_dat, fa, fb, lam):
    def halves(f):
        if torch.is_tensor(f):
            return f[:f.shape[0] // 2], f[f.shape[0] // 2:]
        return torch.cat(f[:len(f) // 2], 0), torch.cat(f[len(f) // 2:], 0)
    a2 = halves(fa)[1]
    b1, b2 = halves(fb)
    if rank < world // 2:
        return matching.cost_log_kernels([f_gen, f_gen, f_gen], [a2, b1, b2], lam)
    return matching.cost_log_kernels([f_dat, f_gen, f_gen], [b1, b1, b2], lam)


def rank_stack_ok(nb, allg):
    N, D = allg.shape[0] // 2, allg.shape[1]
    return nb >= 256 and nb % 32 == 0 and N % nb == 0 and matching.FeatureStack.supported(N, D)


def rank_matching_stack(rank, world, nb, allg, alld, lam, iters, need_dat, gather=None):
    N = allg.shape[0] // 2
    ranges, own_gen, own_dat = matching.FeatureStack.rank_plan(rank * nb, nb, N, need_dat)
    st = matching.FeatureStack(allg, alld, ranges)
    if rank < world // 2:
        mine = st.cost_slices([own_gen] * 3, [3 * N, N, 2 * N], nb, lam)
    else:
        mine = st.cost_slices([own_dat, own_gen, own_gen], [N, N, 2 * N], nb, lam)
    allk = gather(mine) if callable(gather) else gather
    K = assemble_log_kernels(allk, world)
    return st.rows_grad(lam, iters, (rank * nb, nb), K, need_b=need_dat)


def rank_single_log_kernel_slices(f_gen, f_dat, allg, alld, lam):
    return matching.cost_log_kernels([f_gen, f_dat, f_gen], [allg, alld, alld], lam)


def assemble_single_log_kernels(allk, lam):
    n = allk.shape[3]
    K = allk.permute(1, 0, 2, 3).reshape(3, n, n).contiguous()
    K[0].diagonal().add_(-float(lam) * 999.0)
    K[1].diagonal().add_(-float(lam) * 999.0)
    return K


_ASSEMBLE_IDX = {}


def assemble_log_kernels(allk, world):
    W2 = world // 2
    N = allk.shape[3]
    key = (allk.device, "assemble")
    idx = _ASSEMBLE_IDX.get(key)
    if idx is None:
        idx = (torch.tensor([0, 1, 0, 0, 1, 1], device=allk.device), torch.tensor([0, 0, 1, 2, 1, 2], device=allk.device))
        _ASSEMBLE_IDX[key] = idx
    a5 = allk.reshape(2, W2, 3, allk.shape[2], N)
    return a5[idx[0], :, idx[1]].reshape(6, N, N)


def default_args(**over):
    import argparse
    d = dict(seed=1, batch_size=625, learning_rate_disc=0.0003, learning_rate_gen=0.0003,
             data_dir='/home/tim/data', save_dir='/local_home/tim/med_gan', optimizer='adam',
             nonlinearity='crelu', nr_gpu=8, nr_gen_per_disc=5, sinkhorn_lambda=500.,
             nr_sinkhorn_iter=500, single_batch=False, train_disc_against_ema=False, model='dcgan',
             load_params=False, model_name='med_gan_params-2399', no_sinkhorn=False,
             image_size=32, matching_scope='global', synthetic=False, max_steps=0, save_every=200,
             synthetic_size=50000, data_dependent_init=False, eval_every=100, eval_samples=50000,
             inception_model='', ranks=0, step_graph=None, fid_stats='', fid_real_samples=0, dataset='cifar10',
             data_on_device=False, kid_subsets=0, kid_subset_size=1000, kid_real_samples=0,
             pr_neighbours=0, pr_real_samples=0, probe_every=0, probe_neighbours=5, probe_train_samples=5000,
             probe_test_samples=1000, augment='')
    d.update(over)
    return argparse.Namespace(**d)


def smoke_step(device):
    args = default_args(batch_size=4, nr_gpu=2, nr_sinkhorn_iter=10, nr_gen_per_disc=1)
    m = OTGAN(args, device)
    x = torch.rand(m.nb, 32, 32, 3, device=device) * 2 - 1
    r0 = m.step(x)
    r1 = m.step(x)
    assert r0["kind"] == "disc" and r1["kind"] == "gen"
    for r in (r0, r1):
        assert torch.isfinite(r["distance"]).item() and torch.isfinite(r["entropy"]).item()
    print("smoke ok: train steps", float(r0["distance"]), float(r1["distance"]))
```

### ot-gan_amd/utils/nn.py

```python
import contextlib
import os
import threading
import weakref
from collections import OrderedDict

import torch

from .. import ops

_scope = threading.local()


def _stack():
    if not hasattr(_scope, "stack"):
        _scope.stack = []
    return _scope.stack


@contextlib.contextmanager
def arg_scope(funcs, **kwargs):
    _stack().append(({f.__name__ for f in funcs}, kwargs))
    try:
        yield
    finally:
# ... 46 lines not shown


class FlatGroup:

    _by_param = weakref.WeakValueDictionary()

    def __init__(self, params):
        order = [p for p in params if p.numel() % 4 == 0] + [p for p in params if p.numel() % 4 != 0]
        self.params = order
        self.total = sum(p.numel() for p in order)
        self.flat = torch.empty(self.total, dtype=order[0].dtype, device=order[0].device)
        off = 0
        with torch.no_grad():
            for p in order:
                n = p.numel()
                view = self.flat[off:off + n].view(p.shape)
                view.copy_(p)
                p.data = view
                off += n
        for p in order:
            FlatGroup._by_param[id(p)] = self

    @staticmethod
    def of(params):
        params = list(params)
        grp = FlatGroup._by_param.get(id(params[0])) if params else None
        if grp is None or len(params) != len(grp.params):
            return None
        ids = {id(p) for p in params}
        return grp if all(id(p) in ids for p in grp.params) else None

    def offsets(self):
        out, off = [], 0
        for p in self.params:
            out.append(off)
            off += p.numel()
        return out + [off]

    def in_buffer_order(self, tensors, params):
        pos = {id(p): i for i, p in enumerate(params)}
        return [tensors[pos[id(p)]].contiguous() for p in self.params]

    def flatten_like(self, tensors, params):
        pos = {id(p): i for i, p in enumerate(params)}
        return torch.cat([tensors[pos[id(p)]].reshape(-1) for p in self.params])

    def views_of(self, flat):
        out, off = {}, 0
        for p in self.params:
            out[id(p)] = flat[off:off + p.numel()].view(p.shape)
            off += p.numel()
        return out


_current = threading.local()


def _store():
    st = getattr(_current, "store", None)
    if st is None:
        raise RuntimeError("layers must be called inside a template (nn.make_template)")
    return st


class Template:

    def __init__(self, name, fn, seed=1):
        self.name = name
        self.fn = fn
        self.store = VariableStore(name, seed=seed)

    def __call__(self, *args, **kwargs):
        prev = getattr(_current, "store", None)
        _current.store = self.store
        try:
            return self.fn(*args, **kwargs)
        finally:
            _current.store = prev

    def trainable_variables(self):
        return list(self.store.vars.values())

    def named_variables(self):
        return OrderedDict(self.store.vars)

    def reset(self, seed=1, device=None):
        seen = set()
        for v in self.store.vars.values():
            key = v.untyped_storage().data_ptr()
            if key not in seen:
                seen.add(key)
                ops.forget_weights(v)
        self.store = VariableStore(self.name, device=device, seed=seed)

    def flatten(self):
        return FlatGroup(self.trainable_variables())


def make_template(name, fn, seed=1):
    return Template(name, fn, seed)


class ExponentialMovingAverage:

    def __init__(self, decay=0.999):
        self.decay = decay
        self._shadow = {}
        self._params = []

    def apply(self, params):
        params = list(params)
        grp = FlatGroup.of(params) if not self._params else None
        if grp is not None:
            self._flat = (grp.flat.detach().clone(), grp)
            self._shadow.update(grp.views_of(self._flat[0]))
            self._params.extend(params)
            return self.update
        for p in params:
            if id(p) not in self._shadow:
                self._shadow[id(p)] = p.detach().clone()
                self._params.append(p)
        return self.update

    def update(self):
        flat = getattr(self, "_flat", None)
        if flat is not None:
            ops.ema_update(flat[0], flat[1].flat, self.decay)
            return
        for p in self._params:
            ops.ema_update(self._shadow[id(p)], p.detach(), self.decay)

    def average(self, p):
        return self._shadow[id(p)]

    def state(self):
        return [self._shadow[id(p)] for p in self._params]


def get_var_maybe_avg(name, shape, kind, ema, device):
    v = _store().get(name, shape, kind, device)
    return ema.average(v) if ema is not None else v


def get_name(layer_name, counters):
    if layer_name not in counters:
        counters[layer_name] = 0
    name = f"{layer_name}_{counters[layer_name]}"
    counters[layer_name] += 1
    return name


def _as_list(x):
    if isinstance(x, tuple):
        return list(x)
    if not isinstance(x, list):
        return [x]
    return x


def _channels_eff(xs, pre_activation):
    c = sum(int(t.shape[-1]) for t in xs)
    return c * (2 if pre_activation in ("celu", "crelu") else 1), c


_DATA_INIT = [False]


def data_dependent_init(on=True):
    _DATA_INIT[0] = bool(on)


def _run_data_init(y0, g, b, init_scale):
    with torch.no_grad():
        flat = y0.reshape(-1, y0.shape[-1]).double()
        m = flat.mean(0)
        v = flat.var(0, unbiased=False)
        gi = init_scale / torch.sqrt(v)
        g.copy_(gi.to(g.dtype))
        b.copy_((-m * gi).to(b.dtype))
    ops.bump_weights_epoch()


@_scoped
def dense(x, num_units, pre_activation='celu', init_scale=1., counters={}, init=False, ema=None,
          weight_norm=True, use_b=True, use_g=True, **kwargs):
    if not (weight_norm and use_g and use_b):
        raise NotImplementedError("only the weight_norm=True, use_g=True, use_b=True layer of the "
                                  "reference models is implemented")
    name = get_name('dense', counters)
    xs = _as_list(x)
    nr_in, c = _channels_eff(xs, pre_activation)
    dev = xs[0].device
    V = get_var_maybe_avg(f"{name}/V", (nr_in, num_units), "normal", ema, dev)
    g = get_var_maybe_avg(f"{name}/g", (num_units,), "ones", ema, dev)
    b = get_var_maybe_avg(f"{name}/b", (num_units,), "zeros", ema, dev)
    xin = xs[0] if len(xs) == 1 else torch.cat(xs, 1)
    if init and _DATA_INIT[0] and ema is None:
        with torch.no_grad():
            y0 = ops.dense_op(xin, V, torch.ones_like(g), torch.zeros_like(b), preact=ops.ACT[pre_activation],
                              segs=[int(t.shape[-1]) for t in xs])
        _run_data_init(y0, g, b, init_scale)
    return ops.dense_op(xin, V, g, b, preact=ops.ACT[pre_activation], segs=[int(t.shape[-1]) for t in xs])


@_scoped
def conv2d(x, num_filters, pre_activation='celu', filter_size=[3, 3], stride=[1, 1], pad='SAME',
           dilate=1, upsample=False, init_scale=1., counters={}, init=False, ema=None,
           weight_norm=True, use_b=True, use_g=True, glu_hint=False, grow=0, **kwargs):
    if pad != 'SAME' or dilate != 1:
        raise NotImplementedError("the reference models only use pad='SAME', dilate=1")
    if not (weight_norm and use_g and use_b):
        raise NotImplementedError("only the weight_norm=True, use_g=True, use_b=True layer of the "
                                  "reference models is implemented")
    if stride[0] != stride[1]:
        raise NotImplementedError("square strides only")
    name = get_name('conv2d', counters)
    xs = _as_list(x)
    nr_in, c = _channels_eff(xs, pre_activation)
    dev = xs[0].device
    V = get_var_maybe_avg(f"{name}/V", (filter_size[0], filter_size[1], nr_in, num_filters), "normal", ema, dev)
    g = get_var_maybe_avg(f"{name}/g", (num_filters,), "ones", ema, dev)
    b = get_var_maybe_avg(f"{name}/b", (num_filters,), "zeros", ema, dev)
    if isinstance(xs, ConcatList) and xs.buffer is not None:
        xin = xs.buffer
    else:
        xin = xs[0] if len(xs) == 1 else torch.cat(xs, 3)
    if init and _DATA_INIT[0] and ema is None:
        with torch.no_grad():
            y0 = ops.conv2d_op(xin, V, torch.ones_like(g), torch.zeros_like(b), stride=stride[0], upsample=upsample,
                               preact=ops.ACT[pre_activation], segs=[int(t.shape[-1]) for t in xs])
        _run_data_init(y0, g, b, init_scale)
    return ops.conv2d_op(xin, V, g, b, stride=stride[0], upsample=upsample,
                         preact=ops.ACT[pre_activation], segs=[int(t.shape[-1]) for t in xs], glu_hint=glu_hint,
                         grow=grow)


class ConcatList(list):
    buffer = None


@_scoped
def dense_block(x, layers_per_block, filters_per_layer, pre_activation='celu', filter_size=[3, 3],
                counters={}, init=False, ema=None, weight_norm=True, **kwargs):
    xs = _as_list(x)
    if init and _DATA_INIT[0] and ema is None:
        feats = list(xs)
        for _ in range(layers_per_block):
            feats.append(conv2d(feats, filters_per_layer, pre_activation=pre_activation, filter_size=filter_size,
                                counters=counters, init=True, ema=None, weight_norm=weight_norm))
        return feats
    dev = xs[0].device
    segs0 = [int(t.shape[-1]) for t in xs]
    if isinstance(xs, ConcatList) and xs.buffer is not None:
        x0 = xs.buffer
    elif len(xs) == 1:
        x0 = xs[0]
    else:
        x0 = ops.extend_channels(xs, sum(segs0) + layers_per_block * filters_per_layer)
        if x0 is None:
            x0 = ops.concat_channels(xs)
    mult = 2 if pre_activation in ("celu", "crelu") else 1
    params = []
    c = sum(segs0)
    for _ in range(layers_per_block):
        name = get_name('conv2d', counters)
        V = get_var_maybe_avg(f"{name}/V", (filter_size[0], filter_size[1], c * mult, filters_per_layer),
                              "normal", ema, dev)
        g = get_var_maybe_avg(f"{name}/g", (filters_per_layer,), "ones", ema, dev)
        b = get_var_maybe_avg(f"{name}/b", (filters_per_layer,), "zeros", ema, dev)
        params.append((V, g, b))
        c += filters_per_layer
    buf = ops.dense_block_op(x0, segs0, params, ksize=filter_size[0], preact=ops.ACT[pre_activation])
    out = ConcatList(torch.split(buf, segs0 + [filters_per_layer] * layers_per_block, dim=3))
    out.buffer = buf
    return out


def feature_head(x):
    return ops.feature_head(x)


def glu(x):
    return ops.glu(x)


def tanh(x):
    return ops.tanh(x)


class _Updates:

    def __init__(self, params, lr, mom1, mom2):
        self.params = list(params)
        self.lr, self.mom1, self.mom2 = lr, mom1, mom2
        self.group = FlatGroup.of(self.params)
        self.state = [{}] if self.group is not None else [{} for _ in self.params]
        self.t = 1.0

    def fuse_ema(self, ema):
        return False

    def __call__(self, grads, lr=None):
        lr = self.lr if lr is None else lr
        with torch.no_grad():
            if self.group is not None and self._step_gather(list(grads), lr):
                pass
            elif self.group is not None:
                self._step(self.group.flat, self.group.flatten_like(list(grads), self.params), self.state[0], lr)
            else:
                for p, g, st in zip(self.params, grads, self.state):
                    self._step(p, g.contiguous(), st, lr)
        self.t += 1.0

    def state_dict(self):
        return {"t": self.t, "slots": [{k: (None if v is None else v.detach().cpu()) for k, v in st.items()}
                                       for st in self.state]}

    def load_state_dict(self, sd):
        self.t = float(sd["t"])
        targets = [self.group.flat] if self.group is not None else self.params
        if len(sd["slots"]) != len(self.state):
            raise ValueError("optimiser state does not match this parameter layout")
        for st, saved, p in zip(self.state, sd["slots"], targets):
            for k in [k for k in st if k not in saved]:
                del st[k]
            for k, v in saved.items():
                cur = st.get(k)
                if v is not None and cur is not None and cur.shape == v.shape and cur.dtype == v.dtype:
                    cur.copy_(v)
                else:
                    st[k] = None if v is None else v.to(p.device).clone()


    def _step_gather(self, grads, lr):
        return False


class _Adam(_Updates):
    _ema = None

    def fuse_ema(self, ema):
        flat = getattr(ema, "_flat", None)
        if self.group is None or flat is None or flat[1] is not self.group or len(self.params) > ops.ADAM_MAX_SEGMENTS:
            return False
        self._ema = ema
        return True

    def _step_gather(self, grads, lr):
        if len(self.params) > ops.ADAM_MAX_SEGMENTS:
            if self._ema is not None:
                raise RuntimeError("fused EMA needs the gathered Adam step")
            return False
        st, p = self.state[0], self.group.flat
        if not st:
            st["mg"] = torch.zeros_like(p)
            st["v"] = torch.zeros_like(p) if self.mom1 > 0 else None
        ema = self._ema
        ops.adam_step_gather(p, self.group.in_buffer_order(grads, self.params), self.group.offsets(), st["v"], st["mg"],
                             lr, self.mom1, self.mom2, self.t,
                             ema._flat[0] if ema is not None else None, ema.decay if ema is not None else 0.0,
                             coef=self.coef_dev if self.capturing else None)
        return True

    coef_dev = None
    capturing = False

    def ensure_state(self):
        if self.group is not None and not self.state[0]:
            p = self.group.flat
            self.state[0]["mg"] = torch.zeros_like(p)
            self.state[0]["v"] = torch.zeros_like(p) if self.mom1 > 0 else None

    def write_coefficients(self):
        c1, c2 = ops.adam_coefficients(self.mom1, self.mom2, self.t)
        self.coef_dev.copy_(torch.tensor([c1, c2], dtype=torch.float32))

    def _step(self, p, g, st, lr):
        if not st:
            st["mg"] = torch.zeros_like(p)
            st["v"] = torch.zeros_like(p) if self.mom1 > 0 else None
        ops.adam_step(p, g, st["v"], st["mg"], lr, self.mom1, self.mom2, self.t, coef=self.coef_dev if self.capturing else None)


class _Adamax(_Updates):
    def _step(self, p, g, st, lr):
        if not st:
            st["mg"] = torch.zeros_like(p)
            st["v"] = torch.zeros_like(p) if self.mom1 > 0 else None
        ops.adamax_step(p, g, st["v"], st["mg"], lr, self.mom1, self.mom2)


class _Nesterov(_Updates):
    def _step(self, p, g, st, lr):
        if not st:
            st["v"] = torch.zeros_like(p)
        ops.nesterov_step(p, g, st["v"], lr, self.mom1)


def _maybe_apply(upd, cost_or_grads):
    if isinstance(cost_or_grads, (list, tuple)):
        upd(cost_or_grads)
    elif cost_or_grads is not None:
        upd(torch.autograd.grad(cost_or_grads, upd.params))
    return upd


def adam_updates(params, cost_or_grads=None, lr=0.001, mom1=0.9, mom2=0.999):
    return _maybe_apply(_Adam(params, lr, mom1, mom2), cost_or_grads)


def adamax_updates(params, cost_or_grads=None, lr=0.001, mom1=0.9, mom2=0.999):
    return _maybe_apply(_Adamax(params, lr, mom1, mom2), cost_or_grads)


def nesterov_updates(params, cost_or_grads=None, lr=0.01, mom1=0.9):
    return _maybe_apply(_Nesterov(params, lr, mom1, None), cost_or_grads)
```

Before: 30580.

## Defer weight-norm backward into a fused Adam step that also emits column sums

In eager single-device runs, weight-norm backward now computes only the dot/dg reduction, and passes the raw dw to the optimizer tagged as pending. A new fused Adam kernel applies the weight-norm gradient transform, the Adam update and the EMA in one pass over the parameters. The same pass accumulates column sum-of-squares and amax partials of the updated weights, which the next forward pass reuses so it can skip recomputing the weight-norm scale. This removes a full elementwise dV pass and a separate norm reduction. In exchange it adds cross-module bookkeeping for pending gradients, is disabled under graphs and collectives, and raises an error for weights used twice in one backward pass.

```diff
diff --git a/include/otgan_layers.h b/include/otgan_layers.h
--- a/include/otgan_layers.h
+++ b/include/otgan_layers.h
@@ -103,6 +103,12 @@
 int otgan_weightnorm_bwd_f32(const float* V, const float* g, const float* inv_norm,
                              const float* dw, int K, int Cout, float* dV, float* dg,
                              float* scratch, void* stream);
+size_t otgan_weightnorm_dot_scratch_floats(int K, int Cout);
+int otgan_weightnorm_bwd_dot_f32(const float* V, const float* inv_norm, const float* dw, int K, int Cout, float* dot,
+                                 float* dg, float* scratch, size_t scratch_floats, void* stream);
+int otgan_colreduce_nchunk(long rows, int cols);
+int otgan_weightnorm_scale_amax_partials_f32(const float* g, int K, int Cout, float* inv_norm, float* scale, float* w_amax,
+                                             const float* scratch, size_t scratch_floats, void* stream);
 
 #define OTGAN_WN_MAX_LAYERS 16
 typedef struct otgan_wn_fwd_layer {
@@ -161,6 +167,10 @@
 int otgan_adam_step_gather_coef_f32(float* p, const float* const* grads, const long* offsets, int nseg, float* v, float* mg,
                                     double lr, double mom1, double mom2, double t, const float* coef_dev, float* ema_shadow,
                                     double ema_decay, void* stream);
+int otgan_adam_weightnorm_step_f32(float* p, long offset, const float* dw, const float* dot, const float* inv_norm,
+                                   const float* g, int K, int Cout, float* v, float* mg, double lr, double mom1, double mom2,
+                                   double t, const float* coef_dev, float* ema_shadow, double ema_decay, float* scratch,
+                                   size_t scratch_floats, void* stream);
 #define OTGAN_COPY2D_MAX_SEGMENTS 64
 int otgan_copy2d_batched_f32(const float* const* src, float* const* dst, const int* rows, const int* cols,
                              const long* src_ld, const long* dst_ld, int nseg, void* stream);
diff --git a/ot-gan_amd/_lib_layers.py b/ot-gan_amd/_lib_layers.py
--- a/ot-gan_amd/_lib_layers.py
+++ b/ot-gan_amd/_lib_layers.py
@@ -84,6 +84,12 @@
     "otgan_weightnorm_scale_amax_f32": (c_int, [c_fp, c_fp, c_int, c_int, c_fp, c_fp, c_fp, c_fp, c_size_t, c_fp]),
     "otgan_conv2d_prepare_filters_raw_f32": (c_int, [P_DESC, c_int, c_fp, c_fp, c_fp, c_size_t, c_fp]),
     "otgan_weightnorm_bwd_f32": (c_int, [c_fp, c_fp, c_fp, c_fp, c_int, c_int, c_fp, c_fp, c_fp, c_fp]),
+    "otgan_weightnorm_dot_scratch_floats": (c_size_t, [c_int, c_int]),
+    "otgan_weightnorm_bwd_dot_f32": (c_int, [c_fp, c_fp, c_fp, c_int, c_int, c_fp, c_fp, c_fp, c_size_t, c_fp]),
+    "otgan_colreduce_nchunk": (c_int, [c_long, c_int]),
+    "otgan_weightnorm_scale_amax_partials_f32": (c_int, [c_fp, c_int, c_int, c_fp, c_fp, c_fp, c_fp, c_size_t, c_fp]),
+    "otgan_adam_weightnorm_step_f32": (c_int, [c_fp, c_long, c_fp, c_fp, c_fp, c_fp, c_int, c_int, c_fp, c_fp, c_double,
+                                               c_double, c_double, c_double, c_fp, c_fp, c_double, c_fp, c_size_t, c_fp]),
     "otgan_weightnorm_fwd_batched16_f32": (c_int, [ctypes.POINTER(WnFwdLayer), c_int, c_fp]),
     "otgan_weightnorm_bwd_batched16_f32": (c_int, [ctypes.POINTER(WnBwdLayer), c_int, c_fp]),
     "otgan_colsum_f32": (c_int, [c_fp, c_long, c_int, c_long, c_fp, c_fp, c_fp]),
diff --git a/ot-gan_amd/csrc/pointwise.hip b/ot-gan_amd/csrc/pointwise.hip
--- a/ot-gan_amd/csrc/pointwise.hip
+++ b/ot-gan_amd/csrc/pointwise.hip
@@ -83,6 +83,46 @@
   }
 }
 
+template <bool CMAX>
+__device__ __forceinline__ void colsq_step(float a, float& s, unsigned& m) {
+  s = __fmaf_rn(a, a, s);
+  if constexpr (CMAX) {
+    const unsigned b = amax_bits(a);
+    m = b > m ? b : m;
+  }
+}
+template <bool CMAX>
+__device__ __forceinline__ void colreduce4_tail(float4 s, uint4 m, int rsub, int cq, bool live, int chunk, int cols,
+                                                float* __restrict__ partial, unsigned* __restrict__ pmax) {
+  __shared__ float4 red[16][17];
+  red[rsub][cq] = s;
+  __syncthreads();
+  if (threadIdx.x < 16 && live) {
+    float4 t = make_float4(0.f, 0.f, 0.f, 0.f);
+#pragma unroll
+    for (int k = 0; k < 16; ++k) {
+      const float4 v = red[k][threadIdx.x];
+      t.x += v.x; t.y += v.y; t.z += v.z; t.w += v.w;
+    }
+    const int cc = blockIdx.x * 64 + 4 * threadIdx.x;
+    *reinterpret_cast<float4*>(partial + (long)chunk * cols + cc) = t;
+  }
+  if constexpr (CMAX) {
+    __shared__ uint4 redm[16][17];
+    redm[rsub][cq] = m;
+    __syncthreads();
+    if (threadIdx.x < 16 && live) {
+      uint4 u = make_uint4(0u, 0u, 0u, 0u);
+#pragma unroll
+      for (int k = 0; k < 16; ++k) {
+        const uint4 v = redm[k][threadIdx.x];
+        u.x = v.x > u.x ? v.x : u.x; u.y = v.y > u.y ? v.y : u.y; u.z = v.z > u.z ? v.z : u.z; u.w = v.w > u.w ? v.w : u.w;
+      }
+      *reinterpret_cast<uint4*>(pmax + (long)chunk * cols + (blockIdx.x * 64 + 4 * threadIdx.x)) = u;
+    }
+  }
+}
+
 template <int OP, bool CMAX>
 __device__ __forceinline__ void colreduce4_body(const float* __restrict__ a, const float* __restrict__ b, long rows,
                                                 int cols, long lda, float* __restrict__ partial,
@@ -103,44 +143,15 @@
       if (OP == 0) {
         s.x += av.x; s.y += av.y; s.z += av.z; s.w += av.w;
       } else if (OP == 1) {
-        s.x += av.x * av.x; s.y += av.y * av.y; s.z += av.z * av.z; s.w += av.w * av.w;
+        colsq_step<CMAX>(av.x, s.x, m.x); colsq_step<CMAX>(av.y, s.y, m.y);
+        colsq_step<CMAX>(av.z, s.z, m.z); colsq_step<CMAX>(av.w, s.w, m.w);
       } else {
         const float4 bv = *reinterpret_cast<const float4*>(b + r * lda + c);
         s.x += av.x * bv.x; s.y += av.y * bv.y; s.z += av.z * bv.z; s.w += av.w * bv.w;
       }
-      if constexpr (CMAX) {
-        const unsigned bx = amax_bits(av.x), by = amax_bits(av.y), bz = amax_bits(av.z), bw = amax_bits(av.w);
-        m.x = bx > m.x ? bx : m.x; m.y = by > m.y ? by : m.y; m.z = bz > m.z ? bz : m.z; m.w = bw > m.w ? bw : m.w;
-      }
-    }
-  }
-  __shared__ float4 red[16][17];
-  red[rsub][cq] = s;
-  __syncthreads();
-  if (threadIdx.x < 16 && c < cols) {
-    float4 t = make_float4(0.f, 0.f, 0.f, 0.f);
-#pragma unroll
-    for (int k = 0; k < 16; ++k) {
-      const float4 v = red[k][threadIdx.x];
-      t.x += v.x; t.y += v.y; t.z += v.z; t.w += v.w;
-    }
-    const int cc = blockIdx.x * 64 + 4 * threadIdx.x;
-    *reinterpret_cast<float4*>(partial + (long)chunk * cols + cc) = t;
-  }
-  if constexpr (CMAX) {
-    __shared__ uint4 redm[16][17];
-    redm[rsub][cq] = m;
-    __syncthreads();
-    if (threadIdx.x < 16 && c < cols) {
-      uint4 u = make_uint4(0u, 0u, 0u, 0u);
-#pragma unroll
-      for (int k = 0; k < 16; ++k) {
-        const uint4 v = redm[k][threadIdx.x];
-        u.x = v.x > u.x ? v.x : u.x; u.y = v.y > u.y ? v.y : u.y; u.z = v.z > u.z ? v.z : u.z; u.w = v.w > u.w ? v.w : u.w;
-      }
-      *reinterpret_cast<uint4*>(pmax + (long)chunk * cols + (blockIdx.x * 64 + 4 * threadIdx.x)) = u;
-    }
-  }
+    }
+  }
+  colreduce4_tail<CMAX>(s, m, rsub, cq, c < cols, chunk, cols, partial, pmax);
 }
 template <int OP>
 __global__ __launch_bounds__(256) void colreduce4_kernel(const float* __restrict__ a,
@@ -154,15 +165,19 @@
   colreduce4_body<1, true>(a, nullptr, rows, cols, lda, partial, pmax);
 }
 
+inline int colreduce_nchunk(long rows, int cols) {
+  long nchunk = ceil_div(1024, ceil_div(cols, 64));
+  if (nchunk > kChunks) nchunk = kChunks;
+  if (nchunk > ceil_div_l(rows, 64)) nchunk = ceil_div_l(rows, 64);
+  if (nchunk < 1) nchunk = 1;
+  return (int)nchunk;
+}
 template <int OP>
 int colreduce(const float* a, const float* b, long rows, int cols, long lda, float* partial,
               int* nchunk_out, hipStream_t s, unsigned* pmax = nullptr) {
   const int colblocks = ceil_div(cols, 64);
-  long nchunk = ceil_div(1024, colblocks);
-  if (nchunk > kChunks) nchunk = kChunks;
-  if (nchunk > ceil_div_l(rows, 64)) nchunk = ceil_div_l(rows, 64);
-  if (nchunk < 1) nchunk = 1;
-  dim3 grid(colblocks, (int)nchunk);
+  const int nchunk = colreduce_nchunk(rows, cols);
+  dim3 grid(colblocks, nchunk);
   const bool vec = (cols % 4 == 0) && (lda % 4 == 0) && ((reinterpret_cast<uintptr_t>(a) & 15) == 0) &&
                    (!b || (reinterpret_cast<uintptr_t>(b) & 15) == 0) &&
                    ((reinterpret_cast<uintptr_t>(partial) & 15) == 0) &&
@@ -172,7 +187,7 @@
     else hipLaunchKernelGGL(colsq_cmax_kernel, grid, dim3(256), 0, s, a, rows, cols, lda, partial, pmax);
   } else if (vec) hipLaunchKernelGGL(colreduce4_kernel<OP>, grid, dim3(256), 0, s, a, b, rows, cols, lda, partial);
   else hipLaunchKernelGGL(colreduce_kernel<OP>, grid, dim3(256), 0, s, a, b, rows, cols, lda, partial);
-  *nchunk_out = (int)nchunk;
+  *nchunk_out = nchunk;
   OTGAN_CHECK_LAUNCH("colreduce");
   return OTGAN_OK;
 }
@@ -245,6 +260,10 @@
   amax_commit(rec, mb);
 }
 
+__device__ __forceinline__ float wn_dv(float V, float g, float iv, float dw, float dot) {
+  const float t = __fmul_rn(__fmul_rn(V, dot), iv);
+  return __fmul_rn(__fmul_rn(g, iv), __fmaf_rn(-iv, t, dw));
+}
 __global__ void weightnorm_bwd_kernel(const float* __restrict__ V, const float* __restrict__ g,
                                       const float* __restrict__ inv, const float* __restrict__ dw,
                                       const float* __restrict__ dot, long total, int Cout,
@@ -252,8 +271,7 @@
   for (long i = (long)blockIdx.x * blockDim.x + threadIdx.x; i < total;
        i += (long)gridDim.x * blockDim.x) {
     const int c = (int)(i % Cout);
-    const float iv = inv[c];
-    dV[i] = g[c] * iv * (dw[i] - V[i] * dot[c] * iv * iv);
+    dV[i] = wn_dv(V[i], g[c], inv[c], dw[i], dot[c]);
   }
 }
 __global__ __launch_bounds__(256) void wn_dot_finish_kernel(const float* __restrict__ partial, int nchunk, int cols,
@@ -783,12 +801,70 @@
   const int seg = blockIdx.y;
   const long base = segs.off[seg], n = segs.off[seg + 1] - base;
   const float* __restrict__ g = segs.g[seg];
+  if (!g) return;
   for (long i = (long)blockIdx.x * blockDim.x + threadIdx.x; i < n; i += (long)gridDim.x * blockDim.x) {
     const long j = base + i;
     const float pn = adam_elem(p[j], g[i], v, mg, j, lr, mom1, om1, mom2, om2, c1, c2);
     p[j] = pn;
     if (sh) sh[j] = ema_elem(sh[j], pn, decay, omd);
   }
+}
+__global__ __launch_bounds__(256) void adam_wn_kernel(float* __restrict__ p, const float* __restrict__ dw,
+                                                      const float* __restrict__ dot, const float* __restrict__ inv,
+                                                      const float* __restrict__ g, float* __restrict__ v,
+                                                      float* __restrict__ mg, float* __restrict__ sh, long rows, int cols,
+                                                      float lr, float mom1, float om1, float mom2, float om2, float c1, float c2,
+                                                      float decay, float omd, const float* __restrict__ coef,
+                                                      float* __restrict__ partial, unsigned* __restrict__ pmax) {
+  if (coef) {
+    c1 = coef[0];
+    c2 = coef[1];
+  }
+  const int lane = threadIdx.x & 63, wave = threadIdx.x >> 6;
+  const int cq = lane & 15, rsub = (lane >> 4) + 4 * wave;
+  const int c = blockIdx.x * 64 + 4 * cq;
+  const int chunk = blockIdx.y;
+  const long per = ceil_div_l(rows, (long)gridDim.y);
+  const long r0 = chunk * per;
+  long r1 = r0 + per;
+  if (r1 > rows) r1 = rows;
+  float s[4] = {0.f, 0.f, 0.f, 0.f};
+  unsigned m[4] = {0u, 0u, 0u, 0u};
+  if (c < cols) {
+    const f32x4 g4 = *reinterpret_cast<const f32x4*>(g + c), iv4 = *reinterpret_cast<const f32x4*>(inv + c),
+                dot4 = *reinterpret_cast<const f32x4*>(dot + c);
+    for (long r = r0 + rsub; r < r1; r += 16) {
+      const long i = r * cols + c;
+      f32x4 p4 = *reinterpret_cast<const f32x4*>(p + i);
+      const f32x4 dw4 = *reinterpret_cast<const f32x4*>(dw + i);
+      f32x4 mg4 = *reinterpret_cast<const f32x4*>(mg + i);
+      f32x4 v4 = {0.f, 0.f, 0.f, 0.f}, sh4 = {0.f, 0.f, 0.f, 0.f};
+      if (mom1 > 0.f) v4 = *reinterpret_cast<const f32x4*>(v + i);
+      if (sh) sh4 = *reinterpret_cast<const f32x4*>(sh + i);
+      float va[4], ma[4];
+#pragma unroll
+      for (int k = 0; k < 4; ++k) {
+        va[k] = v4[k];
+        ma[k] = mg4[k];
+      }
+#pragma unroll
+      for (int k = 0; k < 4; ++k) {
+        const float gi = wn_dv(p4[k], g4[k], iv4[k], dw4[k], dot4[k]);
+        const float pn = adam_elem(p4[k], gi, va, ma, k, lr, mom1, om1, mom2, om2, c1, c2);
+        p4[k] = pn;
+        sh4[k] = ema_elem(sh4[k], pn, decay, omd);
+        colsq_step<true>(pn, s[k], m[k]);
+        v4[k] = va[k];
+        mg4[k] = ma[k];
+      }
+      *reinterpret_cast<f32x4*>(p + i) = p4;
+      *reinterpret_cast<f32x4*>(mg + i) = mg4;
+      if (mom1 > 0.f) *reinterpret_cast<f32x4*>(v + i) = v4;
+      if (sh) *reinterpret_cast<f32x4*>(sh + i) = sh4;
+    }
+  }
+  colreduce4_tail<true>(make_float4(s[0], s[1], s[2], s[3]), make_uint4(m[0], m[1], m[2], m[3]), rsub, cq, c < cols, chunk,
+                        cols, partial, pmax);
 }
 __global__ void ema_kernel(float* __restrict__ sh, const float* __restrict__ p, long n, float decay,
                            float omd) {
@@ -859,6 +935,38 @@
   hipLaunchKernelGGL(weightnorm_bwd_kernel, dim3(grid_for(total)), dim3(256), 0, s, V, g, inv_norm, dw,
                      scratch, total, Cout, dV);
   OTGAN_CHECK_LAUNCH("weightnorm bwd");
+  return OTGAN_OK;
+}
+int otgan_colreduce_nchunk(long rows, int cols) { return (rows > 0 && cols > 0) ? colreduce_nchunk(rows, cols) : 0; }
+size_t otgan_weightnorm_dot_scratch_floats(int K, int Cout) {
+  return (K > 0 && Cout > 0) ? (size_t)colreduce_nchunk(K, Cout) * Cout : 0;
+}
+int otgan_weightnorm_bwd_dot_f32(const float* V, const float* inv_norm, const float* dw, int K, int Cout, float* dot,
+                                 float* dg, float* scratch, size_t scratch_floats, void* stream) {
+  OTGAN_CHECK_ARG(V && inv_norm && dw && dot && dg && scratch && K > 0 && Cout > 0, "bad arguments");
+  OTGAN_CHECK_ARG(scratch_floats >= otgan_weightnorm_dot_scratch_floats(K, Cout),
+                  "scratch smaller than otgan_weightnorm_dot_scratch_floats");
+  hipStream_t s = (hipStream_t)stream;
+  ProfScope ps(OTGAN_PROF_POINTWISE, 0.0, 4.0 * 2 * (double)K * Cout, s);
+  int nchunk = 0;
+  int rc = colreduce<2>(dw, V, K, Cout, Cout, scratch, &nchunk, s);
+  if (rc) return rc;
+  hipLaunchKernelGGL(wn_dot_finish_kernel, dim3(ceil_div(Cout, 64)), dim3(256), 0, s, scratch, nchunk, Cout, inv_norm, dot, dg);
+  OTGAN_CHECK_LAUNCH("weightnorm bwd (dot)");
+  return OTGAN_OK;
+}
+int otgan_weightnorm_scale_amax_partials_f32(const float* g, int K, int Cout, float* inv_norm, float* scale, float* w_amax,
+                                             const float* scratch, size_t scratch_floats, void* stream) {
+  OTGAN_CHECK_ARG(g && inv_norm && scale && w_amax && scratch && K > 0 && Cout > 0, "bad arguments");
+  OTGAN_CHECK_ARG(scratch_floats >= otgan_weightnorm_scale_scratch_floats(K, Cout),
+                  "scratch smaller than otgan_weightnorm_scale_scratch_floats");
+  hipStream_t s = (hipStream_t)stream;
+  long bound = ceil_div_l(K, 64);
+  if (bound > kChunks) bound = kChunks;
+  const unsigned* pmax = reinterpret_cast<const unsigned*>(scratch + (size_t)bound * Cout);
+  hipLaunchKernelGGL(weightnorm_scale_finish_kernel, dim3(ceil_div(Cout, 64)), dim3(256), 0, s, scratch, pmax,
+                     colreduce_nchunk(K, Cout), Cout, g, inv_norm, scale, w_amax);
+  OTGAN_CHECK_LAUNCH("weightnorm scale (from partials)");
   return OTGAN_OK;
 }
 
@@ -966,12 +1074,9 @@
   hipStream_t s = (hipStream_t)stream;
   ProfScope ps(OTGAN_PROF_POINTWISE, 0.0, 4.0 * 5 * (double)rows * C, s);
   const int colblocks = ceil_div(C, 64);
-  long nchunk = ceil_div(1024, colblocks);
-  if (nchunk > kChunks) nchunk = kChunks;
-  if (nchunk > ceil_div_l(rows, 64)) nchunk = ceil_div_l(rows, 64);
-  if (nchunk < 1) nchunk = 1;
-  hipLaunchKernelGGL(glu_bwd4_colsum_kernel, dim3(colblocks, (int)nchunk), dim3(256), 0, s, x, dy, rows, C, dx, dx_amax, scratch);
-  hipLaunchKernelGGL(colreduce_finish_kernel<0>, dim3(ceil_div(2 * C, 64)), dim3(256), 0, s, scratch, (int)nchunk, 2 * C, colsum);
+  const int nchunk = colreduce_nchunk(rows, C);
+  hipLaunchKernelGGL(glu_bwd4_colsum_kernel, dim3(colblocks, nchunk), dim3(256), 0, s, x, dy, rows, C, dx, dx_amax, scratch);
+  hipLaunchKernelGGL(colreduce_finish_kernel<0>, dim3(ceil_div(2 * C, 64)), dim3(256), 0, s, scratch, nchunk, 2 * C, colsum);
   OTGAN_CHECK_LAUNCH("glu bwd (+ column sums)");
   return OTGAN_OK;
 }
@@ -1053,15 +1158,17 @@
   hipStream_t s = (hipStream_t)stream;
   AdamSegs segs;
   memset(&segs, 0, sizeof(segs));
-  long longest = 0;
+  long longest = 0, n = 0;
   for (int i = 0; i < nseg; ++i) {
-    OTGAN_CHECK_ARG(grads[i] && offsets[i + 1] > offsets[i], "segment %d: null gradient or empty range", i);
+    OTGAN_CHECK_ARG(offsets[i + 1] > offsets[i], "segment %d: empty range", i);
     segs.g[i] = grads[i];
     segs.off[i] = offsets[i];
+    if (!grads[i]) continue;
     if (offsets[i + 1] - offsets[i] > longest) longest = offsets[i + 1] - offsets[i];
+    n += offsets[i + 1] - offsets[i];
   }
   segs.off[nseg] = offsets[nseg];
-  const long n = offsets[nseg] - offsets[0];
+  if (!n) return OTGAN_OK;
   ProfScope ps(OTGAN_PROF_POINTWISE, 0.0, 4.0 * (ema_shadow ? 9 : 7) * (double)n, s);
   float c[2] = {1.f, 1.f};
   if (!coef_dev) otgan_adam_coefficients(mom1, mom2, t, c);
@@ -1071,6 +1178,32 @@
   OTGAN_CHECK_LAUNCH("adam (gathered gradients)");
   return OTGAN_OK;
 }
+int otgan_adam_weightnorm_step_f32(float* p, long offset, const float* dw, const float* dot, const float* inv_norm,
+                                   const float* g, int K, int Cout, float* v, float* mg, double lr, double mom1, double mom2,
+                                   double t, const float* coef_dev, float* ema_shadow, double ema_decay, float* scratch,
+                                   size_t scratch_floats, void* stream) {
+  OTGAN_CHECK_ARG(p && dw && dot && inv_norm && g && mg && scratch && K > 0 && Cout > 0 && offset >= 0 &&
+                      (coef_dev || t >= 1.0) && (mom1 <= 0.0 || v), "bad arguments");
+  OTGAN_CHECK_ARG(Cout % 4 == 0 && offset % 4 == 0 && aligned16(p) && aligned16(dw) && aligned16(dot) && aligned16(inv_norm) &&
+                      aligned16(g) && aligned16(v) && aligned16(mg) && aligned16(ema_shadow) && aligned16(scratch),
+                  "fused weight-norm Adam needs Cout %% 4 == 0, an offset that is a multiple of 4 and 16-byte aligned tensors");
+  OTGAN_CHECK_ARG(scratch_floats >= otgan_weightnorm_scale_scratch_floats(K, Cout),
+                  "scratch smaller than otgan_weightnorm_scale_scratch_floats");
+  hipStream_t s = (hipStream_t)stream;
+  const long n = (long)K * Cout;
+  ProfScope ps(OTGAN_PROF_POINTWISE, 0.0, 4.0 * ((ema_shadow ? 6 : 4) + (mom1 > 0.0 ? 4 : 2)) * (double)n, s);
+  long bound = ceil_div_l(K, 64);
+  if (bound > kChunks) bound = kChunks;
+  unsigned* pmax = reinterpret_cast<unsigned*>(scratch + (size_t)bound * Cout);
+  float c[2] = {1.f, 1.f};
+  if (!coef_dev) otgan_adam_coefficients(mom1, mom2, t, c);
+  hipLaunchKernelGGL(adam_wn_kernel, dim3(ceil_div(Cout, 64), colreduce_nchunk(K, Cout)), dim3(256), 0, s, p + offset, dw, dot,
+                     inv_norm, g, v ? v + offset : nullptr, mg + offset, ema_shadow ? ema_shadow + offset : nullptr, (long)K,
+                     Cout, (float)lr, (float)mom1, (float)(1.0 - mom1), (float)mom2, (float)(1.0 - mom2), c[0], c[1],
+                     (float)ema_decay, (float)(1.0 - ema_decay), coef_dev, scratch, pmax);
+  OTGAN_CHECK_LAUNCH("adam (weight-norm backward fused)");
+  return OTGAN_OK;
+}
 int otgan_adamax_step_f32(float* p, const float* grad, float* v, float* mg, long n, double lr,
                           double mom1, double mom2, void* stream) {
   OTGAN_CHECK_ARG(p && grad && mg && n > 0 && (mom1 <= 0.0 || v), "bad arguments");
diff --git a/ot-gan_amd/ops.py b/ot-gan_amd/ops.py
--- a/ot-gan_amd/ops.py
+++ b/ot-gan_amd/ops.py
@@ -178,17 +178,24 @@
 FILTERS_FROM_RAW = True
 
 
-def weightnorm_scale(V2d, g):
+def weightnorm_scale(V2d, g, owner=None):
     K, Cout = V2d.shape
     L = _lib.lib()
     inv = torch.empty(Cout, dtype=V2d.dtype, device=V2d.device)
     scale = torch.empty(Cout, dtype=V2d.dtype, device=V2d.device)
     rec = amax_slot(V2d.device)
     n = L.otgan_weightnorm_scale_scratch_floats(K, Cout)
-    scratch = torch.empty(n, dtype=torch.float32, device=V2d.device)
-    _lib.check(L.otgan_weightnorm_scale_amax_f32(V2d.data_ptr(), g.data_ptr(), K, Cout, inv.data_ptr(), scale.data_ptr(),
-                                                 rec.data_ptr(), scratch.data_ptr(), n, _lib.stream_ptr()),
-               "weightnorm_scale")
+    sums = _take_column_sums(V2d if owner is None else owner, V2d, g, n)
+    if sums is not None:
+        _lib.check(L.otgan_weightnorm_scale_amax_partials_f32(g.data_ptr(), K, Cout, inv.data_ptr(), scale.data_ptr(),
+                                                              rec.data_ptr(), sums.data_ptr(), n,
+                                                              _lib.stream_ptr()), "weightnorm_scale (partials)")
+        sums.record_stream(torch.cuda.current_stream())
+    else:
+        scratch = torch.empty(n, dtype=torch.float32, device=V2d.device)
+        _lib.check(L.otgan_weightnorm_scale_amax_f32(V2d.data_ptr(), g.data_ptr(), K, Cout, inv.data_ptr(), scale.data_ptr(),
+                                                     rec.data_ptr(), scratch.data_ptr(), n, _lib.stream_ptr()),
+                   "weightnorm_scale")
     tag_amax(scale, rec)
     leave(scale, "raw", V2d)
     return scale, inv
@@ -204,6 +211,99 @@
                                                    dg.data_ptr(), scratch.data_ptr(),
                                                    _lib.stream_ptr()), "weightnorm_bwd")
     return dV, dg
+
+
+WN_BWD_IN_ADAM = False
+_WN_PENDING_SEEN = set()
+_COLUMN_SUMS = "_otgan_column_sums"
+
+
+def _wn_key(V2d):
+    return (V2d.untyped_storage().data_ptr(), V2d.storage_offset())
+
+
+def wn_deferrable(V2d, g, dw):
+    return (V2d.shape[1] % 4 == 0 and V2d.storage_offset() % 4 == 0 and V2d.is_contiguous() and
+            all(t.data_ptr() % 16 == 0 for t in (V2d, g, dw)))
+
+
+def weightnorm_bwd_dot(V2d, inv, dw):
+    K, Cout = V2d.shape
+    L = _lib.lib()
+    dot = torch.empty(Cout, dtype=V2d.dtype, device=V2d.device)
+    dg = torch.empty(Cout, dtype=V2d.dtype, device=V2d.device)
+    n = L.otgan_weightnorm_dot_scratch_floats(K, Cout)
+    scratch = torch.empty(n, dtype=torch.float32, device=V2d.device)
+    _lib.check(L.otgan_weightnorm_bwd_dot_f32(V2d.data_ptr(), inv.data_ptr(), dw.data_ptr(), K, Cout, dot.data_ptr(),
+                                              dg.data_ptr(), scratch.data_ptr(), n, _lib.stream_ptr()), "weightnorm_bwd_dot")
+    return dot, dg
+
+
+def finish_weightnorm_bwd(t):
+    pend = take(t, "wn_pending", remove=True)
+    if pend is None:
+        return t
+    _dot, inv, g, V2d = pend
+    dV, _dg = weightnorm_bwd(V2d, g, inv, t.view(V2d.shape))
+    return dV.view(t.shape)
+
+
+class PendingGrads(list):
+
+    def __init__(self, raw):
+        super().__init__(raw)
+        self.raw = list(raw)
+        self._true = {}
+
+    def _get(self, i):
+        if i not in self._true:
+            t = self.raw[i]
+            pend = take(t, "wn_pending")
+            self._true[i] = t if pend is None else weightnorm_bwd(pend[3], pend[2], pend[1], t.view(pend[3].shape))[0].view(t.shape)
+        return self._true[i]
+
+    def __getitem__(self, i):
+        if isinstance(i, slice):
+            return [self._get(j) for j in range(*i.indices(len(self.raw)))]
+        return self._get(range(len(self.raw))[i])
+
+    def __iter__(self):
+        return (self._get(i) for i in range(len(self.raw)))
+
+
+def forget_pending_weightnorm():
+    _WN_PENDING_SEEN.clear()
+
+
+def adam_weightnorm_step(p_flat, offset, dw, pend, v, mg, lr, mom1, mom2, t, ema_shadow=None, ema_decay=0.0, coef=None):
+    dot, inv, g, V2d = pend
+    K, Cout = V2d.shape
+    L = _lib.lib()
+    n = L.otgan_weightnorm_scale_scratch_floats(K, Cout)
+    sums = torch.empty(n, dtype=torch.float32, device=p_flat.device)
+    bump_weights_epoch(p_flat)
+    if ema_shadow is not None:
+        bump_weights_epoch(ema_shadow)
+    dot.record_stream(torch.cuda.current_stream())
+    _lib.check(L.otgan_adam_weightnorm_step_f32(p_flat.data_ptr(), offset, dw.data_ptr(), dot.data_ptr(), inv.data_ptr(),
+                                                g.data_ptr(), K, Cout, _lib.ptr(v), mg.data_ptr(), float(lr), float(mom1),
+                                                float(mom2), float(t), _lib.ptr(coef), _lib.ptr(ema_shadow), float(ema_decay),
+                                                sums.data_ptr(), n, _lib.stream_ptr()), "adam_weightnorm_step")
+    return sums
+
+
+def leave_column_sums(V, g, sums):
+    setattr(V, _COLUMN_SUMS, (_token(V, g), sums))
+
+
+def _take_column_sums(owner, V2d, g, numel):
+    ent = getattr(owner, _COLUMN_SUMS, None)
+    if ent is None:
+        return None
+    delattr(owner, _COLUMN_SUMS)
+    if ent[0] != _token(V2d, g) or ent[1].numel() != numel or torch.cuda.is_current_stream_capturing():
+        return None
+    return ent[1]
 
 
 def colsum(a2d_ptr, rows, cols, lda, device):
@@ -475,7 +575,7 @@
 
         def compute(raw=raw_ok):
             if raw:
-                scale, inv_norm = weightnorm_scale(V2d, g)
+                scale, inv_norm = weightnorm_scale(V2d, g, owner=V)
                 return scale, scale, inv_norm, {"fwd": prepare_filters(desc, 2 if nfold else 0, scale), "bwd": None,
                                                 "bwd_done": False, "bwd_which": 3 if nfold else 1, "raw": scale}
             w, wT, inv_norm = weightnorm_fwd(V2d, g)
@@ -578,8 +678,16 @@
             if need_w:
                 dw = torch.empty_like(V2d)
                 conv_wgrad_raw(desc, x, ctx.cmap, dy, dw)
-                dV2d, dg = weightnorm_bwd(V2d, g, inv_norm, dw)
-                dV = dV2d.view(ctx.vshape)
+                if WN_BWD_IN_ADAM and wn_deferrable(V2d, g, dw):
+                    if _wn_key(V2d) in _WN_PENDING_SEEN:
+                        raise RuntimeError("WN_BWD_IN_ADAM: a weight used twice in one backward pass cannot defer its "
+                                           "weight-norm backward (the engine would add the raw weight gradients)")
+                    _WN_PENDING_SEEN.add(_wn_key(V2d))
+                    dot, dg = weightnorm_bwd_dot(V2d, inv_norm, dw)
+                    dV = leave(dw.view(ctx.vshape), "wn_pending", (dot, inv_norm, g, V2d))
+                else:
+                    dV2d, dg = weightnorm_bwd(V2d, g, inv_norm, dw)
+                    dV = dV2d.view(ctx.vshape)
             if need_b:
                 db = colsum_of(dy)
                 if db is None:
@@ -1429,7 +1537,7 @@
     bump_weights_epoch(p_flat)
     if ema_shadow is not None:
         bump_weights_epoch(ema_shadow)
-    gp = (ctypes.c_void_p * n)(*[g.data_ptr() for g in grads])
+    gp = (ctypes.c_void_p * n)(*[_lib.ptr(g) for g in grads])
     off = (ctypes.c_long * (n + 1))(*offsets)
     _lib.check(_lib.lib().otgan_adam_step_gather_coef_f32(p_flat.data_ptr(), ctypes.cast(gp, ctypes.c_void_p),
                                                           ctypes.cast(off, ctypes.c_void_p), n, _lib.ptr(v), mg.data_ptr(),
diff --git a/ot-gan_amd/trainer.py b/ot-gan_amd/trainer.py
--- a/ot-gan_amd/trainer.py
+++ b/ot-gan_amd/trainer.py
@@ -139,6 +139,7 @@
         asked = getattr(args, "step_graph", None)
         want = (env == "1") if env in ("0", "1") else (args.model == "densenet" if asked is None else bool(asked))
         self.graphs = GraphedSteps(self) if (want and not self.collectives and self.world == 1) else None
+        self.wn_bwd_in_adam = not self.collectives and self.world == 1 and self.disc_buckets is None
 
     def enable_timers(self, on=True):
         self.timers = {} if on else None
@@ -245,10 +246,15 @@
                 return self.last
         from . import ops
         ops.SIDE_STREAM = self._side_stream if self.fork_wgrad else None
+        opt = self.disc_optimizer if kind == "disc" else self.gen_optimizer
+        ops.WN_BWD_IN_ADAM = bool(self.wn_bwd_in_adam and apply_updates and self.graphs is None and
+                                  getattr(opt, "applies_weightnorm_bwd", lambda: False)())
         try:
             dist, ent, grads = self._step_body(x_data, kind, noise, apply_updates, aug)
         finally:
             ops.SIDE_STREAM = None
+            ops.WN_BWD_IN_ADAM = False
+            ops.forget_pending_weightnorm()
         self._mark_step_end()
         self._d_weights_in_graph = False
         self.step_counter += 1
@@ -275,6 +281,11 @@
         opt(grads, lr=lr)
         if not critic and not self.ema_fused:
             self.maintain_averages()
+
+    @staticmethod
+    def _handed_on(grads):
+        from . import ops
+        return ops.PendingGrads(grads) if ops.WN_BWD_IN_ADAM else grads
 
     def _backward(self, outputs, params, grad_outputs):
         from . import ops
@@ -322,7 +333,7 @@
                 grads = (self.disc_buckets.finish() if self.disc_buckets is not None
                          else parallel.allreduce_sum_(list(grads)))
             if apply_updates:
-                self._optimise(self.disc_optimizer, grads, -a.learning_rate_disc, critic=True)
+                self._optimise(self.disc_optimizer, self._handed_on(grads), -a.learning_rate_disc, critic=True)
         else:
             side = self._side_stream if self.fork_real_pass else None
             if side is not None:
@@ -355,7 +366,7 @@
                 grads = (self.gen_buckets.finish() if self.gen_buckets is not None
                          else parallel.allreduce_sum_(list(grads)))
             if apply_updates:
-                self._optimise(self.gen_optimizer, grads, a.learning_rate_gen, critic=False)
+                self._optimise(self.gen_optimizer, self._handed_on(grads), a.learning_rate_gen, critic=False)
         return dist, ent, grads
 
     @torch.no_grad()
diff --git a/ot-gan_amd/utils/nn.py b/ot-gan_amd/utils/nn.py
--- a/ot-gan_amd/utils/nn.py
+++ b/ot-gan_amd/utils/nn.py
@@ -372,14 +372,17 @@
 
     def __call__(self, grads, lr=None):
         lr = self.lr if lr is None else lr
+        grads = grads.raw if isinstance(grads, ops.PendingGrads) else list(grads)
         with torch.no_grad():
-            if self.group is not None and self._step_gather(list(grads), lr):
+            if self.group is not None and self._step_gather(grads, lr):
                 pass
-            elif self.group is not None:
-                self._step(self.group.flat, self.group.flatten_like(list(grads), self.params), self.state[0], lr)
             else:
-                for p, g, st in zip(self.params, grads, self.state):
-                    self._step(p, g.contiguous(), st, lr)
+                grads = [ops.finish_weightnorm_bwd(g) for g in grads]
+                if self.group is not None:
+                    self._step(self.group.flat, self.group.flatten_like(grads, self.params), self.state[0], lr)
+                else:
+                    for p, g, st in zip(self.params, grads, self.state):
+                        self._step(p, g.contiguous(), st, lr)
         self.t += 1.0
 
     def state_dict(self):
@@ -416,6 +419,9 @@
         self._ema = ema
         return True
 
+    def applies_weightnorm_bwd(self):
+        return self.group is not None and len(self.params) <= ops.ADAM_MAX_SEGMENTS
+
     def _step_gather(self, grads, lr):
         if len(self.params) > ops.ADAM_MAX_SEGMENTS:
             if self._ema is not None:
@@ -426,10 +432,22 @@
             st["mg"] = torch.zeros_like(p)
             st["v"] = torch.zeros_like(p) if self.mom1 > 0 else None
         ema = self._ema
-        ops.adam_step_gather(p, self.group.in_buffer_order(grads, self.params), self.group.offsets(), st["v"], st["mg"],
-                             lr, self.mom1, self.mom2, self.t,
-                             ema._flat[0] if ema is not None else None, ema.decay if ema is not None else 0.0,
-                             coef=self.coef_dev if self.capturing else None)
+        shadow, decay = (ema._flat[0], ema.decay) if ema is not None else (None, 0.0)
+        coef = self.coef_dev if self.capturing else None
+        ordered, offsets = self.group.in_buffer_order(grads, self.params), self.group.offsets()
+        left = []
+        for i, (gr, prm) in enumerate(zip(ordered, self.group.params)):
+            pend = ops.take(gr, "wn_pending", remove=True)
+            if pend is not None:
+                sums = ops.adam_weightnorm_step(p, offsets[i], gr, pend, st["v"], st["mg"], lr, self.mom1, self.mom2, self.t,
+                                                shadow, decay, coef=coef)
+                left.append((prm, pend[2], sums))
+                ordered[i] = None
+        if len(left) < len(ordered):
+            ops.adam_step_gather(p, ordered, offsets, st["v"], st["mg"], lr, self.mom1, self.mom2, self.t, shadow, decay,
+                                 coef=coef)
+        for prm, g, sums in left:
+            ops.leave_column_sums(prm, g, sums)
         return True
 
     coef_dev = None
```

Result: no change. 30830, median of 6 (+0.8%).
